# tudocomp/tudocomp

Hardware: AMD Instinct MI355X
Metric: input MB/s end-to-end lcpcomp+huffman (higher is better)
Workload: dtype u32; 1 GPU; lcpcomp(coder=huff,threshold=2,flatten=1,comp=arrays) on 2000000000 B english text (SURVEY 8d generator, seed 42): pinned host text -> H2D -> kernels + host Huffman table -> D2H -> stream in pinned host memory, all timed; bytes_per_gpu=2000000000, parallelism=single GPU

## Files before the change

tudocomp_amd/csrc/api_ctx.hip:

```cpp
#include "api.hpp"
#include "huffman_host.hpp"

#include <strings.h>
#include <ctype.h>

using namespace tdc;

namespace tdc {

int lcpcomp_enc_coder(int coder) {
    const int base = coder & 0xFF, k = coder >> 8;
    if (base == TDC_GPU_CODER_SLE) {
        if (k < 0 || k > 7) throw ArgError{TDC_GPU_ERR_ARG, "sle: kmer must be in 1..7"};
        return 3 | ((k ? k : 3) << 8);
    }
    if (k == 0 && base == TDC_GPU_CODER_HUFF) return 0;
    if (k == 0 && base == TDC_GPU_CODER_ARITH) return 1;
    if (k == 0 && base == TDC_GPU_CODER_ASCII) return 2;
    throw ArgError{TDC_GPU_ERR_UNSUPPORTED, "lcpcomp: coder must be huff, arithmetic, ascii or sle"};
}

void reserve_arena(Ctx& c, size_t bytes) {
    if (c.arena.size < bytes) {
        size_t fr = 0, tot = 0;
        if (hipMemGetInfo(&fr, &tot) == hipSuccess && fr + c.arena.size < bytes) {
            static thread_local char msg[256];
            snprintf(msg, sizeof(msg), "device %d has %.1f GB free of %.1f GB, this call needs an arena of %.1f GB (112 bytes per text byte + 192 MiB): "
                     "use smaller blocks (tdc_gpu_arena_bytes)", c.device, (double)(fr + c.arena.size) / 1e9, (double)tot / 1e9, (double)bytes / 1e9);
            throw ArgError{TDC_GPU_ERR_OOM, msg};
        }
        (void)hipGetLastError();
    }
    c.ensure_arena(bytes);
}

}

extern "C" {

const char* tdc_gpu_strerror(int status) {
    switch (status) {
        case TDC_GPU_OK: return "success";
        case TDC_GPU_ERR_HIP: return "HIP runtime error (is a gfx950 GPU visible?)";
        case TDC_GPU_ERR_ARG: return "invalid argument";
        case TDC_GPU_ERR_NO_SENTINEL: return "Expected a sentinel byte (0) at the end of the input text";
        case TDC_GPU_ERR_TOO_LARGE: return "input too large: text length must be < 2^31";
        case TDC_GPU_ERR_OOM: return "out of memory";
        case TDC_GPU_ERR_UNSUPPORTED: return "No implementation found for this coder/strategy";
        case TDC_GPU_ERR_INTERNAL: return "internal error";
        default: return "unknown status";
    }
}

const char* tdc_gpu_last_error(const tdc_gpu_ctx* ctx) { return ctx ? ctx->last_error.c_str() : ""; }

void tdc_gpu_free(void* p) { free(p); }

namespace {
struct OptionDef { const char* name; void (*set)(Ctx&, long); };
inline int clampi(long v, long lo, long hi) { return (int)(v < lo ? lo : (v > hi ? hi : v)); }
const OptionDef OPTIONS[] = {
    { "fastread",         [](Ctx& c, long v) { c.fast_read = v ? 1 : 0; } },
    { "sa_local",         [](Ctx& c, long v) { c.sa_local_sort = (int)v; } },
    { "radix_waves",      [](Ctx& c, long v) { c.radix_waves = v == 8 ? 8 : 4; } },
    { "window_lcut",      [](Ctx& c, long v) { c.window_lcut = clampi(v, 0, 63); } },
    { "window_halo",      [](Ctx& c, long v) { c.window_halo = clampi(v, 0, 2048); } },
    { "dec_seg",          [](Ctx& c, long v) { c.dec_seg = v < 4096 ? 4096 : (v > (1l << 30) ? (size_t)1 << 30 : (size_t)v); } },
    { "dec_lean",         [](Ctx& c, long v) { c.dec_lean = v != 0; } },
    { "dec_parse",        [](Ctx& c, long v) { c.dec_parse = clampi(v, 0, 2); } },
    { "dec_done",         [](Ctx& c, long v) { c.dec_done = v != 0; } },
    { "dec_log",          [](Ctx& c, long v) { c.dec_log = v != 0; } },
    { "bwt_log",          [](Ctx& c, long v) { c.bwt_log = v != 0; } },
    { "pipe_log",         [](Ctx& c, long v) { c.pipe_log = v != 0; } },
    { "window_force_fail",[](Ctx& c, long v) { c.window_force_fail = v ? 1 : 0; } },
    { "window_large",     [](Ctx& c, long v) { c.window_large_lists = v ? 1 : 0; } },
    { "window_src",       [](Ctx& c, long v) { c.window_src = v ? 1 : 0; } },
    { "plcp_samples",     [](Ctx& c, long v) { c.plcp_samples = v != 0; } },
    { "small_pipeline",   [](Ctx& c, long v) { c.small_pipeline = v != 0; } },
    { "small_big",        [](Ctx& c, long v) { c.small_big = (int)v; } },
    { "small_prof",       [](Ctx& c, long v) { c.small_prof = v != 0; } },
    { "phi_lazy",         [](Ctx& c, long v) { c.phi_lazy = v != 0; } },
    { "fs_pair",          [](Ctx& c, long v) { c.fs_pair = v != 0; } },
    { "enc_early",        [](Ctx& c, long v) { c.enc_early = (int)v; } },
    { "owner_rem",        [](Ctx& c, long v) { c.owner_rem = (int)std::min<long>(std::max<long>(v, 0), 8); } },
    { "enc_rec",          [](Ctx& c, long v) { c.enc_rec = v != 0; } },
    { "level_purge",      [](Ctx& c, long v) { c.level_purge = v != 0; } },
    { "level_log",        [](Ctx& c, long v) { c.level_log = v != 0; } },
    { "eager",            [](Ctx& c, long v) { c.eager_levels = v != 0; } },
    { "eager_dump",       [](Ctx& c, long v) { c.eager_dump = v != 0; } },
    { "flen_bytes",       [](Ctx& c, long v) { c.flen_bytes = v != 0; } },
    { "flatten_steps",    [](Ctx& c, long v) { c.flatten_steps = v <= 0 ? (1 << 30) : clampi(v, 1, 1 << 30); } },
    { "flatten_growth",   [](Ctx& c, long v) { c.flatten_growth = clampi(v, 2, 1 << 20); } },
    { "sa_refine",        [](Ctx& c, long v) { c.sa_refine = v != 0; } },
    { "sa_pairs",         [](Ctx& c, long v) { c.sa_pairs = v != 0; } },
    { "sa_stars",         [](Ctx& c, long v) { c.sa_stars = v != 0; } },
    { "sa_fused_init",    [](Ctx& c, long v) { c.sa_fused_init = v != 0; } },
    { "sa_init_syms",     [](Ctx& c, long v) { c.sa_init_syms = clampi(v, 0, 64); } },
    { "radix_lds",        [](Ctx& c, long v) { c.radix_lds = (v >= 0 && v <= 2) ? (int)v : 2; } },
    { "xcd_remap",        [](Ctx& c, long v) { c.xcd_remap = (v >= 0 && v <= 2) ? (int)v : 0; } },
    { "bucket_scatter",   [](Ctx& c, long v) { c.bucket_scatter = v ? 1 : 0; } },
    { "ssort",            [](Ctx& c, long v) { c.ssort = v ? 1 : 0; } },
    { "ssort_levels",     [](Ctx& c, long v) { c.ssort_levels = (v >= 1 && v <= 3) ? (int)v : 0; } },
    { "msd_partition",    [](Ctx& c, long v) { c.msd_partition = v ? 1 : 0; } },
    { "wsort",            [](Ctx& c, long v) { c.wsort = v ? 1 : 0; } },
    { "wsort_min",        [](Ctx& c, long v) { c.wsort_min = v < 4096 ? 4096 : (size_t)v; } },
    { "wsort_syms",       [](Ctx& c, long v) { c.wsort_syms = (v >= 4 && v <= 64) ? (int)v : 0; } },
    { "wsort_kw",         [](Ctx& c, long v) { c.wsort_kw = (v == 1 || v == 2) ? (int)v : 0; } },
    { "wsort_rounds",     [](Ctx& c, long v) { c.wsort_rounds = clampi(v, 0, 100); } },
    { "wsort_smallrun",   [](Ctx& c, long v) { c.wsort_small = v ? 1 : 0; } },
    { "wsort_overlap",    [](Ctx& c, long v) { c.wsort_overlap = v ? 1 : 0; } },
    { "wsort_predig",     [](Ctx& c, long v) { c.wsort_predig = v ? 1 : 0; } },
    { "wsort_prehist",    [](Ctx& c, long v) { c.wsort_prehist = v ? 1 : 0; } },
    { "sa_seg_bigcap",    [](Ctx& c, long v) { c.sa_seg_bigcap = clampi(v, 0, 65536); } },
    { "sa_seg_rounds",    [](Ctx& c, long v) { c.sa_seg_rounds = clampi(v, 0, 2); } },
    { "wsort_run_streams",[](Ctx& c, long v) { c.wsort_run_streams = v != 0; } },
    { "wsort_predig_skip",[](Ctx& c, long v) { c.wsort_predig_skip = clampi(v, 0, 24); } },
    { "wsort_fuse",       [](Ctx& c, long v) { c.wsort_fuse = v ? 1 : 0; } },
    { "wsort_order",      [](Ctx& c, long v) { c.wsort_order = v ? 1 : 0; } },
    { "wsort_two",        [](Ctx& c, long v) { c.wsort_two = (v >= 0 && v <= 2) ? (int)v : 0; } },
    { "wsort_leaf",       [](Ctx& c, long v) { c.wsort_leaf = v == 1024 ? 1024 : 2048; } },
    { "wsort_pack",       [](Ctx& c, long v) { c.wsort_pack = (v == 1024 || v == 4096) ? (int)v : 2048; } },
    { "wsort_cmax",       [](Ctx& c, long v) { c.wsort_cmax = clampi(v, 8, 64); } },
    { "wsort_log",        [](Ctx& c, long v) { c.wsort_log = v != 0; } },
    { "upload_chunks",    [](Ctx& c, long v) { c.upload_chunks = clampi(v, 4, 24); } },
    { "upload_tail_n",    [](Ctx& c, long v) { c.upload_tail_n = clampi(v, 0, 12); } },
    { "upload_tail_pct",  [](Ctx& c, long v) { c.upload_tail_pct = clampi(v, 30, 100); } },
    { "arena_log",        [](Ctx& c, long v) { c.arena_log = v != 0; } },
};
constexpr size_t NOPTIONS = sizeof(OPTIONS) / sizeof(OPTIONS[0]);
const OptionDef FOLD_OPTIONS[] = {
    { "fused_cand",       [](Ctx& c, long v) { c.fused_cand = v != 0; } },
    { "sel_tile_counts",  [](Ctx& c, long v) { c.sel_tile_counts = v != 0; } },
};
constexpr size_t NFOLD = sizeof(FOLD_OPTIONS) / sizeof(FOLD_OPTIONS[0]);
const OptionDef* find_option(const char* name) {
    if (!name) return nullptr;
    if (!strncasecmp(name, "TDC_GPU_", 8)) name += 8;
    for (size_t i = 0; i < NOPTIONS; ++i) if (!strcasecmp(name, OPTIONS[i].name)) return &OPTIONS[i];
    for (size_t i = 0; i < NFOLD; ++i) if (!strcasecmp(name, FOLD_OPTIONS[i].name)) return &FOLD_OPTIONS[i];
    return nullptr;
}
void apply_env_options(tdc_gpu_ctx* ctx) {
    const char* on = getenv("TDC_GPU_DEBUG_KNOBS");
    if (!on || atoi(on) == 0) return;
    for (size_t i = 0; i < NOPTIONS + NFOLD; ++i) {
        const OptionDef& o = i < NOPTIONS ? OPTIONS[i] : FOLD_OPTIONS[i - NOPTIONS];
        char var[64] = "TDC_GPU_";
        size_t k = 8;
        for (const char* q = o.name; *q && k + 1 < sizeof(var); ++q) var[k++] = (char)toupper((unsigned char)*q);
        var[k] = 0;
        if (const char* m = getenv(var)) o.set(ctx->c, atol(m));
    }
}
}

int tdc_gpu_ctx_set_option(tdc_gpu_ctx* ctx, const char* name, long value) {
    if (!ctx) return TDC_GPU_ERR_ARG;
    const OptionDef* o = find_option(name);
    if (!o) return TDC_GPU_ERR_ARG;
    o->set(ctx->c, value);
    return TDC_GPU_OK;
}
int tdc_gpu_option_count(void) { return (int)NOPTIONS; }
const char* tdc_gpu_option_name(int i) { return (i >= 0 && (size_t)i < NOPTIONS) ? OPTIONS[i].name : nullptr; }

int tdc_gpu_ctx_create(int device, tdc_gpu_ctx** out) {
    if (!out) return TDC_GPU_ERR_ARG;
    *out = nullptr;
    int count = 0;
    if (hipGetDeviceCount(&count) != hipSuccess || count <= 0) { (void)hipGetLastError(); return TDC_GPU_ERR_HIP; }
    if (device < 0 || device >= count) return TDC_GPU_ERR_ARG;
    tdc_gpu_ctx* ctx = new (std::nothrow) tdc_gpu_ctx();
    if (!ctx) return TDC_GPU_ERR_OOM;
    ctx->c.huff_ok = huffman_selfcheck();
    ctx->c.device = device;
    ctx->c.wpre = &ctx->pre;
    DeviceGuard dg(device);
    try {
        HIP_TRY(dg.enter());
        HIP_TRY(hipStreamCreateWithFlags(&ctx->c.stream, hipStreamNonBlocking));
        for (auto& e : ctx->c.ev) HIP_TRY(hipEventCreate(&e));
        HIP_TRY(hipStreamCreateWithFlags(&ctx->c.copy_stream, hipStreamNonBlocking));
        {
            int lo = 0, hi = 0;
            if (hipDeviceGetStreamPriorityRange(&lo, &hi) != hipSuccess) { lo = 0; (void)hipGetLastError(); }
            if (hipStreamCreateWithPriority(&ctx->c.aux_stream, hipStreamNonBlocking, lo) != hipSuccess) { ctx->c.aux_stream = nullptr; (void)hipGetLastError(); }
        }
        HIP_TRY(hipEventCreateWithFlags(&ctx->c.ev_join, hipEventDisableTiming));
        HIP_TRY(hipEventCreateWithFlags(&ctx->c.ev_dig2, hipEventDisableTiming));
        for (auto& e : ctx->c.ev_chunk) HIP_TRY(hipEventCreateWithFlags(&e, hipEventDisableTiming));
        ctx->c.pinned_size = 4096;
        HIP_TRY(hipHostMalloc(&ctx->c.pinned, ctx->c.pinned_size, hipHostMallocDefault));
        HIP_TRY(hipHostMalloc((void**)&ctx->c.pinned_hdr, Ctx::PINNED_HDR, hipHostMallocDefault));
        if (ctx->c.fast_read) {
            void* zc = nullptr;
            if (hipHostMalloc(&zc, (size_t)Ctx::ZC_WORDS * Ctx::ZC_BLOCKS * 4, hipHostMallocMapped | hipHostMallocCoherent) == hipSuccess) {
                void* dv = nullptr;
                if (hipHostGetDevicePointer(&dv, zc, 0) == hipSuccess) { ctx->c.zc_host = (u32*)zc; ctx->c.zc_dev = (u32*)dv; memset(zc, 0, (size_t)Ctx::ZC_WORDS * Ctx::ZC_BLOCKS * 4); }
                else { (void)hipHostFree(zc); (void)hipGetLastError(); }
            } else (void)hipGetLastError();
        }
        HIP_TRY(hipMalloc((void**)&ctx->c.d_err, 256));
        HIP_TRY(hipMemset(ctx->c.d_err, 0, 256));
        apply_env_options(ctx);
    } catch (const HipError&) {
        (void)hipGetLastError();
        tdc_gpu_ctx_destroy(ctx);
        return TDC_GPU_ERR_HIP;
    }
    *out = ctx;
    return TDC_GPU_OK;
}

void tdc_gpu_ctx_destroy(tdc_gpu_ctx* ctx) {
    if (!ctx) return;
    DeviceGuard dg(ctx->c.device);
    (void)dg.enter();
    (void)sync_streams(ctx->c);
    if (ctx->c.arena.base) (void)hipFree(ctx->c.arena.base);
    if (ctx->c.pinned) (void)hipHostFree(ctx->c.pinned);
    if (ctx->c.pinned_hdr) (void)hipHostFree(ctx->c.pinned_hdr);
    if (ctx->c.pinned_tab) (void)hipHostFree(ctx->c.pinned_tab);
    if (ctx->c.zc_host) (void)hipHostFree(ctx->c.zc_host);
    if (ctx->c.d_err) (void)hipFree(ctx->c.d_err);
    for (auto& e : ctx->c.ev) if (e) (void)hipEventDestroy(e);
    for (auto& e : ctx->c.ev_chunk) if (e) (void)hipEventDestroy(e);
    for (hipEvent_t e : {ctx->c.ev_join, ctx->c.ev_dig2}) if (e) (void)hipEventDestroy(e);
    if (ctx->c.copy_stream) (void)hipStreamDestroy(ctx->c.copy_stream);
    if (ctx->c.aux_stream) (void)hipStreamDestroy(ctx->c.aux_stream);
    if (ctx->c.ev_pool) { for (int i = 0; i < ctx->c.ev_pool_size; ++i) if (ctx->c.ev_pool[i]) (void)hipEventDestroy(ctx->c.ev_pool[i]); free(ctx->c.ev_pool); }
    free(ctx->c.pend);
    if (ctx->c.stream) (void)hipStreamDestroy(ctx->c.stream);
    delete ctx;
}

int tdc_gpu_ctx_set_profiling(tdc_gpu_ctx* ctx, int enabled) {
    return guarded(ctx, [&] {
        Ctx& c = ctx->c;
        if (enabled && !c.ev_pool) {
            c.ev_pool_size = 16384; c.pend_cap = 8192;
            c.ev_pool = (hipEvent_t*)calloc(c.ev_pool_size, sizeof(hipEvent_t));
            c.pend = (Ctx::Pending*)calloc(c.pend_cap, sizeof(Ctx::Pending));
            if (!c.ev_pool || !c.pend) throw std::bad_alloc();
            for (int i = 0; i < c.ev_pool_size; ++i) HIP_TRY(hipEventCreate(&c.ev_pool[i]));
        }
        c.profiling = enabled != 0;
    });
}

void tdc_gpu_ctx_reset_profile(tdc_gpu_ctx* ctx) {
    if (!ctx) return;
    for (auto& k : ctx->c.kprof) k = KernelProfile();
}

const char* tdc_gpu_ctx_kernel_profile(const tdc_gpu_ctx* ctx, int idx, double* ms, uint64_t* launches, uint64_t* bytes) {
    static const char* names[K_CLASS_COUNT] = {
        "rs_scatter_kernel<u64>", "rs_scatter_kernel<u32>", "rs_count_kernel", "scan_kernels",
        "sa_groups_kernel", "sa_build_keys_kernel", "phi_kernel", "plcp_kernel", "cand_kernels",
        "level_init_kernel", "mis_round_kernel", "resolve_kernel", "push_kernel", "apply_kernel", "pool_kernels", "small_level_kernel", "window_levels_kernel",
        "flatten_round_kernel", "gaps_kernel", "literal_hist_kernel", "tile_bits_kernel", "pack_kernel", "extract_kernels",
        "ss_leaf_sort_kernel", "sa_local_sort_kernel", "window_scatter_kernels",
        "ws_leaf_sort_kernel", "ws_leaf_count_kernel", "ws_run_kernels", "fs_image_kernel" };
    if (!ctx || idx < 0 || idx >= K_CLASS_COUNT) return nullptr;
    const KernelProfile& k = ctx->c.kprof[idx];
    if (ms) *ms = k.ms;
    if (launches) *launches = k.launches;
    if (bytes) *bytes = k.bytes;
    return names[idx];
}

size_t tdc_gpu_arena_bytes(size_t n) { return arena_need(n); }

int tdc_gpu_device_memory(int device, size_t* free_bytes, size_t* total_bytes) {
    if (!free_bytes || !total_bytes) return TDC_GPU_ERR_ARG;
    int count = 0;
    if (hipGetDeviceCount(&count) != hipSuccess || device < 0 || device >= count) { (void)hipGetLastError(); return TDC_GPU_ERR_ARG; }
    DeviceGuard dg(device);
    if (dg.enter() != hipSuccess || hipMemGetInfo(free_bytes, total_bytes) != hipSuccess) { (void)hipGetLastError(); return TDC_GPU_ERR_HIP; }
    return TDC_GPU_OK;
}

int tdc_gpu_ctx_reserve(tdc_gpu_ctx* ctx, size_t n) {
    return guarded(ctx, [&] { reserve_arena(ctx->c, arena_need(ctx->c, n)); });
}

int tdc_gpu_host_register(void* p, size_t bytes) {
    if (!p || !bytes) return TDC_GPU_ERR_ARG;
    if (hipHostRegister(p, bytes, hipHostRegisterPortable) != hipSuccess) { (void)hipGetLastError(); return TDC_GPU_ERR_HIP; }
    return TDC_GPU_OK;
}
int tdc_gpu_host_unregister(void* p) {
    if (!p) return TDC_GPU_ERR_ARG;
    if (hipHostUnregister(p) != hipSuccess) { (void)hipGetLastError(); return TDC_GPU_ERR_HIP; }
    return TDC_GPU_OK;
}

int tdc_gpu_device_count(void) {
    int count = 0;
    if (hipGetDeviceCount(&count) != hipSuccess) { (void)hipGetLastError(); return 0; }
    return count;
}

void* tdc_gpu_host_alloc(size_t bytes) {
    void* p = nullptr;
    if (hipHostMalloc(&p, bytes ? bytes : 1, hipHostMallocDefault) != hipSuccess) { (void)hipGetLastError(); return nullptr; }
    return p;
}
void tdc_gpu_host_free(void* p) { if (p) (void)hipHostFree(p); }

size_t tdc_escape(const uint8_t* in, size_t n, uint8_t* out) {
    size_t o = 0;
    for (size_t i = 0; i < n; ++i) {
        const uint8_t ch = in[i];
        if (ch == 0x00) { out[o++] = 0xFF; out[o++] = 0xFE; }
        else if (ch == 0xFF) { out[o++] = 0xFF; out[o++] = 0xFF; }
        else out[o++] = ch;
    }
    out[o++] = 0;
    return o;
}

size_t tdc_unescape(const uint8_t* in, size_t n, uint8_t* out) {
    size_t o = 0;
    if (n && in[n - 1] == 0) --n;
    for (size_t i = 0; i < n; ++i) {
        const uint8_t ch = in[i];
        if (ch == 0xFF && i + 1 < n) { const uint8_t d = in[++i]; out[o++] = (d == 0xFE) ? 0x00 : d; }
        else out[o++] = ch;
    }
    return o;
}

int tdc_huffman_selfcheck(void) { return huffman_selfcheck() ? TDC_GPU_OK : TDC_GPU_ERR_INTERNAL; }

int tdc_huffman_table(const uint32_t counts[256], uint32_t* sigma, uint32_t* longest, uint8_t order[256],
                      uint8_t len_of[256], uint64_t code_of[256]) {
    if (!counts) return TDC_GPU_ERR_ARG;
    try {
        HuffTable t;
        build_huffman_table(counts, &t);
        if (sigma) *sigma = t.sigma;
        if (longest) *longest = t.longest;
        if (order) memcpy(order, t.order, 256);
        if (len_of) memcpy(len_of, t.len_of, 256);
        if (code_of) memcpy(code_of, t.code_of, 256 * sizeof(uint64_t));
    } catch (...) { return TDC_GPU_ERR_OOM; }
    return TDC_GPU_OK;
}

}
```

tudocomp_amd/csrc/common.hpp:

```cpp
#pragma once

#include <hip/hip_runtime.h>
#include <stdint.h>
#include <stddef.h>
#include <stdio.h>
#include <string.h>

namespace tdc {

typedef uint8_t  u8;
typedef uint32_t u32;
typedef uint16_t u16;
typedef uint64_t u64;

constexpr u32 NONE32 = 0xFFFFFFFFu;
constexpr int WAVE = 64;

enum {
    TDC_OK = 0,
    TDC_ERR_HIP = -1,
    TDC_ERR_ARG = -2,
    TDC_ERR_NO_SENTINEL = -3,
    TDC_ERR_TOO_LARGE = -4,
    TDC_ERR_OOM = -5,
    TDC_ERR_UNSUPPORTED = -6,
    TDC_ERR_INTERNAL = -7,
};

struct HipError { hipError_t e; const char* file; int line; };

#define HIP_TRY(expr)                                                                  \
    do {                                                                               \
        hipError_t _e = (expr);                                                        \
        if (_e != hipSuccess) throw ::tdc::HipError{_e, __FILE__, __LINE__};           \
    } while (0)

inline unsigned bits_for(u64 v) {
    unsigned b = 0;
    if (v == 0) return 1;
    while (v) { ++b; v >>= 1; }
    return b;
}

inline size_t align_up(size_t x, size_t a) { return (x + a - 1) / a * a; }
inline unsigned cdiv(size_t a, size_t b) { return (unsigned)((a + b - 1) / b); }

struct Arena {
    char* base = nullptr;
    size_t size = 0;
    size_t top = 0;
    size_t high = 0;

    size_t top_hi = 0;

    void* alloc(size_t bytes) {
        size_t off = align_up(top, 256);
        if (off + bytes > size - top_hi) throw HipError{hipErrorOutOfMemory, "arena", (int)__LINE__};
        top = off + bytes;
        if (top > high) high = top;
        return base + off;
    }
    template <typename T> T* get(size_t count) { return (T*)alloc(count * sizeof(T)); }
    void* alloc_top(size_t bytes) {
        if (bytes + top_hi + 256 > size) throw HipError{hipErrorOutOfMemory, "arena (top)", (int)__LINE__};
        const size_t off = (size - top_hi - bytes) & ~(size_t)255;
        if (off < top) throw HipError{hipErrorOutOfMemory, "arena (top)", (int)__LINE__};
        top_hi = size - off;
        return base + off;
    }
    template <typename T> T* get_top(size_t count) { return (T*)alloc_top(count * sizeof(T)); }
    void release_top() { top_hi = 0; }
    size_t mark() const { return top; }
    void release(size_t m) { top = m; }
};

enum KernelClass {
    K_RS_SCATTER_U64 = 0, K_RS_SCATTER_U32, K_RS_COUNT, K_SCAN,
    K_SA_RANK_SCATTER, K_SA_BUILD_KEYS, K_PHI, K_PLCP, K_CAND,
    K_LEVEL_INIT, K_MIS_ROUND, K_RESOLVE, K_PUSH, K_APPLY, K_POOL, K_SMALL_LEVEL, K_WINDOW_LEVELS,
    K_FLATTEN_ROUND, K_ENC_GAPS, K_ENC_HIST, K_ENC_TILE_BITS, K_ENC_PACK, K_EXTRACT, K_SS_LEAF, K_SA_LOCAL_SORT, K_WINDOW_SCATTER,
    K_WS_LEAF_SORT, K_WS_LEAF_COUNT, K_WS_RUN, K_FS_IMAGE,
    K_CLASS_COUNT
};

struct KernelProfile {
    double ms = 0;
    u64 launches = 0;
    u64 bytes = 0;
};

#ifdef __HIPCC__
static __global__ void publish_words_kernel(const uint32_t* __restrict__ src, uint32_t nwords, uint32_t* host_dst, uint32_t* host_flag,
                                            uint32_t seq) {
    for (uint32_t i = threadIdx.x; i < nwords; i += blockDim.x)
        __hip_atomic_store(&host_dst[i], src[i], __ATOMIC_RELAXED, __HIP_MEMORY_SCOPE_SYSTEM);
    __syncthreads();
    if (threadIdx.x == 0) {
        __threadfence_system();
        __hip_atomic_store(host_flag, seq, __ATOMIC_RELEASE, __HIP_MEMORY_SCOPE_SYSTEM);
    }
}
#endif

struct Ctx {
    int device = 0;
    hipStream_t stream = nullptr;
    Arena arena;
    hipEvent_t ev[16] = {};
    void* pinned = nullptr;
    size_t pinned_size = 0;
    void* pinned_tab = nullptr;
    size_t pinned_tab_size = 0;
    u8* pinned_hdr = nullptr;
    static constexpr size_t PINNED_HDR = 65536;
    void* pinned_table(size_t bytes) {
        if (pinned_tab_size < bytes) {
            if (pinned_tab) { (void)hipHostFree(pinned_tab); pinned_tab = nullptr; pinned_tab_size = 0; }
            HIP_TRY(hipHostMalloc(&pinned_tab, bytes, hipHostMallocDefault));
            pinned_tab_size = bytes;
        }
        return pinned_tab;
    }
    static constexpr u32 ZC_SEG_OFF = 1040, ZC_WORDS = 1040 + 16384;
    static constexpr u32 ZC_BLOCKS = 3;
    u32* zc_host = nullptr;
    u32* zc_dev = nullptr;
    u32 zc_seq = 0;
    int fast_read = 1;
    u32* d_err = nullptr;
    int sa_local_sort = 1;
    int radix_waves = 4;
    int plcp_samples = 1;
    bool huff_ok = true;
    int flen_bytes = 1;
    int eager_levels = 1;
    int level_purge = 1;
    int enc_rec = 1;
    int owner_rem = 8;
    int enc_early = 1;
    int fused_cand = 1;
    int sel_tile_counts = 1;
    int fs_pair = 1;
    int small_big = 1;
    int small_pipeline = 1;
    int sa_pairs = 1;
    int sa_stars = 1;
    int sa_refine = 1;
    int sa_fused_init = 1;
    int radix_lds = 1;
    int xcd_remap = 1;
    int window_src = 1;
    int window_lcut = 56;
    int window_halo = 320;
    size_t dec_seg = 0;
    bool phi_lazy = true;
    int dec_lean = 1;
    int dec_parse = 1;
    int window_force_fail = 0;
    int window_large_lists = 0;
    int ssort = 1;
    int ssort_levels = 0;
    int wsort = 1;
    size_t wsort_min = (size_t)1 << 20;
    int wsort_syms = 0;
    int wsort_kw = 0;
    int wsort_rounds = 24;
    int wsort_cmax = 24;
    int wsort_overlap = 1;
    int wsort_prehist = 1;
    bool wsort_count_nonheads = true;
    int sa_seg_bigcap = 65536;
    int sa_seg_rounds = 2;
    int wsort_run_streams = 1;
    int wsort_predig_skip = 4;
    int wsort_predig = 1;
    int wsort_two = 0;
    int wsort_leaf = 2048;
    int wsort_pack = 1024;
    int wsort_order = 1;
    int wsort_fuse = 1;
    int wsort_small = 0;
    int msd_partition = 1;
    int bucket_scatter = 1;
    int upload_tail_n = 3, upload_tail_pct = 60;
    int upload_chunks = 16;
    int flatten_steps = 1;
    int flatten_growth = 8;
    int sa_init_syms = 0;
    int dec_done = 1;
    int dec_log = 0, bwt_log = 0, pipe_log = 0, level_log = 0, wsort_log = 0, eager_dump = 0, small_prof = 0, arena_log = 0;

    u32 hist_cache[256] = {};
    const u8* hist_ptr = nullptr;
    size_t hist_n = 0;
    hipStream_t copy_stream = nullptr;
    hipStream_t aux_stream = nullptr;
    hipEvent_t ev_join = nullptr;
    static constexpr size_t CHUNK_EVENTS = 32;
    hipEvent_t ev_chunk[CHUNK_EVENTS] = {};
    hipEvent_t ev_dig2 = nullptr;
    struct WPre* wpre = nullptr;
    u8* d2h_host = nullptr;
    size_t d2h_cap = 0;
    size_t d2h_done = 0;

    bool profiling = false;
    KernelProfile kprof[K_CLASS_COUNT];
    struct Pending { hipEvent_t a, b; int cls; u64 bytes; };
    Pending* pend = nullptr;
    int npend = 0, pend_cap = 0;
    hipEvent_t* ev_pool = nullptr;
    int ev_pool_size = 0, ev_pool_used = 0;

    int prof_begin(int cls, u64 bytes) {
        if (!profiling || npend >= pend_cap || ev_pool_used + 2 > ev_pool_size) return -1;
        Pending& p = pend[npend];
        p.a = ev_pool[ev_pool_used++]; p.b = ev_pool[ev_pool_used++]; p.cls = cls; p.bytes = bytes;
        HIP_TRY(hipEventRecord(p.a, stream));
        return npend++;
    }
    void prof_end(int idx) { if (idx >= 0) HIP_TRY(hipEventRecord(pend[idx].b, stream)); }
    void wait_for(hipStream_t waiter, hipStream_t signaller) {
        HIP_TRY(hipEventRecord(ev_join, signaller));
        HIP_TRY(hipStreamWaitEvent(waiter, ev_join, 0));
    }
    struct ProfScope {
        Ctx& c; int idx;
        ProfScope(Ctx& ctx, int cls, u64 bytes) : c(ctx), idx(ctx.prof_begin(cls, bytes)) {}
        ~ProfScope() { if (idx >= 0) (void)hipEventRecord(c.pend[idx].b, c.stream); }
    };
    void prof_collect() {
        for (int i = 0; i < npend; ++i) {
            float t = 0;
            HIP_TRY(hipEventElapsedTime(&t, pend[i].a, pend[i].b));
            KernelProfile& k = kprof[pend[i].cls];
            k.ms += t; k.launches++; k.bytes += pend[i].bytes;
        }
        npend = 0; ev_pool_used = 0;
    }

    void ensure_arena(size_t bytes) {
        arena.top_hi = 0;
        if (arena.size >= bytes) { arena.top = 0; return; }
        if (arena.base) { HIP_TRY(hipFree(arena.base)); arena.base = nullptr; arena.size = 0; }
        HIP_TRY(hipMalloc((void**)&arena.base, bytes));
        if (arena_log) fprintf(stderr, "arena: %zu bytes at %p\n", bytes, (void*)arena.base);
        arena.size = bytes;
        arena.top = 0;
    }
#ifdef __HIPCC__
    bool read_words_fast(const void* dptr, void* out, size_t bytes) {
        if (!fast_read || !zc_host || bytes == 0 || bytes > 4096 || (bytes & 3) || ((uintptr_t)dptr & 3)) return false;
        const u32 seq = ++zc_seq;
        publish_words_kernel<<<1, 64, 0, stream>>>((const u32*)dptr, (u32)(bytes / 4), zc_dev, zc_dev + 1024, seq);
        if (hipGetLastError() != hipSuccess) return false;
        volatile u32* flag = zc_host + 1024;
        for (u64 spins = 0;; ++spins) {
            if (__atomic_load_n((const u32*)flag, __ATOMIC_ACQUIRE) == seq) break;
            if ((spins & 0xFFFF) == 0xFFFF) {
                const hipError_t q = hipStreamQuery(stream);
                if (q != hipSuccess && q != hipErrorNotReady) throw HipError{q, __FILE__, __LINE__};
            }
        }
        memcpy(out, zc_host, bytes);
        return true;
    }
    bool publish_begin(u32** dst, u32** flag, u32* seq, u32 block = 0) {
        if (!fast_read || !zc_host) return false;
        *seq = ++zc_seq; *dst = zc_dev + (size_t)block * ZC_WORDS; *flag = *dst + 1024;
        return true;
    }
    u32 publish_async(const void* dptr, size_t bytes, u32 block) {
        if (!fast_read || !zc_host || bytes == 0 || bytes > 4096 || (bytes & 3) || ((uintptr_t)dptr & 3) || block >= ZC_BLOCKS) return 0;
        u32 seq = ++zc_seq;
        if (seq == 0) seq = ++zc_seq;
        u32* dst = zc_dev + (size_t)block * ZC_WORDS;
        publish_words_kernel<<<1, 64, 0, stream>>>((const u32*)dptr, (u32)(bytes / 4), dst, dst + 1024, seq);
        return hipGetLastError() == hipSuccess ? seq : 0;
    }
    void publish_wait(u32 seq, void* out, size_t bytes, u32 block = 0) {
        volatile u32* flag = zc_host + (size_t)block * ZC_WORDS + 1024;
        for (u64 spins = 0;; ++spins) {
            if (__atomic_load_n((const u32*)flag, __ATOMIC_ACQUIRE) == seq) break;
            if ((spins & 0xFFFF) == 0xFFFF) {
                const hipError_t q = hipStreamQuery(stream);
                if (q != hipSuccess && q != hipErrorNotReady) throw HipError{q, __FILE__, __LINE__};
            }
        }
        memcpy(out, zc_host + (size_t)block * ZC_WORDS, bytes);
    }
#else
    bool read_words_fast(const void*, void*, size_t) { return false; }
#endif
    template <typename T> T read(const T* dptr) {
        T v;
        if (read_words_fast(dptr, &v, sizeof(T))) return v;
        T* h = (T*)pinned;
        HIP_TRY(hipMemcpyAsync(h, dptr, sizeof(T), hipMemcpyDeviceToHost, stream));
        HIP_TRY(hipStreamSynchronize(stream));
        return *h;
    }
    template <typename T> void read_n(const T* dptr, T* out, size_t count) {
        const size_t bytes = sizeof(T) * count;
        if (read_words_fast(dptr, out, bytes)) return;
        if (bytes <= pinned_size) {
            HIP_TRY(hipMemcpyAsync(pinned, dptr, bytes, hipMemcpyDeviceToHost, stream));
            HIP_TRY(hipStreamSynchronize(stream));
            memcpy(out, pinned, bytes);
        } else {
            HIP_TRY(hipMemcpyAsync(out, dptr, bytes, hipMemcpyDeviceToHost, stream));
            HIP_TRY(hipStreamSynchronize(stream));
        }
    }
};

struct StreamSwap {
    Ctx& c; hipStream_t saved;
    StreamSwap(Ctx& ctx, hipStream_t other) : c(ctx), saved(ctx.stream) { c.stream = other; }
    ~StreamSwap() { c.stream = saved; }
};

#define LAUNCH_CHECK() HIP_TRY(hipGetLastError())

#ifdef __HIPCC__

__device__ __forceinline__ int lane_id() { return threadIdx.x & 63; }

__device__ __forceinline__ u32 xcd_tile(u32 bid, u32 per_xcd) { return per_xcd ? (bid & 7u) * per_xcd + (bid >> 3) : bid; }
__device__ __forceinline__ int wave_id() { return threadIdx.x >> 6; }

__device__ __forceinline__ u32 wave_inclusive_sum_u32(u32 v) {
    v += (u32)__builtin_amdgcn_update_dpp(0, (int)v, 0x111, 0xF, 0xF, false);
    v += (u32)__builtin_amdgcn_update_dpp(0, (int)v, 0x112, 0xF, 0xF, false);
    v += (u32)__builtin_amdgcn_update_dpp(0, (int)v, 0x114, 0xF, 0xF, false);
    v += (u32)__builtin_amdgcn_update_dpp(0, (int)v, 0x118, 0xF, 0xF, false);
    v += (u32)__builtin_amdgcn_update_dpp(0, (int)v, 0x142, 0xA, 0xF, false);
    v += (u32)__builtin_amdgcn_update_dpp(0, (int)v, 0x143, 0xC, 0xF, false);
    return v;
}
template <typename T>
__device__ __forceinline__ T wave_inclusive_sum(T v) {
    if constexpr (sizeof(T) == 4) return (T)wave_inclusive_sum_u32((u32)v);
    const int lane = lane_id();
#pragma unroll
    for (int d = 1; d < 64; d <<= 1) {
        T o = __shfl_up(v, d, 64);
        if (lane >= d) v += o;
    }
    return v;
}
__device__ __forceinline__ u32 wave_inclusive_max(u32 v) {
    v = max(v, (u32)__builtin_amdgcn_update_dpp(0, (int)v, 0x111, 0xF, 0xF, false));
    v = max(v, (u32)__builtin_amdgcn_update_dpp(0, (int)v, 0x112, 0xF, 0xF, false));
    v = max(v, (u32)__builtin_amdgcn_update_dpp(0, (int)v, 0x114, 0xF, 0xF, false));
    v = max(v, (u32)__builtin_amdgcn_update_dpp(0, (int)v, 0x118, 0xF, 0xF, false));
    v = max(v, (u32)__builtin_amdgcn_update_dpp(0, (int)v, 0x142, 0xA, 0xF, false));
    v = max(v, (u32)__builtin_amdgcn_update_dpp(0, (int)v, 0x143, 0xC, 0xF, false));
    return v;
}
template <typename T>
__device__ __forceinline__ T wave_reduce_sum(T v) {
    if constexpr (sizeof(T) == 4) return (T)__builtin_amdgcn_readlane((int)wave_inclusive_sum_u32((u32)v), 63);
#pragma unroll
    for (int d = 32; d >= 1; d >>= 1) v += __shfl_xor(v, d, 64);
    return v;
}
__device__ __forceinline__ u32 wave_reduce_max(u32 v) { return (u32)__builtin_amdgcn_readlane((int)wave_inclusive_max(v), 63); }
__device__ __forceinline__ u32 wave_reduce_min(u32 v) { return ~wave_reduce_max(~v); }

template <typename T> __device__ __forceinline__ T lds_load(const T* p) { return *(const volatile __attribute__((address_space(3))) T*)p; }
template <typename T> __device__ __forceinline__ void lds_store(T* p, T v) { *(volatile __attribute__((address_space(3))) T*)p = v; }

__device__ __forceinline__ u64 wave_match_lds(unsigned long long* M, u32 d, bool valid, u64 lanebit) {
    const u32 d0 = __builtin_amdgcn_readfirstlane(d);
    if (__all(valid && d == d0)) return ~0ull;
#ifdef TDC_MATCH_B64
    if (valid) atomicOr(&M[d], (unsigned long long)lanebit);
#else
    if (valid) atomicOr((unsigned*)&M[d] + (lane_id() >> 5), (unsigned)(lanebit >> (32 * (lane_id() >> 5))));
#endif
    __builtin_amdgcn_wave_barrier();
    const u64 peers = valid ? lds_load(&M[d]) : 0ull;
    __builtin_amdgcn_wave_barrier();
    if (valid) lds_store(&M[d], 0ull);
    return peers;
}

template <int PEEL, int MING>
__device__ __forceinline__ u64 wave_match_peel(unsigned long long* M, u32 d, bool valid, u64 lanebit) {
    u64 rem = __ballot(valid);
    u64 peers = 0;
    bool done = !valid;
#pragma unroll
    for (int it = 0; it < PEEL; ++it) {
        if (!rem) break;
        const int lead = __builtin_ctzll(rem);
        const u32 dl = (u32)__builtin_amdgcn_readlane((int)d, lead);
        const u64 grp = __ballot(!done && d == dl);
        if (__popcll(grp) < MING) break;
        if (!done && d == dl) { peers = grp; done = true; }
        rem &= ~grp;
    }
    if (rem) {
        if (!done) atomicOr((unsigned*)&M[d] + (lane_id() >> 5), (unsigned)(lanebit >> (32 * (lane_id() >> 5))));
        __builtin_amdgcn_wave_barrier();
        if (!done) peers = lds_load(&M[d]);
        __builtin_amdgcn_wave_barrier();
        if (!done) lds_store(&M[d], 0ull);
    }
    return peers;
}

template <typename T, int NW>
__device__ __forceinline__ T block_exclusive_sum(T v, T* smem, T& total) {
    const int lane = lane_id(), w = wave_id();
    T inc = wave_inclusive_sum(v);
    if (lane == 63) smem[w] = inc;
    __syncthreads();
    if (threadIdx.x == 0) {
        T run = 0;
#pragma unroll
        for (int i = 0; i < NW; ++i) { T t = smem[i]; smem[i] = run; run += t; }
        smem[NW] = run;
    }
    __syncthreads();
    T res = smem[w] + inc - v;
    total = smem[NW];
    __syncthreads();
    return res;
}

template <int NW>
__device__ __forceinline__ u32 block_inclusive_max(u32 v, u32* smem, u32& total) {
    const int lane = lane_id(), w = wave_id();
    u32 inc = wave_inclusive_max(v);
    if (lane == 63) smem[w] = inc;
    __syncthreads();
    if (threadIdx.x == 0) {
        u32 run = 0;
#pragma unroll
        for (int i = 0; i < NW; ++i) { u32 t = smem[i]; smem[i] = run; run = max(run, t); }
        smem[NW] = run;
    }
    __syncthreads();
// ... 62 lines not shown
```

tudocomp_amd/csrc/fused.hip:

```cpp
#include "stages.hpp"
#include "prim.hpp"

#include <type_traits>

namespace tdc {

constexpr int FS_TILE = 4096;
constexpr int FS_ITEMS = 16;
constexpr u32 FS_WMAX = 8192;

struct FSLevel {
    const u32* idx_in; const void* rp_in; const u32* prev_in; const u8* lcp_in;
    u32* idx_out; void* rp_out; u8* lcp_out;
    u32* counts; const u32* blk_seg; const u32* blk_start; const u32* seg_start;
    u32 nseg, R, per_xcd; int shift;
    int lsh;
};
__device__ __forceinline__ bool fs_row(const FSLevel& P, u32 row, size_t& base, u32& cnt) {
    const u32 blk = row / P.R;
    if (blk >= P.blk_start[P.nseg]) return false;
    const u32 s = P.blk_seg[blk];
    const u64 t = (u64)(blk - P.blk_start[s]) * P.R + row % P.R;
    const u32 s0 = P.seg_start[s], s1 = P.seg_start[s + 1];
    const u64 off = t * FS_TILE;
    base = s0; cnt = 0;
    if (off >= (u64)(s1 - s0)) return true;
    base = (size_t)s0 + off;
    const u64 left = (u64)(s1 - s0) - off;
    cnt = left < FS_TILE ? (u32)left : (u32)FS_TILE;
    return true;
}

template <int DB>
__global__ __launch_bounds__(256) void fs_count_kernel(FSLevel P, u32 rows) {
    constexpr u32 D = 1u << DB;
    __shared__ u32 hist[D];
    const u32 row = xcd_tile(blockIdx.x, P.per_xcd);
    if (row >= rows) return;
    size_t base; u32 cnt;
    if (!fs_row(P, row, base, cnt)) return;
    for (u32 i = threadIdx.x; i < D; i += 256) hist[i] = 0;
    if (cnt == 0) { for (u32 i = threadIdx.x; i < D; i += 256) P.counts[(size_t)row * D + i] = 0; return; }
    __syncthreads();
    const u32 lb = wave_id() * (64 * FS_ITEMS) + lane_id();
    const u32* ip = P.idx_in + base + lb;
    u32 kk[FS_ITEMS];
#pragma unroll
    for (int j = 0; j < FS_ITEMS; ++j) kk[j] = (lb + (u32)j * 64 < cnt) ? ip[j * 64] : 0u;
#pragma unroll
    for (int j = 0; j < FS_ITEMS; ++j) {
        const bool valid = lb + (u32)j * 64 < cnt;
        const u32 d = (kk[j] >> P.shift) & (D - 1);
        const u32 d0 = __builtin_amdgcn_readfirstlane(d);
        if (__all(valid && d == d0)) { if (lane_id() == 0) atomicAdd(&hist[d0], 64u); }
        else if (valid) atomicAdd(&hist[d], 1u);
    }
    __syncthreads();
    for (u32 i = threadIdx.x; i < D; i += 256) P.counts[(size_t)row * D + i] = hist[i];
}

#ifndef TDC_FS_WPE
#define TDC_FS_WPE 4
#endif
template <int DB, bool FIRST, int PAIR, bool WP>
__global__ __launch_bounds__(256 * PAIR) __attribute__((amdgpu_waves_per_eu(TDC_FS_WPE, TDC_FS_WPE))) void fs_scatter_kernel(FSLevel P, u32 rows) {
    constexpr int NT = 256 * PAIR;
    constexpr u32 TILE = (u32)FS_TILE * PAIR;
    constexpr u32 D = 1u << DB;
    __shared__ u32 tcnt[D];
    __shared__ u32 gbase[D];
    __shared__ __align__(16) u64 stage[TILE];
    __shared__ u32 scan_sm[NT / 64 + 1];
    const int lane = lane_id();
    const u32 row = xcd_tile(blockIdx.x, P.per_xcd) * PAIR;
    if (row >= rows) return;
    size_t base; u32 cnt;
    if (!fs_row(P, row, base, cnt) || cnt == 0) return;
    if (PAIR == 2 && row + 1 < rows) {
        size_t base2; u32 cnt2;
        if (fs_row(P, row + 1, base2, cnt2) && cnt2) cnt += cnt2;
    }
    for (u32 i = threadIdx.x; i < D; i += NT) tcnt[i] = 0;
    __syncthreads();
    const u32 lb = wave_id() * (64 * FS_ITEMS) + lane;
    const u32* ip = P.idx_in + base + lb;
    u32 k[FS_ITEMS], pos[FS_ITEMS];
#pragma unroll
    for (int j = 0; j < FS_ITEMS; ++j) k[j] = (lb + (u32)j * 64 < cnt) ? ip[j * 64] : 0u;
    using RT = typename std::conditional<WP, u64, u32>::type;
    RT rp[FS_ITEMS];
    u32 lc[FS_ITEMS];
    const u8* lst = (const u8*)stage;
    size_t lmis = 0;
    if (FIRST) {
        const u8* src = P.lcp_in + base;
        lmis = ((size_t)src) & 15;
        const uint4* a0 = (const uint4*)(src - lmis);
        const u32 nv = (cnt + (u32)lmis + 15u) / 16u;
        for (u32 i = threadIdx.x; i < nv; i += NT) ((uint4*)stage)[i] = a0[i];
        __syncthreads();
    }
#pragma unroll
    for (int j = 0; j < FS_ITEMS; ++j) {
        const u32 e = lb + (u32)j * 64;
        const bool valid = e < cnt;
        if (FIRST) { if constexpr (WP) rp[j] = (u64)(u32)(base + e + 1) | ((u64)(valid ? P.prev_in[base + e] : 0u) << 32); else rp[j] = (u32)(base + e + 1); }
        else rp[j] = valid ? ((const RT*)P.rp_in)[base + e] : (RT)0;
        lc[j] = (FIRST && valid) ? (u32)lst[lmis + e] : 0u;
    }
#pragma unroll
    for (int j = 0; j < FS_ITEMS; ++j) {
        const bool valid = lb + (u32)j * 64 < cnt;
        const u32 d = (k[j] >> P.shift) & (D - 1);
        const u32 d0 = __builtin_amdgcn_readfirstlane(d);
        u32 rank = 0;
        if (__all(valid && d == d0)) {
            if (lane == 0) rank = atomicAdd(&tcnt[d0], 64u);
            rank = __builtin_amdgcn_readfirstlane(rank) + (u32)lane;
        } else if (valid) rank = atomicAdd(&tcnt[d], 1u);
        pos[j] = rank;
    }
    __syncthreads();
    {
        const u32 t = threadIdx.x;
        constexpr u32 DPT = (D + NT - 1) / NT;
        u32 tot[DPT], sum = 0;
#pragma unroll
        for (u32 q = 0; q < DPT; ++q) { const u32 d = t * DPT + q; tot[q] = d < D ? tcnt[d] : 0u; sum += tot[q]; }
        u32 total;
        u32 start = block_exclusive_sum<u32, NT / 64>(sum, scan_sm, total);
#pragma unroll
        for (u32 q = 0; q < DPT; ++q) {
            const u32 d = t * DPT + q;
            if (d < D) {
                tcnt[d] = start;
                gbase[d] = P.counts[(size_t)row * D + d] - start;
            }
            start += tot[q];
        }
    }
    __syncthreads();
    u32 dst[FS_ITEMS];
    u32* stage32 = (u32*)stage;
    unsigned short* stage_d = (unsigned short*)(stage + TILE / 2);
#pragma unroll
    for (int j = 0; j < FS_ITEMS; ++j) {
        if (lb + (u32)j * 64 < cnt) {
            const u32 d = (k[j] >> P.shift) & (D - 1);
            pos[j] += tcnt[d];
            stage32[pos[j]] = FIRST ? ((k[j] & ((1u << P.lsh) - 1u)) | (lc[j] << P.lsh)) : k[j];
            stage_d[pos[j]] = (unsigned short)d;
        }
    }
    __syncthreads();
#pragma unroll
    for (int r = 0; r < FS_ITEMS; ++r) {
        const u32 sp = (u32)r * NT + threadIdx.x;
        dst[r] = 0xFFFFFFFFu;
        if (sp < cnt) {
            dst[r] = gbase[stage_d[sp]] + sp;
            P.idx_out[dst[r]] = stage32[sp];
        }
    }
    __syncthreads();
    RT* stage2 = (RT*)stage;
#pragma unroll
    for (int j = 0; j < FS_ITEMS; ++j) if (lb + (u32)j * 64 < cnt) stage2[pos[j]] = rp[j];
    __syncthreads();
#pragma unroll
    for (int r = 0; r < FS_ITEMS; ++r) if (dst[r] != 0xFFFFFFFFu) ((RT*)P.rp_out)[dst[r]] = stage2[(u32)r * NT + threadIdx.x];
}

constexpr int FS_IMG_T = 1024;
struct FSCand { u32 threshold, lcut; u8* cls; u8* res8; u8* flen8; u32* flen; u32* tilecnt; u32* acc; };
template <bool WP, bool CF>
__global__ __launch_bounds__(FS_IMG_T) void fs_image_kernel(const u32* __restrict__ idx, const void* __restrict__ rp_v, int lsh, size_t m, u32 W,
                                                             u32* __restrict__ isa, u32* __restrict__ phi, u32* __restrict__ plcp, u32* __restrict__ d_max,
                                                             FSCand cf) {
    __shared__ __align__(16) u32 img[FS_WMAX];
    __shared__ u32 smx[FS_IMG_T / 64];
    __shared__ u32 scf[CF ? FS_IMG_T / 64 : 1];
    __shared__ u32 shist[CF ? 64 : 1];
    if (CF && threadIdx.x < 64) shist[threadIdx.x] = 0;
    constexpr int R = FS_WMAX / FS_IMG_T;
    const size_t base = (size_t)blockIdx.x * W;
    const size_t end = (base + W < m) ? base + W : m;
    using RT = typename std::conditional<WP, u64, u32>::type;
    const RT* rp = (const RT*)rp_v;
    u32 ix[R];
    RT rr[R];
    u32 mx = 0;
#pragma unroll
    for (int r = 0; r < R; ++r) {
        const size_t j = base + (size_t)r * FS_IMG_T + threadIdx.x;
        const bool have = j < end;
        ix[r] = have ? idx[j] : 0xFFFFFFFFu;
        rr[r] = have ? rp[j] : (RT)0;
    }
#pragma unroll
    for (int r = 0; r < R; ++r) if (ix[r] != 0xFFFFFFFFu) img[ix[r] & (W - 1)] = (u32)rr[r];
    __syncthreads();
#pragma unroll
    for (int r = 0; r < R; ++r) { const size_t q = base + (size_t)r * FS_IMG_T + threadIdx.x; if (q < end) isa[q] = img[q - base]; }
    __syncthreads();
    if constexpr (WP) {
#pragma unroll
        for (int r = 0; r < R; ++r) if (ix[r] != 0xFFFFFFFFu) img[ix[r] & (W - 1)] = (u32)(rr[r] >> 32);
        __syncthreads();
#pragma unroll
        for (int r = 0; r < R; ++r) { const size_t q = base + (size_t)r * FS_IMG_T + threadIdx.x; if (q < end) phi[q] = img[q - base]; }
        __syncthreads();
    }
#pragma unroll
    for (int r = 0; r < R; ++r) if (ix[r] != 0xFFFFFFFFu) { const u32 l = (ix[r] >> lsh) & 0xFFu; img[ix[r] & (W - 1)] = l; mx = max(mx, l); }
    __syncthreads();
#pragma unroll
    for (int r = 0; r < R; ++r) { const size_t q = base + (size_t)r * FS_IMG_T + threadIdx.x; if (q < end) plcp[q] = img[q - base]; }
    if constexpr (CF) {
        u32 ncand = 0;
#pragma unroll
        for (int r = 0; r < R / 4; ++r) {
            const u32 o = ((u32)r * FS_IMG_T + threadIdx.x) * 4;
            const size_t q = base + o;
            u32 cw = 0, rw = 0, nv = 0;
            if (q < end) {
                nv = (end - q < 4) ? (u32)(end - q) : 4u;
                const uint4 x = *(const uint4*)&img[o];
                const u32 v[4] = { x.x, x.y, x.z, x.w };
#pragma unroll
                for (int j = 0; j < 4; ++j) {
                    if ((u32)j >= nv) break;
                    const u32 is_cand = (v[j] >= cf.threshold) ? 1u : 0u;
                    cw |= ((is_cand && v[j] > cf.lcut) ? 1u : 0u) << (8 * j);
                    rw |= (is_cand ? (v[j] > 255u ? 255u : v[j]) : 0u) << (8 * j);
                    ncand += is_cand;
                    if (j == 0 && cf.lcut && is_cand && v[j] < 64u && (q & 15) == 0) atomicAdd(&shist[v[j]], 1u);
                }
                if (nv == 4) {
                    *(u32*)(cf.cls + q) = cw;
                    if (cf.res8) *(u32*)(cf.res8 + q) = rw;
                    if (cf.flen8) *(u32*)(cf.flen8 + q) = 0u; else *(uint4*)(cf.flen + q) = make_uint4(0, 0, 0, 0);
                } else {
                    for (u32 j = 0; j < nv; ++j) {
                        cf.cls[q + j] = (u8)(cw >> (8 * j));
                        if (cf.res8) cf.res8[q + j] = (u8)(rw >> (8 * j));
                        if (cf.flen8) cf.flen8[q + j] = 0; else cf.flen[q + j] = 0;
                    }
                }
            }
            if (cf.tilecnt) {
                const u32 wsum = wave_reduce_sum((u32)__popc(cw));
                if (lane_id() == 0 && wsum) atomicAdd(&cf.tilecnt[q / SEL_TILE_CLASSES], wsum);
            }
        }
        ncand = wave_reduce_sum(ncand);
        if (lane_id() == 0) scf[wave_id()] = ncand;
    }
    mx = wave_reduce_max(mx);
    if (lane_id() == 0) smx[wave_id()] = mx;
    __syncthreads();
    if (wave_id() == 0) {
        u32 v = (lane_id() < FS_IMG_T / 64) ? smx[lane_id()] : 0u;
        v = wave_reduce_max(v);
        if (lane_id() == 0 && v) atomicMax(d_max, v);
    }
    if constexpr (CF) {
        u32* acc = cf.acc + (size_t)(blockIdx.x % CF_COPIES) * CF_ACC;
        if (threadIdx.x < 64) { if (shist[threadIdx.x]) atomicAdd(&acc[threadIdx.x], shist[threadIdx.x]); }
        else if (threadIdx.x == 64) { u32 t = 0; for (int i = 0; i < FS_IMG_T / 64; ++i) t += scf[i]; if (t) atomicAdd(&acc[64], t); }
    }
}
__global__ void fs_cand_fold_kernel(const u32* __restrict__ acc, u32* __restrict__ out) {
    if (threadIdx.x > 64) return;
    u32 t = 0;
    for (u32 k = 0; k < CF_COPIES; ++k) t += acc[(size_t)k * CF_ACC + threadIdx.x];
    out[threadIdx.x] = t;
}

__global__ void fs_first_kernel(const u32* __restrict__ sa, size_t n, u32* __restrict__ isa, u32* __restrict__ phi, u32* __restrict__ plcp, FSCand cf) {
    const u32 p = sa[0];
    isa[p] = 0; if (phi) phi[p] = sa[n - 1]; plcp[p] = 0;
    if (cf.cls) {
        cf.cls[p] = 0;
        if (cf.res8) cf.res8[p] = 0;
        if (cf.flen8) cf.flen8[p] = 0; else cf.flen[p] = 0;
    }
}
__global__ void fs_direct_kernel(const u32* __restrict__ sa, const u8* __restrict__ lcp8, size_t n, u32* __restrict__ isa, u32* __restrict__ phi,
                                 u32* __restrict__ plcp, u32* __restrict__ d_max) {
    const size_t i = (size_t)blockIdx.x * blockDim.x + threadIdx.x;
    u32 l = 0;
    if (i < n) {
        const u32 p = sa[i];
        isa[p] = (u32)i;
        if (phi) phi[p] = (i == 0) ? sa[n - 1] : sa[i - 1];
        l = (i == 0) ? 0u : (u32)lcp8[i];
        plcp[p] = l;
    }
    l = wave_reduce_max(l);
    if (lane_id() == 0 && l) atomicMax(d_max, l);
}

bool fused_scatter_has_image(const Ctx& c, size_t n) { return n >= ((size_t)1 << 20) && c.bucket_scatter; }

void build_isa_phi_plcp_fused(Ctx& c, const u32* sa, const u8* lcp8, size_t n, u32* isa, u32* phi, u32* plcp, u32* d_maxlcp, CandFused* cf) {
    hipStream_t s = c.stream;
    if (cf) cf->filled = false;
    HIP_TRY(hipMemsetAsync(d_maxlcp, 0, sizeof(u32), s));
    if (!n) return;
    const int bits = (int)bits_for(n - 1);
    if (!fused_scatter_has_image(c, n)) {
        Ctx::ProfScope prof(c, K_PHI, (u64)n * 17);
        fs_direct_kernel<<<cdiv(n, 256), 256, 0, s>>>(sa, lcp8, n, isa, phi, plcp, d_maxlcp);
        LAUNCH_CHECK();
        return;
    }
    const size_t mark = c.arena.mark();
    const size_t m = n - 1;
    const int db = (bits - 16 > 13) ? 9 : 8;
    const u32 D = 1u << db;
    u32* idx[2] = { c.arena.get<u32>(m), c.arena.get<u32>(m) };
    const bool wp = phi != nullptr;
    void* rp[2] = { c.arena.alloc(m * (wp ? 8 : 4)), c.arena.alloc(m * (wp ? 8 : 4)) };
    const u32* seg_start = ss_first_segment(c, m);
    u32 nseg = 1;
    for (int l = 0; l < 2; ++l) {
        u32* nstart = c.arena.get<u32>((size_t)nseg * D + 1);
        const size_t lm = c.arena.mark();
        SegTables Tb;
        ss_level_tables(c, seg_start, nseg, m, D, Tb);
        FSLevel P;
        if (l == 0) { P.idx_in = sa + 1; P.rp_in = nullptr; P.prev_in = sa; P.lcp_in = lcp8 + 1; }
        else { P.idx_in = idx[0]; P.rp_in = rp[0]; P.prev_in = nullptr; P.lcp_in = nullptr; }
        P.idx_out = idx[l]; P.rp_out = rp[l]; P.lcp_out = nullptr;
        P.lsh = bits - db;
        P.counts = Tb.counts; P.blk_seg = Tb.blk_seg; P.blk_start = Tb.blk_start; P.seg_start = seg_start;
        P.nseg = nseg; P.R = Tb.R; P.shift = bits - db * (l + 1);
        const u32 rows = Tb.rows;
        P.per_xcd = (c.xcd_remap == 1 && rows >= 64) ? cdiv(rows, 8) : 0u;
        const u32 grid = P.per_xcd ? 8 * P.per_xcd : rows;
        {
            const int pc = c.prof_begin(K_RS_COUNT, (u64)m * 4);
            if (db == 9) fs_count_kernel<9><<<grid, 256, 0, s>>>(P, rows); else fs_count_kernel<8><<<grid, 256, 0, s>>>(P, rows);
            LAUNCH_CHECK();
            c.prof_end(pc);
        }
        ss_level_offsets(c, Tb, seg_start, nseg, D, nstart, m);
        {
            const int ps = c.prof_begin(K_RS_SCATTER_U32, (u64)m * (wp ? (l == 0 ? 5 + 12 : 24) : (l == 0 ? 5 + 8 : 16)));
            const bool pair = (Tb.R % 2) == 0 && c.fs_pair;
            FSLevel P2 = P;
            const u32 groups = pair ? (rows + 1) / 2 : rows;
            P2.per_xcd = (c.xcd_remap == 1 && groups >= 64) ? cdiv(groups, 8) : 0u;
            const u32 grid2 = P2.per_xcd ? 8 * P2.per_xcd : groups;
            auto launch = [&](auto wpc) {
                constexpr bool WPC = decltype(wpc)::value;
                if (pair) {
                    if (l == 0) { if (db == 9) fs_scatter_kernel<9, true, 2, WPC><<<grid2, 512, 0, s>>>(P2, rows); else fs_scatter_kernel<8, true, 2, WPC><<<grid2, 512, 0, s>>>(P2, rows); }
                    else { if (db == 9) fs_scatter_kernel<9, false, 2, WPC><<<grid2, 512, 0, s>>>(P2, rows); else fs_scatter_kernel<8, false, 2, WPC><<<grid2, 512, 0, s>>>(P2, rows); }
                } else {
                    if (l == 0) { if (db == 9) fs_scatter_kernel<9, true, 1, WPC><<<grid, 256, 0, s>>>(P, rows); else fs_scatter_kernel<8, true, 1, WPC><<<grid, 256, 0, s>>>(P, rows); }
                    else { if (db == 9) fs_scatter_kernel<9, false, 1, WPC><<<grid, 256, 0, s>>>(P, rows); else fs_scatter_kernel<8, false, 1, WPC><<<grid, 256, 0, s>>>(P, rows); }
                }
            };
            if (wp) launch(std::true_type{}); else launch(std::false_type{});
            LAUNCH_CHECK();
            c.prof_end(ps);
        }
        c.arena.release(lm);
        seg_start = nstart;
        nseg *= D;
    }
    {
        const u32 W = 1u << (bits - 2 * db);
        if (W > FS_WMAX) throw HipError{hipErrorUnknown, "fused scatter: window larger than the LDS image", (int)__LINE__};
        if (W < 16) throw HipError{hipErrorUnknown, "fused scatter: window smaller than a thread's group of positions", (int)__LINE__};
        FSCand fc{};
        if (cf) {
            if (!cf->cls || !cf->acc || !cf->lvlhist || (!cf->flen8 && !cf->flen) || (cf->lcut && !cf->res8))
                throw HipError{hipErrorUnknown, "fused scatter: candidate arrays missing", (int)__LINE__};
            fc.threshold = cf->threshold; fc.lcut = cf->lcut;
            fc.cls = cf->cls; fc.res8 = cf->lcut ? cf->res8 : nullptr; fc.flen8 = cf->flen8; fc.flen = cf->flen; fc.tilecnt = cf->tilecnt; fc.acc = cf->acc;
            HIP_TRY(hipMemsetAsync(cf->acc, 0, (size_t)CF_COPIES * CF_ACC * sizeof(u32), s));
            if (cf->tilecnt) HIP_TRY(hipMemsetAsync(cf->tilecnt, 0, (size_t)cdiv(n, SEL_TILE_CLASSES) * sizeof(u32), s));
        }
        Ctx::ProfScope prof(c, K_FS_IMAGE, (u64)m * (wp ? 24 : 16) + (cf ? (u64)m * ((cf->lcut ? 2 : 1) + (cf->flen8 ? 1 : 4)) : 0));
        if (cf) {
            if (wp) fs_image_kernel<true, true><<<cdiv(m, W), FS_IMG_T, 0, s>>>(idx[1], rp[1], bits - db, m, W, isa, phi, plcp, d_maxlcp, fc);
            else fs_image_kernel<false, true><<<cdiv(m, W), FS_IMG_T, 0, s>>>(idx[1], rp[1], bits - db, m, W, isa, phi, plcp, d_maxlcp, fc);
        } else {
            if (wp) fs_image_kernel<true, false><<<cdiv(m, W), FS_IMG_T, 0, s>>>(idx[1], rp[1], bits - db, m, W, isa, phi, plcp, d_maxlcp, fc);
            else fs_image_kernel<false, false><<<cdiv(m, W), FS_IMG_T, 0, s>>>(idx[1], rp[1], bits - db, m, W, isa, phi, plcp, d_maxlcp, fc);
        }
        LAUNCH_CHECK();
        fs_first_kernel<<<1, 1, 0, s>>>(sa, n, isa, phi, plcp, fc);
        LAUNCH_CHECK();
        if (cf) {
            fs_cand_fold_kernel<<<1, 128, 0, s>>>(cf->acc, cf->lvlhist);
            LAUNCH_CHECK();
            cf->filled = true;
        }
    }
    c.arena.release(mark);
}

}
```

tudocomp_amd/csrc/prim.hpp:

```cpp
#pragma once
#include "common.hpp"

namespace tdc {

void exclusive_sum_u32(Ctx& c, const u32* in, u32* out, size_t n, u32* d_total);
void exclusive_sum_u64(Ctx& c, const u64* in, u64* out, size_t n, u64* d_total);
void inclusive_max_u32(Ctx& c, const u32* in, u32* out, size_t n);

int radix_sort_pairs_u64(Ctx& c, u64* keys[2], u32* vals[2], size_t n, int begin_bit, int end_bit);
int radix_sort_pairs_u32(Ctx& c, u32* keys[2], u32* vals[2], size_t n, int begin_bit, int end_bit);

struct TextKeyGen { const u8* text; size_t n; u32 sigma; int k, chunk; u64 top ; u8 code[256]; };
int radix_sort_text_keys_u64(Ctx& c, const TextKeyGen& g, u64* keys[2], u32* vals[2], int end_bit);

struct SplitSortStats { u32 levels = 0, range_leaves = 0, samples = 0, units = 0, large_leaves = 0, wide_units = 0; u64 large_pairs = 0; };
bool splitter_sort_applicable(size_t n);
int splitter_sort_pairs_u64(Ctx& c, u64* keys[2], u32* vals[2], size_t n, const TextKeyGen* gen, SplitSortStats* st);

void msd_partition_pairs_u32(Ctx& c, const u32* idx, const u32* val, size_t m, int bits, int db, u32* out_idx, u32* out_val, u32* tmp_idx, u32* tmp_val);

struct SegTables { u32* blk_start; u32* blk_seg; u32* counts; u32* bs; u32 R, blocks_ub, rows; };
struct UnitTables { u32* unit_rng; u32* cls_list; u32* large; u32 cap, large_cap; u32 hc[6];  int wide_classes = 0;  u32 whc[16] = {0, 0, 0, 0, 0, 0, 0, 0, 0, 0, 0, 0, 0, 0, 0, 0};  };
constexpr int WIDE_NCLS = 10;
__host__ __device__ inline u32 wide_class(u32 m) {
    if (m <= 2048u) return m <= 1024u ? 0u : (m - 769u) / 256u;
    if (m <= 4096u) return 5u + (m <= 2560u ? 0u : (m - 2049u) / 512u);
    return 9u;
}
u32* ss_first_segment(Ctx& c, size_t n);
void ss_level_tables(Ctx& c, const u32* seg_start, u32 nseg, size_t n, u32 D, SegTables& T);
void ss_level_offsets(Ctx& c, const SegTables& T, const u32* seg_start, u32 nseg, u32 D, u32* nstart, size_t n);
void ss_level_offsets_sub(Ctx& c, const SegTables& T, u32 nsub, const u32* blk_super, const u32* out_start, u32 nsuper, u32 D, u32* nstart, size_t n);
void ss_build_units(Ctx& c, const u32* leaf_start, u32 nleaf, UnitTables& U, u32 small = 0);
void ss_fanouts(Ctx& c, size_t n, int& L, u32 F[3], u32& os, u32 leaf3 = 0, int wide2 = 0);

struct WKeyGen { const u8* text; size_t n; int b, s, pad; u32 inv ; u8 code[256]; };
struct WSortStats { u32 levels = 0, range_leaves = 0, samples = 0, units = 0, large_leaves = 0, kw = 0, refined_units = 0, trunc_units = 0, longrun_units = 0, leaf_stages = 0, wave_runs = 0; u64 large_pairs = 0; u64 nonheads = 0; };
struct WPre {
    bool begun = false, active = false;
    const u8* text = nullptr; size_t n = 0;
    int KW = 0; WKeyGen g;
    int L = 0; u32 F[3] = { 1, 1, 1 }; u32 os = 0, NLr = 0, NS = 0, S = 0;
    u64* K1[2] = { nullptr, nullptr }; u64* K2[2] = { nullptr, nullptr }; u32* V[2] = { nullptr, nullptr };
    u16* digits = nullptr; u64* sp1 = nullptr; u64* sp2 = nullptr;
    u32 nchunks = 0; size_t chunk_off[33] = {};
    u32* nstart_all = nullptr;
    const u32* dig2_counts[32] = {}; const u32* dig2_blk[32] = {}; u32 dig2_R[32] = {};
    bool dig2 = false; u32 dig2_chunks = 0;
    u32 present[8] = { 0, 0, 0, 0, 0, 0, 0, 0 };
};
bool wsort_pre_begin(Ctx& c, WPre& P, const u8* text, size_t n, const size_t* chunk_off, u32 nchunks, const u32* hist0);
void wsort_pre_chunk(Ctx& c, WPre& P, u32 q);
void wsort_pre_finish(Ctx& c, WPre& P, const u32* hist_full);
bool wsort_applicable(const Ctx& c, size_t n);
void wsort_make_keygen(const Ctx& c, const u8* text, size_t n, u32 sigma, const u8* code, int& KW, WKeyGen& g);
int wsort_result_index(Ctx& c, size_t n);
int wsort_suffixes(Ctx& c, int KW, const WKeyGen& g, u64* K1[2], u64* K2[2], u32* V[2], size_t n, u8* flags, u8* lcp8, WSortStats* st);
void wsort_suffixes_pre(Ctx& c, const WPre& P, u32* v_final, u8* flags, u8* lcp8, WSortStats* st);
int wsort_records(Ctx& c, u64* K1[2], u64* K2[2], u32* V[2], size_t m, int k1_bits, WSortStats* st);
bool wsort_sorted_runs(Ctx& c, const u64* k1, u64* k2, u32* v, size_t m, int k1_bits);
bool wsort_sorted_runs_from_text(Ctx& c, const u32* a_sa, const u32* a_r1, size_t m, const WKeyGen& g, u32 h, u64* k1, u64* k2, u32* v, int k1_bits);

int sort_pairs_u64_distinct(Ctx& c, u64* keys[2], u32* vals[2], size_t n, int begin_bit, int end_bit);

void bucketed_scatter_u32(Ctx& c, const u32* idx, const u32* val, size_t m, u32* dst, size_t n_dst, u32* tmp_idx, u32* tmp_val,
                          u32* tmp_idx2, u32* tmp_val2, bool permutation = false);

constexpr size_t SEL_TILE_CLASSES = 2048;
void select_by_class(Ctx& c, const u8* cls, u8 want, size_t m, const u32* srcA, u32* outA, const u64* srcB, u64* outB,
                     u32* d_count, const u32* tile_counts = nullptr);

void mark_orbit_u32(Ctx& c, const u32* next, size_t n, u8* mark, u32* scratch1, u32* scratch2);

void fill_u32(Ctx& c, u32* p, size_t n, u32 v);
void fill_u8(Ctx& c, u8* p, size_t n, u8 v);

}
```

tudocomp_amd/csrc/ssort.hip:

```cpp
#include "prim.hpp"

#include <vector>

namespace tdc {

constexpr int SS_TILE = 4096;
constexpr int SS_ITEMS = 16;
constexpr int SS_SMALL = 4096;
constexpr int SS_UNIT_MAX = 8192;
constexpr int SS_GEN_HALO = 32;

struct SSLevel {
    const u64* keys_in; const u32* vals_in;
    u64* keys_out; u32* vals_out;
    u32* counts;
    const u32* blk_seg;
    const u32* blk_start;
    const u32* seg_start;
    const u64* sp;
    u16* digits;
    u32 nseg, F, stride, R, D, per_xcd;
};

__device__ __forceinline__ bool ss_row(const SSLevel& P, u32 row, u32& s, size_t& base, u32& cnt) {
    const u32 blk = row / P.R;
    if (blk >= P.blk_start[P.nseg]) return false;
    s = P.blk_seg[blk];
    const u64 t = (u64)(blk - P.blk_start[s]) * P.R + row % P.R;
    const u32 s0 = P.seg_start[s], s1 = P.seg_start[s + 1];
    const u64 off = t * SS_TILE;
    base = s0; cnt = 0;
    if (off >= (u64)(s1 - s0)) return true;
    base = (size_t)s0 + off;
    const u64 left = (u64)(s1 - s0) - off;
    cnt = left < SS_TILE ? (u32)left : (u32)SS_TILE;
    return true;
}

template <bool LAST>
__device__ __forceinline__ void ss_load_splitters(const SSLevel& P, u32 s, u64* spl) {
    for (u32 i = threadIdx.x; i < 256; i += blockDim.x) {
        u64 v = ~0ull;
        if (LAST) { if (i < P.F) v = P.sp[(size_t)s * P.F + i]; }
        else if (i + 1 < P.F) v = P.sp[((size_t)s * P.F + i + 1) * P.stride - 1];
        spl[i] = v;
    }
}

template <bool LAST>
__device__ __forceinline__ u32 ss_digit(const u64* spl, u64 x) {
    u32 lo = 0;
#pragma unroll
    for (u32 step = 128; step >= 1; step >>= 1) lo += (spl[lo + step - 1] < x) ? step : 0u;
    if (LAST) return 2 * lo + (spl[lo] == x ? 1u : 0u);
    return lo;
}

__device__ __forceinline__ void ss_gen_stage(const TextKeyGen& g, size_t t0, const u8* __restrict__ code, u8* __restrict__ sy) {
    const size_t p = t0 + (size_t)threadIdx.x * 16;
    u8 b[16];
    if (p + 16 <= g.n && (((size_t)g.text) & 15) == 0) {
        const uint4 v = *(const uint4*)(g.text + p);
        const u32 wv[4] = { v.x, v.y, v.z, v.w };
#pragma unroll
        for (int i = 0; i < 16; ++i) b[i] = (u8)(wv[i >> 2] >> (8 * (i & 3)));
    } else {
#pragma unroll
        for (int i = 0; i < 16; ++i) b[i] = (p + i < g.n) ? g.text[p + i] : (u8)0;
    }
    u32 o[4] = { 0, 0, 0, 0 };
#pragma unroll
    for (int i = 0; i < 16; ++i) o[i >> 2] |= (u32)((p + i < g.n) ? code[b[i]] : (u8)0) << (8 * (i & 3));
    *(uint4*)(sy + (size_t)threadIdx.x * 16) = make_uint4(o[0], o[1], o[2], o[3]);
    if (threadIdx.x < SS_GEN_HALO) {
        const size_t q = t0 + SS_TILE + threadIdx.x;
        sy[SS_TILE + threadIdx.x] = (q < g.n) ? code[g.text[q]] : (u8)0;
    }
}
__device__ __forceinline__ u64 ss_gen_key(const TextKeyGen& g, const u8* sy, int lb) {
    u64 key = 0;
    for (int j0 = 0; j0 < g.k; j0 += g.chunk) {
        const int len = (g.k - j0 < g.chunk) ? g.k - j0 : g.chunk;
        u32 acc = 0, scale = 1;
        for (int t = 0; t < len; ++t) { acc = acc * g.sigma + sy[lb + j0 + t]; scale *= g.sigma; }
        key = (j0 == 0) ? (u64)acc : key * scale + acc;
    }
    return key;
}

__device__ __forceinline__ size_t ss_sample_pos(u32 i, size_t n) {
    const u64 h = ((u64)i + 1) * 0x9E3779B97F4A7C15ull;
    return (size_t)(((unsigned __int128)(h ^ (h >> 29)) * n) >> 64);
}
template <bool GEN>
__global__ __launch_bounds__(256) void ss_sample_kernel(const u64* __restrict__ keys, TextKeyGen g, size_t n, u32 S, u64* __restrict__ out,
                                                        u32* __restrict__ dummy) {
    __shared__ u8 code[256];
    if (GEN) { code[threadIdx.x] = g.code[threadIdx.x]; __syncthreads(); }
    const u32 i = blockIdx.x * 256 + threadIdx.x;
    if (i >= S) return;
    const size_t p = ss_sample_pos(i, n);
    u64 key;
    if (GEN) {
        key = 0;
        for (int j0 = 0; j0 < g.k; j0 += g.chunk) {
            const int len = (g.k - j0 < g.chunk) ? g.k - j0 : g.chunk;
            u32 acc = 0, scale = 1;
            for (int t = 0; t < len; ++t) {
                const size_t q = p + j0 + t;
                acc = acc * g.sigma + ((q < n) ? code[g.text[q]] : 0u);
                scale *= g.sigma;
            }
            key = (j0 == 0) ? (u64)acc : key * scale + acc;
        }
    } else key = keys[p];
    out[i] = key;
    dummy[i] = i;
}
__global__ void ss_pick_kernel(const u64* __restrict__ sorted, u32 NS, u32 os, u64* __restrict__ sp) {
    const u32 i = blockIdx.x * blockDim.x + threadIdx.x;
    if (i < NS) sp[i] = sorted[(size_t)(i + 1) * os - 1];
    else if (i == NS) sp[i] = ~0ull;
}

__global__ void ss_nblk_kernel(const u32* __restrict__ seg_start, u32 nseg, u32 R, u32* __restrict__ nblk) {
    const u32 s = blockIdx.x * blockDim.x + threadIdx.x;
    if (s > nseg) return;
    if (s == nseg) { nblk[s] = 0; return; }
    const u64 size = seg_start[s + 1] - seg_start[s];
    nblk[s] = (u32)((size + (u64)SS_TILE * R - 1) / ((u64)SS_TILE * R));
}
__global__ void ss_blkseg_kernel(const u32* __restrict__ blk_start, u32 nseg, u32* __restrict__ blk_seg) {
    const u32 s = blockIdx.x * blockDim.x + threadIdx.x;
    if (s >= nseg) return;
    for (u32 b = blk_start[s]; b < blk_start[s + 1]; ++b) blk_seg[b] = s;
}

template <bool GEN, bool LAST>
__global__ __launch_bounds__(256) void ss_count_kernel(SSLevel P, TextKeyGen g, u32 rows) {
    __shared__ u32 hist[512];
    __shared__ u64 spl[256];
    __shared__ u8 code[256];
    __shared__ __align__(16) u8 sy[GEN ? SS_TILE + SS_GEN_HALO : 16];
    const u32 row = xcd_tile(blockIdx.x, P.per_xcd);
    if (row >= rows) return;
    u32 s, cnt; size_t base;
    if (!ss_row(P, row, s, base, cnt)) return;
    for (u32 i = threadIdx.x; i < P.D; i += 256) hist[i] = 0;
    if (cnt == 0) {
        for (u32 i = threadIdx.x; i < P.D; i += 256) P.counts[(size_t)row * P.D + i] = 0;
        return;
    }
    ss_load_splitters<LAST>(P, s, spl);
    if (GEN) code[threadIdx.x] = g.code[threadIdx.x];
    __syncthreads();
    if (GEN) { ss_gen_stage(g, base, code, sy); __syncthreads(); }
    if (GEN) {
        const int lb = wave_id() * (64 * SS_ITEMS) + lane_id() * SS_ITEMS;
        u64 key = ss_gen_key(g, sy, lb);
        u32 pk[SS_ITEMS / 2];
#pragma unroll
        for (int j = 0; j < SS_ITEMS; ++j) {
            const bool valid = (u32)(lb + j) < cnt;
            const u32 d = valid ? ss_digit<LAST>(spl, key) : 0u;
            key = (key - (u64)sy[lb + j] * g.top) * g.sigma + sy[lb + j + g.k];
            pk[j >> 1] = (j & 1) ? (pk[j >> 1] | (d << 16)) : d;
            const u32 d0 = __builtin_amdgcn_readfirstlane(d);
            if (__all(valid && d == d0)) { if (lane_id() == 0) atomicAdd(&hist[d0], 64u); }
            else if (valid) atomicAdd(&hist[d], 1u);
        }
        uint4* dp = (uint4*)(P.digits + base + lb);
        dp[0] = make_uint4(pk[0], pk[1], pk[2], pk[3]);
        dp[1] = make_uint4(pk[4], pk[5], pk[6], pk[7]);
    } else {
        const u32 lb = wave_id() * (64 * SS_ITEMS) + lane_id();
        const u64* kp = P.keys_in + base + lb;
        u16* dgp = P.digits + base + lb;
        u64 kk[SS_ITEMS];
#pragma unroll
        for (int j = 0; j < SS_ITEMS; ++j) kk[j] = (lb + (u32)j * 64 < cnt) ? kp[j * 64] : 0ull;
#pragma unroll 4
        for (int j = 0; j < SS_ITEMS; ++j) {
            const u32 e = lb + (u32)j * 64;
            const bool valid = e < cnt;
            const u32 d = valid ? ss_digit<LAST>(spl, kk[j]) : 0u;
            if (valid) dgp[j * 64] = (u16)d;
            const u32 d0 = __builtin_amdgcn_readfirstlane(d);
            if (__all(valid && d == d0)) { if (lane_id() == 0) atomicAdd(&hist[d0], 64u); }
            else if (valid) atomicAdd(&hist[d], 1u);
        }
    }
    __syncthreads();
    for (u32 i = threadIdx.x; i < P.D; i += 256) P.counts[(size_t)row * P.D + i] = hist[i];
}

__global__ __launch_bounds__(256) void ss_blocksum_kernel(const u32* __restrict__ counts, const u32* __restrict__ blk_start, u32 nseg,
                                                          u32 R, u32 D, u32* __restrict__ bs) {
    const u32 b = blockIdx.x;
    if (b >= blk_start[nseg]) return;
    for (u32 d = threadIdx.x; d < D; d += 256) {
        u32 acc = 0;
        for (u32 r = 0; r < R; ++r) acc += counts[((size_t)b * R + r) * D + d];
        bs[(size_t)b * D + d] = acc;
    }
}
__global__ __launch_bounds__(1024) void ss_segbase_kernel(u32* __restrict__ bs, const u32* __restrict__ blk_start, const u32* __restrict__ seg_start,
                                                          u32 D, u32* __restrict__ next_start) {
    __shared__ u32 part[4][2048];
    __shared__ u32 dstart[2048];
    __shared__ u32 wsum[16];
    const u32 s = blockIdx.x;
    const u32 b0 = blk_start[s], b1 = blk_start[s + 1];
    const u32 t = threadIdx.x & 255u, g = threadIdx.x >> 8;
    const u32 nb = b1 - b0, per = (nb + 3) / 4;
    const u32 lo = b0 + (g * per < nb ? g * per : nb);
    const u32 hi = (lo + per < b1) ? lo + per : b1;
    for (u32 d = t; d < D; d += 256) {
        u32 acc = 0;
        u32 b = lo;
        for (; b + 8 <= hi; b += 8) {
            u32 v[8];
#pragma unroll
            for (int i = 0; i < 8; ++i) v[i] = bs[(size_t)(b + i) * D + d];
#pragma unroll
            for (int i = 0; i < 8; ++i) acc += v[i];
        }
        for (; b < hi; ++b) acc += bs[(size_t)b * D + d];
        part[g][d] = acc;
    }
    __syncthreads();
    const u32 d0 = 2 * threadIdx.x, d1 = d0 + 1;
    const u32 tot0 = d0 < D ? part[0][d0] + part[1][d0] + part[2][d0] + part[3][d0] : 0u;
    const u32 tot1 = d1 < D ? part[0][d1] + part[1][d1] + part[2][d1] + part[3][d1] : 0u;
    const u32 tot = tot0 + tot1;
    u32 inc = wave_inclusive_sum(tot);
    if (lane_id() == 63) wsum[wave_id()] = inc;
    __syncthreads();
    {
        u32 run = 0;
        for (int w = 0; w < wave_id(); ++w) run += wsum[w];
        const u32 st = seg_start[s] + run + inc - tot;
        if (d0 < D) { dstart[d0] = st; next_start[(size_t)s * D + d0] = st; }
        if (d1 < D) { dstart[d1] = st + tot0; next_start[(size_t)s * D + d1] = st + tot0; }
    }
    __syncthreads();
    for (u32 d = t; d < D; d += 256) {
        u32 run = dstart[d];
        for (u32 k = 0; k < g; ++k) run += part[k][d];
        u32 b = lo;
        for (; b + 8 <= hi; b += 8) {
            u32 v[8];
#pragma unroll
            for (int i = 0; i < 8; ++i) v[i] = bs[(size_t)(b + i) * D + d];
#pragma unroll
            for (int i = 0; i < 8; ++i) { bs[(size_t)(b + i) * D + d] = run; run += v[i]; }
        }
        for (; b < hi; ++b) { const u32 v = bs[(size_t)b * D + d]; bs[(size_t)b * D + d] = run; run += v; }
    }
}
__global__ __launch_bounds__(256) void ss_apply_kernel(u32* __restrict__ counts, const u32* __restrict__ blk_start, u32 nseg, u32 R, u32 D,
                                                       const u32* __restrict__ bs) {
    const u32 b = blockIdx.x;
    if (b >= blk_start[nseg]) return;
    for (u32 d = threadIdx.x; d < D; d += 256) {
        u32 run = bs[(size_t)b * D + d];
        for (u32 r = 0; r < R; ++r) {
            const size_t i = ((size_t)b * R + r) * D + d;
            const u32 v = counts[i];
            counts[i] = run;
            run += v;
        }
    }
}
__global__ void ss_set_word_kernel(u32* p, u32 v) { *p = v; }

template <bool GEN, bool LAST>
__global__ __launch_bounds__(256) __attribute__((amdgpu_waves_per_eu(4, 4))) void ss_scatter_kernel(SSLevel P, TextKeyGen g, u32 rows) {
    constexpr int DMAX = LAST ? 512 : 256;
    __shared__ u32 tcnt[DMAX];
    __shared__ u32 gbase[DMAX];
    __shared__ __align__(16) u64 stage[SS_TILE];
    __shared__ u32 scan_sm[5];
    __shared__ u8 code[GEN ? 256 : 4];
    const int lane = lane_id(), w = wave_id();
    const u32 row = xcd_tile(blockIdx.x, P.per_xcd);
    if (row >= rows) return;
    u32 s, cnt; size_t base;
    if (!ss_row(P, row, s, base, cnt) || cnt == 0) return;
    u8* sy = (u8*)stage;
    u16* stage_d = (u16*)(stage + 2048);
    u32* stage32 = (u32*)stage;
    for (int i = threadIdx.x; i < DMAX; i += 256) tcnt[i] = 0;
    if (GEN) code[threadIdx.x] = g.code[threadIdx.x];
    __syncthreads();
    if (GEN) { ss_gen_stage(g, base, code, sy); __syncthreads(); }

    u64 k[SS_ITEMS];
    u32 v[SS_ITEMS];
    u32 ld[SS_ITEMS];
    const u32 lbs = GEN ? (u32)(w * (64 * SS_ITEMS) + lane * SS_ITEMS) : (u32)(w * (64 * SS_ITEMS) + lane);
    u64 gkey = 0;
    u32 pk[SS_ITEMS / 2];
    if (GEN) {
        gkey = ss_gen_key(g, sy, (int)lbs);
        const uint4* dp = (const uint4*)(P.digits + base + lbs);
        const uint4 q0 = dp[0], q1 = dp[1];
        pk[0] = q0.x; pk[1] = q0.y; pk[2] = q0.z; pk[3] = q0.w; pk[4] = q1.x; pk[5] = q1.y; pk[6] = q1.z; pk[7] = q1.w;
    }
    const u64* kp = GEN ? nullptr : P.keys_in + base + lbs;
    const u32* vp = GEN ? nullptr : P.vals_in + base + lbs;
    const u16* dgp = P.digits + base + lbs;
#pragma unroll
    for (int j = 0; j < SS_ITEMS; ++j) {
        const u32 e = GEN ? lbs + (u32)j : lbs + (u32)j * 64;
        const bool valid = e < cnt;
        if (GEN) {
            k[j] = gkey; v[j] = (u32)(base + e);
            gkey = (gkey - (u64)sy[lbs + j] * g.top) * g.sigma + sy[lbs + j + g.k];
            ld[j] = (pk[j >> 1] >> (16 * (j & 1))) & 0xFFFFu;
        } else {
            k[j] = valid ? kp[j * 64] : 0ull;
            v[j] = valid ? vp[j * 64] : 0u;
            ld[j] = valid ? (u32)dgp[j * 64] : 0u;
        }
    }
#pragma unroll
    for (int j = 0; j < SS_ITEMS; ++j) {
        const u32 e = GEN ? lbs + (u32)j : lbs + (u32)j * 64;
        const bool valid = e < cnt;
        const u32 d = valid ? ld[j] : 0u;
        u32 rank = 0;
        {
            u64 rem = __ballot(valid);
            bool done = !valid;
#pragma unroll
            for (int it = 0; it < 2; ++it) {
                if (!rem) break;
                const int lead = __ffsll((long long)rem) - 1;
                const u32 dl = __shfl(d, lead, 64);
                const u64 grp = __ballot(!done && d == dl);
                const u32 c = (u32)__popcll(grp);
                if (c < 8) break;
                u32 b0 = 0;
                if (lane == lead) b0 = atomicAdd(&tcnt[dl], c);
                b0 = __shfl(b0, lead, 64);
                if ((grp >> lane) & 1ull) { rank = b0 + (u32)__popcll(grp & ((1ull << lane) - 1)); done = true; }
                rem &= ~grp;
            }
            if (!done) rank = atomicAdd(&tcnt[d], 1u);
        }
        ld[j] = (d << 16) | rank;
    }
    __syncthreads();
    {
        const u32 t = threadIdx.x;
        u32 tot[DMAX / 256], sum = 0;
#pragma unroll
        for (int q = 0; q < DMAX / 256; ++q) {
            tot[q] = tcnt[t * (DMAX / 256) + q];
            sum += tot[q];
        }
        u32 total;
        u32 start = block_exclusive_sum<u32, 4>(sum, scan_sm, total);
#pragma unroll
        for (int q = 0; q < DMAX / 256; ++q) {
            const u32 d = t * (DMAX / 256) + q;
            tcnt[d] = start;
            gbase[d] = (d < P.D ? P.counts[(size_t)row * P.D + d] : 0u) - start;
            start += tot[q];
        }
    }
    __syncthreads();
    u32 dst[SS_ITEMS];
#pragma unroll
    for (int j = 0; j < SS_ITEMS; ++j) {
        const u32 e = GEN ? lbs + (u32)j : lbs + (u32)j * 64;
        const u32 d = ld[j] >> 16;
        const u32 pos = (ld[j] & 0xFFFFu) + tcnt[d];
        ld[j] = pos;
        if (e < cnt) { stage32[pos] = v[j]; stage_d[pos] = (u16)d; }
    }
    __syncthreads();
#pragma unroll
    for (int r = 0; r < SS_ITEMS; ++r) {
        const u32 sp = (u32)r * 256 + threadIdx.x;
        dst[r] = 0xFFFFFFFFu;
        if (sp < cnt) {
            dst[r] = gbase[stage_d[sp]] + sp;
            P.vals_out[dst[r]] = stage32[sp];
        }
    }
    __syncthreads();
#pragma unroll
    for (int j = 0; j < SS_ITEMS; ++j) {
        const u32 e = GEN ? lbs + (u32)j : lbs + (u32)j * 64;
        if (e < cnt) stage[ld[j]] = k[j];
    }
    __syncthreads();
#pragma unroll
    for (int r = 0; r < SS_ITEMS; ++r) {
        const u32 sp = (u32)r * 256 + threadIdx.x;
        if (dst[r] != 0xFFFFFFFFu) P.keys_out[dst[r]] = stage[sp];
    }
}

template <bool GEN, bool LAST>
__global__ __launch_bounds__(256) __attribute__((amdgpu_waves_per_eu(4, 4))) void ss_scatter_stable_kernel(SSLevel P, TextKeyGen g, u32 rows) {
    constexpr int DMAX = LAST ? 512 : 256;
    __shared__ __align__(16) u16 wcnt[4][DMAX];
    __shared__ u32 gbase[DMAX];
    __shared__ __align__(16) u64 stage[SS_TILE];
    __shared__ u32 scan_sm[5];
    __shared__ u8 code[GEN ? 256 : 4];
    const int lane = lane_id(), w = wave_id();
    const u32 row = xcd_tile(blockIdx.x, P.per_xcd);
    if (row >= rows) return;
    u32 s, cnt; size_t base;
    if (!ss_row(P, row, s, base, cnt) || cnt == 0) return;
    u8* sy = (u8*)stage;
    u16* stage_d = (u16*)(stage + 2048);
    u32* stage32 = (u32*)stage;
    unsigned long long* M = (unsigned long long*)stage + 1024 + w * DMAX;
    for (int i = threadIdx.x; i < 4 * DMAX; i += 256) { (&wcnt[0][0])[i] = 0; ((unsigned long long*)stage)[1024 + i] = 0; }
    if (GEN) code[threadIdx.x] = g.code[threadIdx.x];
    __syncthreads();
    if (GEN) { ss_gen_stage(g, base, code, sy); __syncthreads(); }

    u64 k[SS_ITEMS];
    u32 v[SS_ITEMS];
    u32 ld[SS_ITEMS];
    u16* mycnt = wcnt[w];
    const u64 lanebit = 1ull << lane;
    const u64 lt_mask = (lane == 0) ? 0ull : (~0ull >> (64 - lane));
    const u32 lbs = GEN ? (u32)(w * (64 * SS_ITEMS) + lane * SS_ITEMS) : (u32)(w * (64 * SS_ITEMS) + lane);
    u64 gkey = 0;
    u32 pk[SS_ITEMS / 2];
    if (GEN) {
        gkey = ss_gen_key(g, sy, (int)lbs);
        const uint4* dp = (const uint4*)(P.digits + base + lbs);
        const uint4 q0 = dp[0], q1 = dp[1];
        pk[0] = q0.x; pk[1] = q0.y; pk[2] = q0.z; pk[3] = q0.w; pk[4] = q1.x; pk[5] = q1.y; pk[6] = q1.z; pk[7] = q1.w;
    }
    const u64* kp = GEN ? nullptr : P.keys_in + base + lbs;
    const u32* vp = GEN ? nullptr : P.vals_in + base + lbs;
    const u16* dgp = P.digits + base + lbs;
#pragma unroll
    for (int j = 0; j < SS_ITEMS; ++j) {
        const u32 e = GEN ? lbs + (u32)j : lbs + (u32)j * 64;
        const bool valid = e < cnt;
        if (GEN) {
            k[j] = gkey; v[j] = (u32)(base + e);
            gkey = (gkey - (u64)sy[lbs + j] * g.top) * g.sigma + sy[lbs + j + g.k];
            ld[j] = (pk[j >> 1] >> (16 * (j & 1))) & 0xFFFFu;
        } else {
            k[j] = valid ? kp[j * 64] : 0ull;
            v[j] = valid ? vp[j * 64] : 0u;
            ld[j] = valid ? (u32)dgp[j * 64] : 0u;
        }
    }
#pragma unroll
    for (int j = 0; j < SS_ITEMS; ++j) {
        const u32 e = GEN ? lbs + (u32)j : lbs + (u32)j * 64;
        const bool valid = e < cnt;
        const u32 d = valid ? ld[j] : 0u;
        const u64 peers = wave_match_lds(M, d, valid, lanebit);
        const u32 prefix = lds_load(&mycnt[d]);
        const u32 rank = (u32)__popcll(peers & lt_mask);
        ld[j] = (d << 16) | (prefix + rank);
        if (valid && rank == 0) lds_store(&mycnt[d], (u16)(prefix + (u32)__popcll(peers)));
    }
    __syncthreads();
    {
        const u32 t = threadIdx.x;
        u32 tot[DMAX / 256], sum = 0;
#pragma unroll
        for (int q = 0; q < DMAX / 256; ++q) {
            const u32 d = t * (DMAX / 256) + q;
            tot[q] = (u32)wcnt[0][d] + wcnt[1][d] + wcnt[2][d] + wcnt[3][d];
            sum += tot[q];
        }
        u32 total;
        u32 start = block_exclusive_sum<u32, 4>(sum, scan_sm, total);
#pragma unroll
        for (int q = 0; q < DMAX / 256; ++q) {
            const u32 d = t * (DMAX / 256) + q;
            u32 run = start;
#pragma unroll
            for (int i = 0; i < 4; ++i) { const u32 c = wcnt[i][d]; wcnt[i][d] = (u16)run; run += c; }
            gbase[d] = (d < P.D ? P.counts[(size_t)row * P.D + d] : 0u) - start;
            start += tot[q];
        }
    }
    __syncthreads();
    u32 dst[SS_ITEMS];
#pragma unroll
    for (int j = 0; j < SS_ITEMS; ++j) {
        const u32 e = GEN ? lbs + (u32)j : lbs + (u32)j * 64;
        const u32 d = ld[j] >> 16;
        const u32 pos = (ld[j] & 0xFFFFu) + wcnt[w][d];
        ld[j] = pos;
        if (e < cnt) { stage32[pos] = v[j]; stage_d[pos] = (u16)d; }
    }
    __syncthreads();
#pragma unroll
    for (int r = 0; r < SS_ITEMS; ++r) {
        const u32 sp = (u32)r * 256 + threadIdx.x;
        dst[r] = 0xFFFFFFFFu;
        if (sp < cnt) {
            dst[r] = gbase[stage_d[sp]] + sp;
            P.vals_out[dst[r]] = stage32[sp];
        }
    }
    __syncthreads();
#pragma unroll
    for (int j = 0; j < SS_ITEMS; ++j) {
        const u32 e = GEN ? lbs + (u32)j : lbs + (u32)j * 64;
        if (e < cnt) stage[ld[j]] = k[j];
    }
    __syncthreads();
#pragma unroll
    for (int r = 0; r < SS_ITEMS; ++r) {
        const u32 sp = (u32)r * 256 + threadIdx.x;
        if (dst[r] != 0xFFFFFFFFu) P.keys_out[dst[r]] = stage[sp];
    }
}

struct PSLevel {
    const u32* idx_in; const u32* val_in; u32* idx_out; u32* val_out;
    u32* counts; const u32* blk_seg; const u32* blk_start; const u32* seg_start;
    u32 nseg, R, per_xcd; int shift;
};
__device__ __forceinline__ bool ps_row(const PSLevel& P, u32 row, size_t& base, u32& cnt) {
    const u32 blk = row / P.R;
    if (blk >= P.blk_start[P.nseg]) return false;
    const u32 s = P.blk_seg[blk];
    const u64 t = (u64)(blk - P.blk_start[s]) * P.R + row % P.R;
    const u32 s0 = P.seg_start[s], s1 = P.seg_start[s + 1];
    const u64 off = t * SS_TILE;
    base = s0; cnt = 0;
    if (off >= (u64)(s1 - s0)) return true;
    base = (size_t)s0 + off;
    const u64 left = (u64)(s1 - s0) - off;
    cnt = left < SS_TILE ? (u32)left : (u32)SS_TILE;
    return true;
}
template <int DB>
__global__ __launch_bounds__(256) void ps_count_kernel(PSLevel P, u32 rows) {
    constexpr u32 D = 1u << DB;
    __shared__ u32 hist[D];
    const u32 row = xcd_tile(blockIdx.x, P.per_xcd);
    if (row >= rows) return;
    size_t base; u32 cnt;
    if (!ps_row(P, row, base, cnt)) return;
    for (u32 i = threadIdx.x; i < D; i += 256) hist[i] = 0;
    if (cnt == 0) { for (u32 i = threadIdx.x; i < D; i += 256) P.counts[(size_t)row * D + i] = 0; return; }
    __syncthreads();
    const u32 lb = wave_id() * (64 * SS_ITEMS) + lane_id();
    const u32* ip = P.idx_in + base + lb;
    u32 kk[SS_ITEMS];
#pragma unroll
    for (int j = 0; j < SS_ITEMS; ++j) kk[j] = (lb + (u32)j * 64 < cnt) ? ip[j * 64] : 0u;
#pragma unroll
    for (int j = 0; j < SS_ITEMS; ++j) {
        const bool valid = lb + (u32)j * 64 < cnt;
        const u32 d = (kk[j] >> P.shift) & (D - 1);
        const u32 d0 = __builtin_amdgcn_readfirstlane(d);
        if (__all(valid && d == d0)) { if (lane_id() == 0) atomicAdd(&hist[d0], 64u); }
        else if (valid) atomicAdd(&hist[d], 1u);
    }
    __syncthreads();
    for (u32 i = threadIdx.x; i < D; i += 256) P.counts[(size_t)row * D + i] = hist[i];
}
template <int DB>
__global__ __launch_bounds__(256) __attribute__((amdgpu_waves_per_eu(4, 4))) void ps_scatter_kernel(PSLevel P, u32 rows) {
    constexpr u32 D = 1u << DB;
    __shared__ u32 tcnt[D];
    __shared__ u32 gbase[D];
    __shared__ u32 stage_i[SS_TILE];
    __shared__ u32 stage_v[SS_TILE];
    __shared__ u32 scan_sm[5];
    const int lane = lane_id();
    const u32 row = xcd_tile(blockIdx.x, P.per_xcd);
    if (row >= rows) return;
    size_t base; u32 cnt;
    if (!ps_row(P, row, base, cnt) || cnt == 0) return;
    for (u32 i = threadIdx.x; i < D; i += 256) tcnt[i] = 0;
    __syncthreads();
    const u32 lb = wave_id() * (64 * SS_ITEMS) + lane;
    const u32* ip = P.idx_in + base + lb;
    const u32* vp = P.val_in + base + lb;
    u32 k[SS_ITEMS], v[SS_ITEMS], ld[SS_ITEMS];
#pragma unroll
    for (int j = 0; j < SS_ITEMS; ++j) {
        const bool valid = lb + (u32)j * 64 < cnt;
        k[j] = valid ? ip[j * 64] : 0u;
        v[j] = valid ? vp[j * 64] : 0u;
    }
#pragma unroll
    for (int j = 0; j < SS_ITEMS; ++j) {
        const bool valid = lb + (u32)j * 64 < cnt;
        const u32 d = (k[j] >> P.shift) & (D - 1);
        const u32 d0 = __builtin_amdgcn_readfirstlane(d);
        u32 rank = 0;
        if (__all(valid && d == d0)) {
            if (lane == 0) rank = atomicAdd(&tcnt[d0], 64u);
            rank = __builtin_amdgcn_readfirstlane(rank) + (u32)lane;
        } else if (valid) rank = atomicAdd(&tcnt[d], 1u);
        ld[j] = rank;
    }
    __syncthreads();
    {
        const u32 t = threadIdx.x;
        u32 tot[D / 256], sum = 0;
#pragma unroll
        for (u32 q = 0; q < D / 256; ++q) { tot[q] = tcnt[t * (D / 256) + q]; sum += tot[q]; }
        u32 total;
        u32 start = block_exclusive_sum<u32, 4>(sum, scan_sm, total);
#pragma unroll
        for (u32 q = 0; q < D / 256; ++q) {
            const u32 d = t * (D / 256) + q;
            tcnt[d] = start;
            gbase[d] = P.counts[(size_t)row * D + d] - start;
            start += tot[q];
        }
    }
    __syncthreads();
#pragma unroll
    for (int j = 0; j < SS_ITEMS; ++j) {
        if (lb + (u32)j * 64 < cnt) {
            const u32 pos = ld[j] + tcnt[(k[j] >> P.shift) & (D - 1)];
            stage_i[pos] = k[j]; stage_v[pos] = v[j];
        }
    }
    __syncthreads();
#pragma unroll
    for (int r = 0; r < SS_ITEMS; ++r) {
        const u32 sp = (u32)r * 256 + threadIdx.x;
        if (sp < cnt) {
            const u32 key = stage_i[sp];
            const u32 dst = gbase[(key >> P.shift) & (D - 1)] + sp;
            P.idx_out[dst] = key;
            P.val_out[dst] = stage_v[sp];
        }
    }
}

void msd_partition_pairs_u32(Ctx& c, const u32* idx, const u32* val, size_t m, int bits, int db, u32* out_idx, u32* out_val, u32* tmp_idx, u32* tmp_val) {
    hipStream_t s = c.stream;
    const size_t mark = c.arena.mark();
    const u32 D = 1u << db;
    u32* seg_start = c.arena.get<u32>(2);
    ss_set_word_kernel<<<1, 1, 0, s>>>(seg_start, 0u);
    LAUNCH_CHECK();
    ss_set_word_kernel<<<1, 1, 0, s>>>(seg_start + 1, (u32)m);
    LAUNCH_CHECK();
    u32 nseg = 1;
    const u64 tiles = (m + SS_TILE - 1) / SS_TILE;
    for (int l = 0; l < 2; ++l) {
        u32 R = 128;
        while (R > 1 && (u64)nseg * R > tiles / 8 + 64) R >>= 1;
        const u32 blocks_ub = (u32)((tiles + R - 1) / R) + nseg;
        const u32 rows = blocks_ub * R;
        u32* nstart = c.arena.get<u32>((size_t)nseg * D + 1);
        const size_t lm = c.arena.mark();
        u32* blk_start = c.arena.get<u32>((size_t)nseg + 1);
        u32* blk_seg = c.arena.get<u32>(blocks_ub);
        u32* counts = c.arena.get<u32>((size_t)rows * D);
        u32* bs = c.arena.get<u32>((size_t)blocks_ub * D);
        ss_nblk_kernel<<<cdiv((size_t)nseg + 1, 256), 256, 0, s>>>(seg_start, nseg, R, blk_start);
        LAUNCH_CHECK();
        exclusive_sum_u32(c, blk_start, blk_start, (size_t)nseg + 1, nullptr);
        ss_blkseg_kernel<<<cdiv(nseg, 256), 256, 0, s>>>(blk_start, nseg, blk_seg);
        LAUNCH_CHECK();
        PSLevel P;
        P.idx_in = l == 0 ? idx : tmp_idx; P.val_in = l == 0 ? val : tmp_val;
        P.idx_out = l == 0 ? tmp_idx : out_idx; P.val_out = l == 0 ? tmp_val : out_val;
        P.counts = counts; P.blk_seg = blk_seg; P.blk_start = blk_start; P.seg_start = seg_start;
        P.nseg = nseg; P.R = R; P.shift = bits - db * (l + 1);
        P.per_xcd = (c.xcd_remap == 1 && rows >= 64) ? cdiv(rows, 8) : 0u;
        const u32 grid = P.per_xcd ? 8 * P.per_xcd : rows;
        {
            const int pc = c.prof_begin(K_RS_COUNT, (u64)m * 4);
            if (db == 9) ps_count_kernel<9><<<grid, 256, 0, s>>>(P, rows); else ps_count_kernel<8><<<grid, 256, 0, s>>>(P, rows);
            LAUNCH_CHECK();
            c.prof_end(pc);
        }
        {
            Ctx::ProfScope prof(c, K_SCAN, (u64)rows * D * 12);
            ss_blocksum_kernel<<<blocks_ub, 256, 0, s>>>(counts, blk_start, nseg, R, D, bs);
            LAUNCH_CHECK();
            ss_segbase_kernel<<<nseg, 1024, 0, s>>>(bs, blk_start, seg_start, D, nstart);
            LAUNCH_CHECK();
            ss_set_word_kernel<<<1, 1, 0, s>>>(nstart + (size_t)nseg * D, (u32)m);
            LAUNCH_CHECK();
            ss_apply_kernel<<<blocks_ub, 256, 0, s>>>(counts, blk_start, nseg, R, D, bs);
            LAUNCH_CHECK();
        }
        {
            const int ps = c.prof_begin(K_RS_SCATTER_U32, (u64)m * 16);
            if (db == 9) ps_scatter_kernel<9><<<grid, 256, 0, s>>>(P, rows); else ps_scatter_kernel<8><<<grid, 256, 0, s>>>(P, rows);
            LAUNCH_CHECK();
            c.prof_end(ps);
        }
        c.arena.release(lm);
        seg_start = nstart;
        nseg *= D;
    }
    c.arena.release(mark);
}

__device__ __forceinline__ u32 ss_leaf_class(const u32* __restrict__ leaf_start, u32 l, u32 small = SS_SMALL) {
    const u32 size = leaf_start[l + 1] - leaf_start[l];
    if (size <= small) return 0;
    if (l & 1u) return 2;
    return size <= SS_UNIT_MAX ? 1u : 3u;
}
__device__ __forceinline__ bool ss_unit_first(const u32* __restrict__ leaf_start, u32 l, u32 cls, u32 small = SS_SMALL) {
    if (cls == 1) return true;
    if (cls != 0) return false;
    if (l == 0) return true;
    return ss_leaf_class(leaf_start, l - 1, small) != 0 || (leaf_start[l] / small) != (leaf_start[l - 1] / small);
}
__global__ void ss_unit_flag_kernel(const u32* __restrict__ leaf_start, u32 nleaf, u32* __restrict__ flag, u32* __restrict__ large_list,
                                    u32* __restrict__ large_count, u32 large_cap, u32 small = SS_SMALL) {
    const u32 l = blockIdx.x * blockDim.x + threadIdx.x;
    if (l >= nleaf) return;
    const u32 cls = ss_leaf_class(leaf_start, l, small);
    flag[l] = ss_unit_first(leaf_start, l, cls, small) ? 1u : 0u;
    if (cls == 3) { const u32 i = atomicAdd(large_count, 1u); if (i < large_cap) large_list[i] = l; }
}
__global__ void ss_unit_fill_kernel(const u32* __restrict__ leaf_start, u32 nleaf, const u32* __restrict__ uidx, u32* __restrict__ unit_rng, u32 small = SS_SMALL) {
    const u32 l = blockIdx.x * blockDim.x + threadIdx.x;
    if (l >= nleaf) return;
    const u32 cls = ss_leaf_class(leaf_start, l, small);
    if (cls > 1) return;
    const bool first = ss_unit_first(leaf_start, l, cls, small);
    const u32 u = uidx[l] - (first ? 0u : 1u);
    if (first) unit_rng[2 * u] = leaf_start[l];
    bool last = (cls == 1) || (l + 1 == nleaf);
    if (!last) {
        const u32 c2 = ss_leaf_class(leaf_start, l + 1, small);
        last = c2 != 0 || (leaf_start[l + 1] / small) != (leaf_start[l] / small);
    }
    if (last) unit_rng[2 * u + 1] = leaf_start[l + 1];
}

constexpr int LS_NW = 8;
__device__ __forceinline__ u32 ls_rank(u32 d, bool valid, u32* mycnt, unsigned long long* M, u64 lanebit, u64 lt_mask) {
    const u64 peers = wave_match_lds(M, d, valid, lanebit);
    const u32 prefix = lds_load(&mycnt[d]);
    const u32 rank = (u32)__popcll(peers & lt_mask);
    if (valid && rank == 0) lds_store(&mycnt[d], prefix + (u32)__popcll(peers));
    return prefix + rank;
}
__device__ __forceinline__ void ls_digit_starts(u32 (*wcnt)[256], int lane) {
    uint4 c[LS_NW];
    u32 t0 = 0, t1 = 0, t2 = 0, t3 = 0;
#pragma unroll
    for (int i = 0; i < LS_NW; ++i) {
        c[i] = *(const uint4*)&wcnt[i][4 * lane];
        t0 += c[i].x; t1 += c[i].y; t2 += c[i].z; t3 += c[i].w;
    }
    const u32 sum = t0 + t1 + t2 + t3;
    u32 r0 = wave_inclusive_sum(sum) - sum;
    u32 r1 = r0 + t0, r2 = r1 + t1, r3 = r2 + t2;
#pragma unroll
    for (int i = 0; i < LS_NW; ++i) {
        *(uint4*)&wcnt[i][4 * lane] = make_uint4(r0, r1, r2, r3);
        r0 += c[i].x; r1 += c[i].y; r2 += c[i].z; r3 += c[i].w;
    }
}
template <int ROWS>
__global__ __launch_bounds__(LS_NW * 64) __attribute__((amdgpu_waves_per_eu(4, 4))) void ss_leaf_comp_kernel(u64* __restrict__ keys, u32* __restrict__ vals, const u32* __restrict__ unit_rng,
                                                                   const u32* __restrict__ list, u32 count, u32* __restrict__ d_err, u32* __restrict__ wide_list) {
    __shared__ __align__(16) u32 wcnt[LS_NW][256];
    __shared__ u64 stage[ROWS * LS_NW * 64];
    __shared__ u64 red[2][LS_NW];
    if (blockIdx.x >= count) return;
    const u32 u = list[blockIdx.x];
    const u32 a = unit_rng[2 * u], b = unit_rng[2 * u + 1];
    const u32 m = b - a;
    if (m <= 1) return;
    if (m > (u32)ROWS * LS_NW * 64) { if (threadIdx.x == 0) atomicOr(d_err, 2u); return; }
    const int lane = lane_id(), w = wave_id();
    const u32 wbase = (u32)w * ROWS * 64 + (u32)lane;
    u64 k[ROWS];
    u64 kmin = ~0ull, kmax = 0;
#pragma unroll
    for (int j = 0; j < ROWS; ++j) {
        const u32 L = wbase + (u32)j * 64;
        const bool valid = L < m;
        k[j] = valid ? keys[(size_t)a + L] : 0ull;
        if (valid) { kmin = k[j] < kmin ? k[j] : kmin; kmax = k[j] > kmax ? k[j] : kmax; }
    }
#pragma unroll
    for (int d = 32; d >= 1; d >>= 1) {
        const u64 o1 = __shfl_xor(kmin, d, 64), o2 = __shfl_xor(kmax, d, 64);
        kmin = o1 < kmin ? o1 : kmin; kmax = o2 > kmax ? o2 : kmax;
    }
    if (lane == 0) { red[0][w] = kmin; red[1][w] = kmax; }
    __syncthreads();
    kmin = red[0][0]; kmax = red[1][0];
#pragma unroll
    for (int i = 1; i < LS_NW; ++i) { kmin = red[0][i] < kmin ? red[0][i] : kmin; kmax = red[1][i] > kmax ? red[1][i] : kmax; }
    const u64 diff = kmin ^ kmax;
    if (diff == 0) return;
    const int nbits = 64 - __clzll((long long)diff);
    if (nbits + 13 > 64) { if (threadIdx.x == 0) wide_list[1 + atomicAdd(wide_list, 1u)] = u; return; }
    const u64 lt_mask = (lane == 0) ? 0ull : (~0ull >> (64 - lane));
    u32* mycnt = wcnt[w];
    u32* stage32 = (u32*)stage;
    unsigned long long* M = (unsigned long long*)stage + w * 256;
    const u64 lanebit = 1ull << lane;
    const u64 lowmask = (nbits == 64) ? ~0ull : ((1ull << nbits) - 1);
    const u64 high = kmin & ~lowmask;
#pragma unroll
    for (int j = 0; j < ROWS; ++j) k[j] = ((k[j] & lowmask) << 13) | (u64)(wbase + (u32)j * 64);
    for (int i = lane; i < 256; i += 64) mycnt[i] = 0;
    u32 loc[ROWS];
    for (int shift = 13; shift < 13 + nbits; shift += 8) {
        for (int i = lane; i < 256; i += 64) M[i] = 0;
#pragma unroll
        for (int j = 0; j < ROWS; ++j) {
            loc[j] = ls_rank((u32)(k[j] >> shift) & 255u, wbase + (u32)j * 64 < m, mycnt, M, lanebit, lt_mask);
            if ((j & 3) == 3) __builtin_amdgcn_sched_barrier(0);
        }
        __syncthreads();
        if (w == 0) ls_digit_starts(wcnt, lane);
        __syncthreads();
#pragma unroll
        for (int j = 0; j < ROWS; ++j)
            if (wbase + (u32)j * 64 < m) stage[loc[j] + mycnt[(u32)(k[j] >> shift) & 255u]] = k[j];
        for (int i = lane; i < 256; i += 64) mycnt[i] = 0;
        __syncthreads();
#pragma unroll
        for (int j = 0; j < ROWS; ++j) if (wbase + (u32)j * 64 < m) k[j] = stage[wbase + (u32)j * 64];
        __syncthreads();
    }
#pragma unroll
    for (int j = 0; j < ROWS; ++j) if (wbase + (u32)j * 64 < m) stage32[wbase + (u32)j * 64] = vals[(size_t)a + wbase + (u32)j * 64];
    __syncthreads();
#pragma unroll
    for (int j = 0; j < ROWS; ++j) {
        const u32 L = wbase + (u32)j * 64;
        if (L < m) {
            keys[(size_t)a + L] = (k[j] >> 13) | high;
            vals[(size_t)a + L] = stage32[(u32)k[j] & 8191u];
        }
    }
}

__global__ __launch_bounds__(LS_NW * 64) __attribute__((amdgpu_waves_per_eu(4, 4))) void ss_leaf_wide_kernel(u64* __restrict__ keys, u32* __restrict__ vals, const u32* __restrict__ unit_rng,
                                                                   const u32* __restrict__ wide_list, u32 count, u32* __restrict__ d_err) {
    __shared__ __align__(16) u32 wcnt[LS_NW][256];
    __shared__ u64 stage[SS_UNIT_MAX];
    if (blockIdx.x >= count) return;
    const u32 u = wide_list[1 + blockIdx.x];
    const u32 a = unit_rng[2 * u], b = unit_rng[2 * u + 1];
    const u32 m = b - a;
    if (m <= 1) return;
    if (m > SS_UNIT_MAX) { if (threadIdx.x == 0) atomicOr(d_err, 2u); return; }
    const int lane = lane_id(), w = wave_id();
    const u32 rows = (m + LS_NW * 64 - 1) / (LS_NW * 64);
    const u32 wbase = (u32)w * rows * 64 + (u32)lane;
    u64 k[SS_ITEMS];
    u32 v[SS_ITEMS];
    u32 loc[SS_ITEMS];
#pragma unroll
    for (int j = 0; j < SS_ITEMS; ++j) {
        const u32 L = wbase + (u32)j * 64;
        const bool valid = (u32)j < rows && L < m;
        k[j] = valid ? keys[(size_t)a + L] : 0ull;
        v[j] = valid ? vals[(size_t)a + L] : 0u;
    }
    const u64 lt_mask = (lane == 0) ? 0ull : (~0ull >> (64 - lane));
    u32* mycnt = wcnt[w];
    u32* stage32 = (u32*)stage;
    unsigned long long* M = (unsigned long long*)stage + w * 256;
    const u64 lanebit = 1ull << lane;
    for (int shift = 0; shift < 64; shift += 8) {
        for (int i = threadIdx.x; i < LS_NW * 256; i += LS_NW * 64) { (&wcnt[0][0])[i] = 0; stage[i] = 0; }
        __syncthreads();
#pragma unroll
        for (int j = 0; j < SS_ITEMS; ++j)
            if ((u32)j < rows) loc[j] = ls_rank((u32)(k[j] >> shift) & 255u, wbase + (u32)j * 64 < m, mycnt, M, lanebit, lt_mask);
        __syncthreads();
        if (w == 0) ls_digit_starts(wcnt, lane);
        __syncthreads();
#pragma unroll
        for (int j = 0; j < SS_ITEMS; ++j) {
            if ((u32)j < rows && wbase + (u32)j * 64 < m) {
                loc[j] += wcnt[w][(u32)(k[j] >> shift) & 255u];
                stage[loc[j]] = k[j];
            }
        }
        __syncthreads();
#pragma unroll
        for (int j = 0; j < SS_ITEMS; ++j) if ((u32)j < rows && wbase + (u32)j * 64 < m) k[j] = stage[wbase + (u32)j * 64];
        __syncthreads();
#pragma unroll
        for (int j = 0; j < SS_ITEMS; ++j) if ((u32)j < rows && wbase + (u32)j * 64 < m) stage32[loc[j]] = v[j];
        __syncthreads();
#pragma unroll
        for (int j = 0; j < SS_ITEMS; ++j) if ((u32)j < rows && wbase + (u32)j * 64 < m) v[j] = stage32[wbase + (u32)j * 64];
        __syncthreads();
    }
#pragma unroll
    for (int j = 0; j < SS_ITEMS; ++j) {
        const u32 L = wbase + (u32)j * 64;
        if ((u32)j < rows && L < m) { keys[(size_t)a + L] = k[j]; vals[(size_t)a + L] = v[j]; }
    }
}

constexpr int UC_T = 1024;
__global__ __launch_bounds__(UC_T) void ss_unit_class_kernel(const u32* __restrict__ unit_rng, const u32* __restrict__ d_nunits, u32* __restrict__ cls_count,
                                                            u32* __restrict__ cls_list, u32 cap, int wide = 0) {
    __shared__ u32 wcnt[UC_T / 64][16];
    __shared__ u32 wbase[16];
    const u32 u = blockIdx.x * blockDim.x + threadIdx.x;
    const u32 ncls = wide ? (u32)WIDE_NCLS : 4u;
    u32 c = 15u;
    if (u < *d_nunits) {
        const u32 m = unit_rng[2 * u + 1] - unit_rng[2 * u];
        if (m > 1 && m <= SS_UNIT_MAX) c = wide ? wide_class(m) : (m - 1) / 2048;
    }
    const int lane = lane_id(), w = wave_id();
    u32 below = 0;
    for (u32 q = 0; q < ncls; ++q) {
        const u64 mask = __ballot(c == q);
        if (lane == 0) wcnt[w][q] = (u32)__popcll(mask);
        if (c == q) below = (u32)__popcll(mask & ((1ull << lane) - 1));
    }
    __syncthreads();
    if (threadIdx.x < ncls) {
        const u32 q = threadIdx.x;
        u32 tot = 0;
        for (int i = 0; i < UC_T / 64; ++i) { const u32 t = wcnt[i][q]; wcnt[i][q] = tot; tot += t; }
        wbase[q] = tot ? atomicAdd(&cls_count[q], tot) : 0u;
    }
    __syncthreads();
    if (c < ncls) cls_list[(size_t)c * cap + wbase[c] + wcnt[w][c] + below] = u;
}

static u32 pow2_ceil(u64 x) { u32 p = 1; while ((u64)p < x) p <<= 1; return p; }

bool splitter_sort_applicable(size_t n) { return n >= ((size_t)1 << 20) && n < ((size_t)1 << 32); }

int splitter_sort_pairs_u64(Ctx& c, u64* keys[2], u32* vals[2], size_t n, const TextKeyGen* gen, SplitSortStats* st) {
    SplitSortStats local;
    if (!st) st = &local;
    *st = SplitSortStats();
    hipStream_t s = c.stream;
    const size_t mark = c.arena.mark();
    TextKeyGen g;
    if (gen) g = *gen; else memset(&g, 0, sizeof(g));

    int L = n <= (size_t)256 * 3072 ? 1 : ((n + 65535) / 65536 <= 4352 ? 2 : 3);
    if (c.ssort_levels >= 1 && c.ssort_levels <= 3) L = c.ssort_levels;
    u32 F[3] = { 1, 1, 1 };
    u32 os;
    {
        const u32 cap = L == 1 ? 256u : (L == 2 ? 65536u : (1u << 24));
        u32 nl = pow2_ceil((n + (L == 3 ? 2047 : 3071)) / (L == 3 ? 2048 : 3072));
        if (nl > cap) nl = cap;
        if (nl < (2u << (L - 1))) nl = 2u << (L - 1);
        const u32 lastF = nl > 256 ? 256u : (L == 1 ? nl : nl >> (L - 1));
        F[L - 1] = lastF;
        u32 rest = nl / lastF;
        if (L == 2) F[0] = rest;
        if (L == 3) { F[0] = 1; while ((u64)F[0] * F[0] < rest) F[0] <<= 1; F[1] = rest / F[0]; if (F[1] < 2) { F[1] = 2; } }
        const u64 avg = (n + nl - 1) / nl;
        os = avg > 3072 ? 64 : (avg > 2304 ? 32 : 16);
    }
    const u32 NLr = F[0] * F[1] * F[2];
    const u32 NS = NLr - 1;
    const u32 S = os * NLr;
    st->levels = (u32)L; st->range_leaves = NLr; st->samples = S;

    u64* sp = c.arena.get<u64>((size_t)NS + 1);
    {
        const size_t m2 = c.arena.mark();
        u64* sk[2] = { c.arena.get<u64>(S), c.arena.get<u64>(S) };
        u32* sv[2] = { c.arena.get<u32>(S), c.arena.get<u32>(S) };
        if (gen) ss_sample_kernel<true><<<cdiv(S, 256), 256, 0, s>>>(nullptr, g, n, S, sk[0], sv[0]);
        else ss_sample_kernel<false><<<cdiv(S, 256), 256, 0, s>>>(keys[0], g, n, S, sk[0], sv[0]);
        LAUNCH_CHECK();
        const int x = radix_sort_pairs_u64(c, sk, sv, S, 0, 64);
        ss_pick_kernel<<<cdiv((size_t)NS + 1, 256), 256, 0, s>>>(sk[x], NS, os, sp);
        LAUNCH_CHECK();
        c.arena.release(m2);
    }

    u16* digits = c.arena.get<u16>(align_up(n, SS_TILE) + SS_TILE);
    u32* seg_start = c.arena.get<u32>(2);
    ss_set_word_kernel<<<1, 1, 0, s>>>(seg_start, 0u);
    LAUNCH_CHECK();
    ss_set_word_kernel<<<1, 1, 0, s>>>(seg_start + 1, (u32)n);
    LAUNCH_CHECK();
    u32 nseg = 1;
    int cur = gen ? -1 : 0;
    for (int l = 0; l < L; ++l) {
        const bool last = (l == L - 1);
        const bool gl = gen && l == 0;
        const u32 D = last ? 2 * F[l] : F[l];
        u32 stride = 1;
        for (int q = l + 1; q < L; ++q) stride *= F[q];
        const u64 tiles = (n + SS_TILE - 1) / SS_TILE;
        u32 R = 128;
        while (R > 1 && (u64)nseg * R > tiles / 8 + 64) R >>= 1;
        const u32 blocks_ub = (u32)((tiles + R - 1) / R) + nseg;
        const u32 rows = blocks_ub * R;
        u32* nstart = c.arena.get<u32>((size_t)nseg * D + 1);
        const size_t lm2 = c.arena.mark();
        u32* blk_start = c.arena.get<u32>((size_t)nseg + 1);
        u32* blk_seg = c.arena.get<u32>(blocks_ub);
        u32* counts = c.arena.get<u32>((size_t)rows * D);
        u32* bs = c.arena.get<u32>((size_t)blocks_ub * D);
        ss_nblk_kernel<<<cdiv((size_t)nseg + 1, 256), 256, 0, s>>>(seg_start, nseg, R, blk_start);
        LAUNCH_CHECK();
        exclusive_sum_u32(c, blk_start, blk_start, (size_t)nseg + 1, nullptr);
        ss_blkseg_kernel<<<cdiv(nseg, 256), 256, 0, s>>>(blk_start, nseg, blk_seg);
        LAUNCH_CHECK();
        SSLevel P;
        P.keys_in = cur >= 0 ? keys[cur] : nullptr; P.vals_in = cur >= 0 ? vals[cur] : nullptr;
        const int nxt = cur < 0 ? 0 : (cur ^ 1);
        P.keys_out = keys[nxt]; P.vals_out = vals[nxt];
        P.digits = digits;
        P.counts = counts; P.blk_seg = blk_seg; P.blk_start = blk_start; P.seg_start = seg_start; P.sp = sp;
        P.nseg = nseg; P.F = F[l]; P.stride = stride; P.R = R; P.D = D;
        P.per_xcd = (c.xcd_remap == 1 && rows >= 64) ? cdiv(rows, 8) : 0u;
        const u32 grid = P.per_xcd ? 8 * P.per_xcd : rows;
        {
            const int pc = c.prof_begin(K_RS_COUNT, (u64)n * (gl ? 1 : 8));
            if (gl && last) ss_count_kernel<true, true><<<grid, 256, 0, s>>>(P, g, rows);
            else if (gl) ss_count_kernel<true, false><<<grid, 256, 0, s>>>(P, g, rows);
            else if (last) ss_count_kernel<false, true><<<grid, 256, 0, s>>>(P, g, rows);
            else ss_count_kernel<false, false><<<grid, 256, 0, s>>>(P, g, rows);
            LAUNCH_CHECK();
            c.prof_end(pc);
        }
        {
            Ctx::ProfScope prof(c, K_SCAN, (u64)rows * D * 12);
            ss_blocksum_kernel<<<blocks_ub, 256, 0, s>>>(counts, blk_start, nseg, R, D, bs);
            LAUNCH_CHECK();
            ss_segbase_kernel<<<nseg, 1024, 0, s>>>(bs, blk_start, seg_start, D, nstart);
            LAUNCH_CHECK();
            ss_set_word_kernel<<<1, 1, 0, s>>>(nstart + (size_t)nseg * D, (u32)n);
            LAUNCH_CHECK();
            ss_apply_kernel<<<blocks_ub, 256, 0, s>>>(counts, blk_start, nseg, R, D, bs);
            LAUNCH_CHECK();
        }
        {
            const int ps = c.prof_begin(K_RS_SCATTER_U64, (u64)n * (gl ? 13 : 24));
            if (gl && last) ss_scatter_stable_kernel<true, true><<<grid, 256, 0, s>>>(P, g, rows);
            else if (gl) ss_scatter_kernel<true, false><<<grid, 256, 0, s>>>(P, g, rows);
            else if (last) ss_scatter_stable_kernel<false, true><<<grid, 256, 0, s>>>(P, g, rows);
            else ss_scatter_kernel<false, false><<<grid, 256, 0, s>>>(P, g, rows);
            LAUNCH_CHECK();
            c.prof_end(ps);
        }
        c.arena.release(lm2);
        seg_start = nstart;
        nseg = nseg * D;
        cur = nxt;
    }
    const u32 nleaf = nseg;
    const u32* leaf_start = seg_start;

    constexpr u32 LARGE_CAP = 1024;
    u32* flag = c.arena.get<u32>((size_t)nleaf + 1);
    u32* unit_rng = c.arena.get<u32>(2 * ((size_t)nleaf + 1));
    u32* large = c.arena.get<u32>(LARGE_CAP + 6);
    u32* wide_list = c.arena.get<u32>((size_t)nleaf + 2);
    u32* cls_list = c.arena.get<u32>(4 * ((size_t)nleaf + 1));
    HIP_TRY(hipMemsetAsync(large, 0, 6 * sizeof(u32), s));
    HIP_TRY(hipMemsetAsync(wide_list, 0, sizeof(u32), s));
    ss_unit_flag_kernel<<<cdiv(nleaf, 256), 256, 0, s>>>(leaf_start, nleaf, flag, large + 6, large, LARGE_CAP);
    LAUNCH_CHECK();
    exclusive_sum_u32(c, flag, flag, nleaf, large + 1);
    ss_unit_fill_kernel<<<cdiv(nleaf, 256), 256, 0, s>>>(leaf_start, nleaf, flag, unit_rng);
    LAUNCH_CHECK();
    ss_unit_class_kernel<<<cdiv((size_t)nleaf + 1, UC_T), UC_T, 0, s>>>(unit_rng, large + 1, large + 2, cls_list, nleaf + 1);
    LAUNCH_CHECK();
    u32 hc[6];
    c.read_n(large, hc, 6);
    const u32 nlarge = hc[0], nunits = hc[1];
    st->units = nunits; st->large_leaves = nlarge;
    {
        Ctx::ProfScope prof(c, K_SS_LEAF, (u64)n * 24);
        u64* K = keys[cur]; u32* V = vals[cur];
        const u32 cap = nleaf + 1;
        if (hc[2]) { ss_leaf_comp_kernel<4><<<hc[2], LS_NW * 64, 0, s>>>(K, V, unit_rng, cls_list, hc[2], c.d_err, wide_list); LAUNCH_CHECK(); }
        if (hc[3]) { ss_leaf_comp_kernel<8><<<hc[3], LS_NW * 64, 0, s>>>(K, V, unit_rng, cls_list + (size_t)cap, hc[3], c.d_err, wide_list); LAUNCH_CHECK(); }
        if (hc[4]) { ss_leaf_comp_kernel<12><<<hc[4], LS_NW * 64, 0, s>>>(K, V, unit_rng, cls_list + 2 * (size_t)cap, hc[4], c.d_err, wide_list); LAUNCH_CHECK(); }
        if (hc[5]) { ss_leaf_comp_kernel<16><<<hc[5], LS_NW * 64, 0, s>>>(K, V, unit_rng, cls_list + 3 * (size_t)cap, hc[5], c.d_err, wide_list); LAUNCH_CHECK(); }
        const u32 nwide = (hc[2] | hc[3] | hc[4] | hc[5]) ? c.read(wide_list) : 0u;
        if (nwide) {
            ss_leaf_wide_kernel<<<nwide, LS_NW * 64, 0, s>>>(K, V, unit_rng, wide_list, nwide, c.d_err);
            LAUNCH_CHECK();
            st->wide_units = nwide;
        }
    }
    if (nlarge) {
        if (nlarge > LARGE_CAP) throw HipError{hipErrorUnknown, "splitter sort: too many oversized leaves", (int)__LINE__};
        std::vector<u32> ll(nlarge), ls((size_t)nleaf + 1);
        HIP_TRY(hipMemcpyAsync(ll.data(), large + 6, nlarge * sizeof(u32), hipMemcpyDeviceToHost, s));
        HIP_TRY(hipMemcpyAsync(ls.data(), leaf_start, ((size_t)nleaf + 1) * sizeof(u32), hipMemcpyDeviceToHost, s));
        HIP_TRY(hipStreamSynchronize(s));
        for (u32 i = 0; i < nlarge; ++i) {
            const size_t a = ls[ll[i]], b = ls[ll[i] + 1];
            u64* kk[2] = { keys[cur] + a, keys[cur ^ 1] + a };
            u32* vv[2] = { vals[cur] + a, vals[cur ^ 1] + a };
            const int y = radix_sort_pairs_u64(c, kk, vv, b - a, 0, 64);
            if (y == 1) {
                HIP_TRY(hipMemcpyAsync(kk[0], kk[1], (b - a) * sizeof(u64), hipMemcpyDeviceToDevice, s));
                HIP_TRY(hipMemcpyAsync(vv[0], vv[1], (b - a) * sizeof(u32), hipMemcpyDeviceToDevice, s));
            }
            st->large_pairs += b - a;
        }
    }
    c.arena.release(mark);
    return cur;
}

void ss_level_tables(Ctx& c, const u32* seg_start, u32 nseg, size_t n, u32 D, SegTables& T) {
    hipStream_t s = c.stream;
    const u64 tiles = (n + SS_TILE - 1) / SS_TILE;
    u32 R = 128;
    while (R > 1 && (u64)nseg * R > tiles / 8 + 64) R >>= 1;
    T.R = R;
    T.blocks_ub = (u32)((tiles + R - 1) / R) + nseg;
    T.rows = T.blocks_ub * R;
    T.blk_start = c.arena.get<u32>((size_t)nseg + 1);
    T.blk_seg = c.arena.get<u32>(T.blocks_ub);
    T.counts = c.arena.get<u32>((size_t)T.rows * D);
    T.bs = c.arena.get<u32>((size_t)T.blocks_ub * D);
    ss_nblk_kernel<<<cdiv((size_t)nseg + 1, 256), 256, 0, s>>>(seg_start, nseg, R, T.blk_start);
    LAUNCH_CHECK();
    exclusive_sum_u32(c, T.blk_start, T.blk_start, (size_t)nseg + 1, nullptr);
    ss_blkseg_kernel<<<cdiv(nseg, 256), 256, 0, s>>>(T.blk_start, nseg, T.blk_seg);
    LAUNCH_CHECK();
}
void ss_level_offsets(Ctx& c, const SegTables& T, const u32* seg_start, u32 nseg, u32 D, u32* nstart, size_t n) {
    hipStream_t s = c.stream;
    Ctx::ProfScope prof(c, K_SCAN, (u64)T.rows * D * 12);
    ss_blocksum_kernel<<<T.blocks_ub, 256, 0, s>>>(T.counts, T.blk_start, nseg, T.R, D, T.bs);
    LAUNCH_CHECK();
    ss_segbase_kernel<<<nseg, 1024, 0, s>>>(T.bs, T.blk_start, seg_start, D, nstart);
    LAUNCH_CHECK();
    ss_set_word_kernel<<<1, 1, 0, s>>>(nstart + (size_t)nseg * D, (u32)n);
    LAUNCH_CHECK();
    ss_apply_kernel<<<T.blocks_ub, 256, 0, s>>>(T.counts, T.blk_start, nseg, T.R, D, T.bs);
    LAUNCH_CHECK();
}
void ss_level_offsets_sub(Ctx& c, const SegTables& T, u32 nsub, const u32* blk_super, const u32* out_start, u32 nsuper, u32 D, u32* nstart, size_t n) {
    hipStream_t s = c.stream;
    Ctx::ProfScope prof(c, K_SCAN, (u64)T.rows * D * 12);
    ss_blocksum_kernel<<<T.blocks_ub, 256, 0, s>>>(T.counts, T.blk_start, nsub, T.R, D, T.bs);
    LAUNCH_CHECK();
    ss_segbase_kernel<<<nsuper, 1024, 0, s>>>(T.bs, blk_super, out_start, D, nstart);
    LAUNCH_CHECK();
    ss_set_word_kernel<<<1, 1, 0, s>>>(nstart + (size_t)nsuper * D, (u32)n);
    LAUNCH_CHECK();
    ss_apply_kernel<<<T.blocks_ub, 256, 0, s>>>(T.counts, T.blk_start, nsub, T.R, D, T.bs);
    LAUNCH_CHECK();
}
u32* ss_first_segment(Ctx& c, size_t n) {
    u32* seg_start = c.arena.get<u32>(2);
    ss_set_word_kernel<<<1, 1, 0, c.stream>>>(seg_start, 0u);
    LAUNCH_CHECK();
    ss_set_word_kernel<<<1, 1, 0, c.stream>>>(seg_start + 1, (u32)n);
    LAUNCH_CHECK();
    return seg_start;
}
void ss_build_units(Ctx& c, const u32* leaf_start, u32 nleaf, UnitTables& U, u32 small) {
    if (small == 0) small = SS_SMALL;
    hipStream_t s = c.stream;
    constexpr u32 LARGE_CAP = 1024;
    U.large_cap = LARGE_CAP;
    u32* flag = c.arena.get<u32>((size_t)nleaf + 1);
    U.unit_rng = c.arena.get<u32>(2 * ((size_t)nleaf + 1));
    U.large = c.arena.get<u32>(LARGE_CAP + 6);
    U.cls_list = c.arena.get<u32>((U.wide_classes ? (size_t)WIDE_NCLS : 4) * ((size_t)nleaf + 1));
    u32* wcnt = U.wide_classes ? c.arena.get<u32>(16) : nullptr;
    if (wcnt) HIP_TRY(hipMemsetAsync(wcnt, 0, 16 * sizeof(u32), s));
    U.cap = nleaf + 1;
    HIP_TRY(hipMemsetAsync(U.large, 0, 6 * sizeof(u32), s));
    ss_unit_flag_kernel<<<cdiv(nleaf, 256), 256, 0, s>>>(leaf_start, nleaf, flag, U.large + 6, U.large, LARGE_CAP, small);
    LAUNCH_CHECK();
    exclusive_sum_u32(c, flag, flag, nleaf, U.large + 1);
    ss_unit_fill_kernel<<<cdiv(nleaf, 256), 256, 0, s>>>(leaf_start, nleaf, flag, U.unit_rng, small);
    LAUNCH_CHECK();
    ss_unit_class_kernel<<<cdiv((size_t)nleaf + 1, UC_T), UC_T, 0, s>>>(U.unit_rng, U.large + 1, wcnt ? wcnt : U.large + 2, U.cls_list, nleaf + 1, U.wide_classes);
    LAUNCH_CHECK();
    c.read_n(U.large, U.hc, 6);
    if (wcnt) c.read_n(wcnt, U.whc, 16);
}
void ss_fanouts(Ctx& c, size_t n, int& L, u32 F[3], u32& os, u32 leaf3, int wide2) {
    L = n <= (size_t)256 * 3072 ? 1 : ((n + 65535) / 65536 <= 3584 ? 2 : 3);
    if (c.ssort_levels >= 1 && c.ssort_levels <= 3) L = c.ssort_levels;
    F[0] = F[1] = F[2] = 1;
    if (leaf3 == 0) leaf3 = 2048;
    if ((wide2 == 1 && L == 3) || wide2 == 2) {
        u32 nl2 = pow2_ceil((n + leaf3 - 1) / leaf3);
        if (nl2 <= (1u << 20) && nl2 >= 2048u) {
            L = 2;
            F[1] = 1024u;
            F[0] = nl2 / F[1];
            const u64 avg2 = (n + nl2 - 1) / nl2;
            os = avg2 > 3072 ? 64 : (avg2 > 2304 ? 32 : 16);
            return;
        }
    }
    const u32 cap = L == 1 ? 256u : (L == 2 ? 65536u : (1u << 24));
    u32 nl = pow2_ceil((n + (L == 3 ? leaf3 - 1 : 3071)) / (L == 3 ? leaf3 : 3072));
    if (nl > cap) nl = cap;
    if (nl < (2u << (L - 1))) nl = 2u << (L - 1);
    const u32 lastF = nl > 256 ? 256u : (L == 1 ? nl : nl >> (L - 1));
    F[L - 1] = lastF;
    u32 rest = nl / lastF;
    if (L == 2) F[0] = rest;
    if (L == 3) { F[0] = 1; while ((u64)F[0] * F[0] < rest) F[0] <<= 1; F[1] = rest / F[0]; if (F[1] < 2) { F[1] = 2; } }
    const u64 avg = (n + nl - 1) / nl;
    os = avg > 3072 ? 64 : (avg > 2304 ? 32 : 16);
}

}
```

tudocomp_amd/csrc/wsort.hip:

```cpp
#include "prim.hpp"

#include <vector>
#include <algorithm>
#include <stdlib.h>

namespace tdc {

constexpr int WS_TILE = 4096;
constexpr int WS_ITEMS = 16;
constexpr int WS_HALO = 64;
#ifndef TDC_WS_PEEL
#define TDC_WS_PEEL 0
#endif
#ifndef TDC_WS_CMAX
#define TDC_WS_CMAX 64
#endif
constexpr u32 WS_CMAX = TDC_WS_CMAX;
constexpr u32 WS_WAVE_MAX = 1024;

struct WSLevel {
    const u64* k1_in; const u64* k2_in; const u32* v_in;
    u64* k1_out; u64* k2_out; u32* v_out;
    u32* counts;
    const u32* blk_seg; const u32* blk_start; const u32* seg_start;
// ... 1077 lines not shown
        if (ll > 0) {
            const u64 x = key ^ prev;
            A.flags[(size_t)a + ll] = x ? 1 : 0;
            if (x && !PAIRS) A.lcp[(size_t)a + ll] = (u8)(((64u + (u32)__builtin_clzll(x)) * A.inv) >> 16);
        }
    }
}

template <int CAPR, bool PAIRS>
__global__ __launch_bounds__(256) void ws_run_wave_kernel(WLeaf A, const u32* __restrict__ list, u32 count) {
    constexpr int WR_ROWS = CAPR / 64;
    __shared__ u64 sk[4][CAPR];
    __shared__ u16 sid[4][CAPR];
    __shared__ __align__(16) u32 cnt[4][256];
    __shared__ u64 mt[4][256];
    const int lane = lane_id(), w = wave_id();
    const u32 r = blockIdx.x * 4 + (u32)w;
    if (r >= count) return;
    const u32 u = list[r];
    const u32 a = A.unit_rng[2 * u], m = (A.unit_rng[2 * u + 1] & 0x7FFFFFFFu) - a;
    if (m <= 1 || m > (u32)CAPR) return;
    u64* W = A.k2 + a;
    u64* K = sk[w]; u16* S = sid[w]; u32* mycnt = cnt[w];
    unsigned long long* M = (unsigned long long*)mt[w];
    const int rows = (int)((m + 63) >> 6);
    u64 k[WR_ROWS];
    u32 id[WR_ROWS];
    u64 orv = 0, andv = ~0ull;
#pragma unroll
    for (int j = 0; j < WR_ROWS; ++j) {
        const u32 L = (u32)j * 64 + (u32)lane;
        k[j] = (j < rows && L < m) ? W[L] : 0ull;
        id[j] = L;
        if (j < rows && L < m) { orv |= k[j]; andv &= k[j]; }
    }
#pragma unroll
    for (int d = 32; d >= 1; d >>= 1) { orv |= __shfl_xor(orv, d, 64); andv &= __shfl_xor(andv, d, 64); }
    const u64 diff = orv ^ andv;
    for (int i = lane; i < 256; i += 64) { mycnt[i] = 0; M[i] = 0; }
    __builtin_amdgcn_wave_barrier();
    if (diff) {
        const int hi = 64 - __builtin_clzll(diff), lo = __builtin_ctzll(diff);
        const u64 lanebit = 1ull << lane;
        const u64 lt_mask = (lane == 0) ? 0ull : (~0ull >> (64 - lane));
        for (int shift = lo; shift < hi; shift += 8) {
            if (((diff >> shift) & 255ull) == 0) continue;
            u32 loc[WR_ROWS];
#pragma unroll
            for (int j = 0; j < WR_ROWS; ++j)
                if (j < rows) loc[j] = wl_rank((u32)(k[j] >> shift) & 255u, (u32)j * 64 + (u32)lane < m, mycnt, M, lanebit, lt_mask);
            __builtin_amdgcn_wave_barrier();
            {
                const uint4 cc = *(const uint4*)&mycnt[4 * lane];
                const u32 sum = cc.x + cc.y + cc.z + cc.w;
                const u32 r0 = wave_inclusive_sum(sum) - sum;
                *(uint4*)&mycnt[4 * lane] = make_uint4(r0, r0 + cc.x, r0 + cc.x + cc.y, r0 + cc.x + cc.y + cc.z);
            }
            __builtin_amdgcn_wave_barrier();
#pragma unroll
            for (int j = 0; j < WR_ROWS; ++j) {
                if (j < rows && (u32)j * 64 + (u32)lane < m) {
                    const u32 p = loc[j] + lds_load(&mycnt[(u32)(k[j] >> shift) & 255u]);
                    lds_store(&K[p], k[j]); lds_store(&S[p], (u16)id[j]);
                }
            }
            __builtin_amdgcn_wave_barrier();
            for (int i = lane; i < 256; i += 64) mycnt[i] = 0;
#pragma unroll
            for (int j = 0; j < WR_ROWS; ++j) {
                const u32 L = (u32)j * 64 + (u32)lane;
                if (j < rows && L < m) { k[j] = lds_load(&K[L]); id[j] = (u32)lds_load(&S[L]); }
            }
            __builtin_amdgcn_wave_barrier();
        }
    }
#pragma unroll
    for (int j = 0; j < WR_ROWS; ++j) {
        const u32 L = (u32)j * 64 + (u32)lane;
        if (j < rows && L < m && L > 0) {
            const u64 x = diff ? (k[j] ^ lds_load(&K[L - 1])) : 0ull;
            A.flags[(size_t)a + L] = x ? 1 : 0;
            if (x && !PAIRS) A.lcp[(size_t)a + L] = (u8)(((64u + (u32)__builtin_clzll(x)) * A.inv) >> 16);
        }
    }
    if (!diff) return;
    __builtin_amdgcn_wave_barrier();
    u32* P = (u32*)K;
    u32 vr[WR_ROWS];
#pragma unroll
    for (int j = 0; j < WR_ROWS; ++j) { const u32 L = (u32)j * 64 + (u32)lane; vr[j] = (j < rows && L < m) ? A.v[(size_t)a + L] : 0u; }
    __builtin_amdgcn_wave_barrier();
#pragma unroll
    for (int j = 0; j < WR_ROWS; ++j) { const u32 L = (u32)j * 64 + (u32)lane; if (j < rows && L < m) lds_store(&P[L], vr[j]); }
    __builtin_amdgcn_wave_barrier();
#pragma unroll
    for (int j = 0; j < WR_ROWS; ++j) {
        const u32 L = (u32)j * 64 + (u32)lane;
        if (j < rows && L < m) {
            A.v[(size_t)a + L] = lds_load(&P[id[j]]);
            if (PAIRS) W[L] = k[j];
        }
    }
}

template <int KW>
__global__ __launch_bounds__(256) void ws_fix_kernel(const u32* __restrict__ leaf_start, u32 nleaf, const u32* __restrict__ v, WKeyGen g,
                                                     u8* __restrict__ flags, u8* __restrict__ lcp) {
    __shared__ u8 code[256];
    code[threadIdx.x] = g.code[threadIdx.x];
    __syncthreads();
    const u32 l = blockIdx.x * 256 + threadIdx.x;
    if (l >= nleaf) return;
    const u32 s = leaf_start[l];
    if (s == leaf_start[l + 1]) return;
    flags[s] = 1;
    if (s == 0) { lcp[0] = 0; return; }
    const size_t pa = v[s - 1], pb = v[s];
    u32 t = 0;
    while (t < (u32)g.s) {
        u64 wa = 0, wb = 0;
        if (pa + t + 8 <= g.n) __builtin_memcpy(&wa, g.text + pa + t, 8);
        else for (int e = 0; e < 8; ++e) if (pa + t + e < g.n) wa |= (u64)g.text[pa + t + e] << (8 * e);
        if (pb + t + 8 <= g.n) __builtin_memcpy(&wb, g.text + pb + t, 8);
        else for (int e = 0; e < 8; ++e) if (pb + t + e < g.n) wb |= (u64)g.text[pb + t + e] << (8 * e);
        bool stop = false;
        for (int e = 0; e < 8 && t < (u32)g.s; ++e, ++t) {
            const u32 ca = (pa + t < g.n) ? code[(wa >> (8 * e)) & 0xFFu] : 0u, cb = (pb + t < g.n) ? code[(wb >> (8 * e)) & 0xFFu] : 0u;
            if (ca != cb) { stop = true; break; }
        }
        if (stop) break;
    }
    lcp[s] = (u8)t;
}
template <int KW>
__global__ void ws_range_flags_kernel(const u64* __restrict__ k1, const u64* __restrict__ k2, u32 a, u32 bnd, u32 inv, u8* __restrict__ flags,
                                      u8* __restrict__ lcp) {
    const u32 i = a + 1 + blockIdx.x * blockDim.x + threadIdx.x;
    if (i >= bnd) return;
    const u64 x1 = k1[i] ^ k1[i - 1];
    const u64 x2 = KW == 2 ? (k2[i] ^ k2[i - 1]) : 0ull;
    const bool h = x1 != 0 || x2 != 0;
    flags[i] = h ? 1 : 0;
    if (h && lcp) lcp[i] = (u8)(((x1 ? (u32)__builtin_clzll(x1) : 64u + (u32)__builtin_clzll(x2)) * inv) >> 16);
}

__global__ __launch_bounds__(1024) void ws_sub_tables_kernel(const u32* __restrict__ nstart_all, u32 F0, u32 nch, u32* __restrict__ seg_begin,
                                                              u32* __restrict__ seg_end, u32* __restrict__ out_start) {
    __shared__ u32 tot[1024];
    const u32 b = threadIdx.x;
    u32 t = 0;
    if (b < F0) {
        for (u32 q = 0; q < nch; ++q) {
            const u32 lo = nstart_all[(size_t)q * (F0 + 1) + b], hi = nstart_all[(size_t)q * (F0 + 1) + b + 1];
            seg_begin[b * nch + q] = lo; seg_end[b * nch + q] = hi;
            t += hi - lo;
        }
    }
    tot[b] = t;
    __syncthreads();
    if (b == 0) {
        u32 run = 0;
        for (u32 i = 0; i < F0; ++i) { out_start[i] = run; run += tot[i]; }
        out_start[F0] = run;
    }
}
__global__ void ws_sub_nblk_kernel(const u32* __restrict__ seg_begin, const u32* __restrict__ seg_end, u32 nsub, u32 R, u32* __restrict__ nblk) {
    const u32 sidx = blockIdx.x * blockDim.x + threadIdx.x;
    if (sidx > nsub) return;
    if (sidx == nsub) { nblk[sidx] = 0; return; }
    const u64 size = seg_end[sidx] - seg_begin[sidx];
    nblk[sidx] = (u32)((size + (u64)WS_TILE * R - 1) / ((u64)WS_TILE * R));
}
__global__ void ws_blkseg_kernel(const u32* __restrict__ blk_start, u32 nseg, u32* __restrict__ blk_seg) {
    const u32 sidx = blockIdx.x * blockDim.x + threadIdx.x;
    if (sidx >= nseg) return;
    for (u32 b = blk_start[sidx]; b < blk_start[sidx + 1]; ++b) blk_seg[b] = sidx;
}
__global__ void ws_blk_super_kernel(const u32* __restrict__ blk_start, u32 nsuper, u32 sub, u32* __restrict__ blk_super) {
    const u32 S = blockIdx.x * blockDim.x + threadIdx.x;
    if (S <= nsuper) blk_super[S] = blk_start[(size_t)S * sub];
}
__global__ void ws_set2_kernel(u32* p, u32 a, u32 b) { p[0] = a; p[1] = b; }

struct WPreHist { const u32* counts[32]; const u32* blk[32]; u32 R[32]; u32 nch, chunks; };
__global__ __launch_bounds__(64) void ws_pre_hist_kernel(WPreHist H, const u32* __restrict__ blk_start, const u32* __restrict__ blk_seg, u32 nsub, u32 R, u32 D,
                                                         u32 rows, u32* __restrict__ counts) {
    const u32 row = blockIdx.x;
    if (row >= rows) return;
    const u32 blk = row / R;
    if (blk >= blk_start[nsub]) return;
    const u32 s = blk_seg[blk];
    const u32 q = s % H.nch, b = s / H.nch;
    if (q >= H.chunks) return;
    const u32 t = (blk - blk_start[s]) * R + row % R;
    const u32 lb0 = H.blk[q][b], lb1 = H.blk[q][b + 1], Rq = H.R[q];
    const bool in = t < (lb1 - lb0) * Rq;
    const u32* src = H.counts[q] + ((size_t)lb0 * Rq + t) * D;
    for (u32 d = threadIdx.x; d < D; d += 64) counts[(size_t)row * D + d] = in ? src[d] : 0u;
}

void wsort_make_keygen(const Ctx& c, const u8* text, size_t n, u32 sigma, const u8* code, int& KW, WKeyGen& g) {
    const int b = (int)bits_for(sigma > 1 ? sigma - 1 : 1);
    const int per_word = 64 / b;
    KW = c.wsort_kw ? c.wsort_kw : (per_word < 16 ? 2 : 1);
    g.text = text; g.n = n; g.b = b;
    g.s = (64 * KW) / b; if (g.s > 64) g.s = 64;
    if (c.wsort_syms > 0 && g.s > c.wsort_syms) g.s = c.wsort_syms;
    g.pad = 64 * KW - g.s * b;
    g.inv = (65536u + (u32)b - 1) / (u32)b;
    memcpy(g.code, code, 256);
}
bool wsort_applicable(const Ctx& c, size_t n) { return c.wsort && n >= c.wsort_min && n < ((size_t)1 << 32); }
int wsort_result_index(Ctx& c, size_t n) {
    int L; u32 F[3], os;
    ss_fanouts(c, n, L, F, os, (u32)c.wsort_leaf, c.wsort_two);
    if (c.wsort_order == 1 && L == 3) std::swap(F[0], F[2]);
    return (L - 1) & 1;
}

namespace {
struct WPlan { int L; u32 F[3]; u32 os, NLr, NS, S; };

template <int KW, bool GEN>
void ws_splitters(Ctx& c, const WPlan& pl, const u64* k1, const u64* k2, const WKeyGen& g, size_t n, u64* sp1, u64* sp2) {
    hipStream_t s = c.stream;
    const size_t m2 = c.arena.mark();
    const u32 S = pl.S;
    u64* a1[2] = { c.arena.get<u64>(S), c.arena.get<u64>(S) };
    u64* a2[2] = { nullptr, nullptr };
    if (KW == 2) { a2[0] = c.arena.get<u64>(S); a2[1] = c.arena.get<u64>(S); }
    u32* iv[2] = { c.arena.get<u32>(S), c.arena.get<u32>(S) };
    ws_sample_kernel<KW, GEN><<<cdiv(S, 256), 256, 0, s>>>(k1, k2, g, n, S, a1[0], a2[0], iv[0]);
    LAUNCH_CHECK();
    if (KW == 1) {
        const int x = radix_sort_pairs_u64(c, a1, iv, S, 0, 64);
        ws_pick_kernel<<<cdiv((size_t)pl.NS + 1, 256), 256, 0, s>>>(a1[x], nullptr, pl.NS, pl.os, sp1, nullptr);
        LAUNCH_CHECK();
    } else {
        ws_lsd_sort_wide(c, a1, a2, nullptr, S, 64);
        ws_pick_kernel<<<cdiv((size_t)pl.NS + 1, 256), 256, 0, s>>>(a1[1], a2[1], pl.NS, pl.os, sp1, sp2);
        LAUNCH_CHECK();
    }
    c.arena.release(m2);
}

template <int KW, bool GEN, bool PAIRS>
int ws_sort_impl(Ctx& c, const WKeyGen* gen, u64* K1[2], u64* K2[2], u32* V[2], size_t n, int k1_bits, u8* flags, u8* lcp8, WSortStats* st,
                 const WPre* pre = nullptr, u32* v_final = nullptr) {
    hipStream_t s = c.stream;
    const size_t mark = c.arena.mark();
    WKeyGen g;
    if (gen) g = *gen; else memset(&g, 0, sizeof(g));
    WPlan pl;
    u64* sp1; u64* sp2;
    if (pre) {
        pl.L = pre->L; pl.F[0] = pre->F[0]; pl.F[1] = pre->F[1]; pl.F[2] = pre->F[2]; pl.os = pre->os;
        pl.NLr = pre->NLr; pl.NS = pre->NS; pl.S = pre->S;
        sp1 = pre->sp1; sp2 = pre->sp2;
    } else {
        ss_fanouts(c, n, pl.L, pl.F, pl.os, (u32)c.wsort_leaf, c.wsort_two);
        if (c.wsort_order == 1 && pl.L == 3) std::swap(pl.F[0], pl.F[2]);
        pl.NLr = pl.F[0] * pl.F[1] * pl.F[2]; pl.NS = pl.NLr - 1; pl.S = pl.os * pl.NLr;
        sp1 = c.arena.get<u64>((size_t)pl.NS + 1);
        sp2 = KW == 2 ? c.arena.get<u64>((size_t)pl.NS + 1) : nullptr;
        ws_splitters<KW, GEN>(c, pl, K1[0], KW == 2 ? K2[0] : nullptr, g, n, sp1, sp2);
    }
    const int L = pl.L;
    st->levels = (u32)L; st->range_leaves = pl.NLr; st->samples = pl.S; st->kw = KW;

    unsigned long long* d_nonheads = (unsigned long long*)c.arena.get<u64>(1);
    HIP_TRY(hipMemsetAsync(d_nonheads, 0, sizeof(u64), s));
    if (PAIRS) flags = c.arena.get<u8>(n + 8);
    HIP_TRY(hipMemsetAsync(flags, 0, n, s));

    u16* digits = pre ? pre->digits : c.arena.get<u16>(align_up(n, WS_TILE) + WS_TILE);
    const u32* seg_start = pre ? nullptr : ss_first_segment(c, n);
    u32 nseg = 1;
    int cur = GEN ? -1 : 0;
    u32* Vlast = nullptr;
    if (pre) {
        const int l = 1;
        const bool last = (l == L - 1);
        const u32 F0 = pl.F[0], nch = pre->nchunks, nsub = F0 * nch;
        const u32 D = last ? 2 * pl.F[l] : pl.F[l];
        u32 stride = 1;
        for (int q = l + 1; q < L; ++q) stride *= pl.F[q];
        u32* nstart = c.arena.get<u32>((size_t)F0 * D + 1);
        const size_t lm2 = c.arena.mark();
        u32* seg_begin = c.arena.get<u32>(nsub + 1);
        u32* seg_end = c.arena.get<u32>(nsub + 1);
        u32* out_start = c.arena.get<u32>(F0 + 1);
        ws_sub_tables_kernel<<<1, 1024, 0, s>>>(pre->nstart_all, F0, nch, seg_begin, seg_end, out_start);
        LAUNCH_CHECK();
        SegTables Tb;
        {
            const u64 tiles = (n + WS_TILE - 1) / WS_TILE;
            u32 R = 128;
            while (R > 1 && (u64)nsub * R > tiles / 8 + 64) R >>= 1;
            Tb.R = R; Tb.blocks_ub = (u32)((tiles + R - 1) / R) + nsub; Tb.rows = Tb.blocks_ub * R;
            Tb.blk_start = c.arena.get<u32>((size_t)nsub + 1);
            Tb.blk_seg = c.arena.get<u32>(Tb.blocks_ub);
            Tb.counts = c.arena.get<u32>((size_t)Tb.rows * D);
            Tb.bs = c.arena.get<u32>((size_t)Tb.blocks_ub * D);
            ws_sub_nblk_kernel<<<cdiv((size_t)nsub + 1, 256), 256, 0, s>>>(seg_begin, seg_end, nsub, R, Tb.blk_start);
            LAUNCH_CHECK();
            exclusive_sum_u32(c, Tb.blk_start, Tb.blk_start, (size_t)nsub + 1, nullptr);
            ws_blkseg_kernel<<<cdiv(nsub, 256), 256, 0, s>>>(Tb.blk_start, nsub, Tb.blk_seg);
            LAUNCH_CHECK();
        }
        u32* blk_super = c.arena.get<u32>(F0 + 1);
        ws_blk_super_kernel<<<cdiv(F0 + 1, 256), 256, 0, s>>>(Tb.blk_start, F0, nch, blk_super);
        LAUNCH_CHECK();
        WSLevel P;
        P.k1_in = pre->K1[0]; P.k2_in = KW == 2 ? pre->K2[0] : nullptr; P.v_in = pre->V[0];
        Vlast = last ? v_final : pre->V[1];
        P.k1_out = pre->K1[1]; P.k2_out = KW == 2 ? pre->K2[1] : nullptr; P.v_out = Vlast;
        P.digits = digits;
        P.counts = Tb.counts; P.blk_seg = Tb.blk_seg; P.blk_start = Tb.blk_start; P.seg_start = seg_begin; P.seg_end = seg_end; P.sub = nch;
        P.sp1 = sp1; P.sp2 = sp2;
        P.nseg = nsub; P.F = pl.F[l]; P.stride = stride; P.R = Tb.R; P.D = D;
        P.pre_digits = pre->dig2 ? pre->dig2_chunks : 0u;
        P.pre_counts = (pre->dig2 && c.wsort_prehist) ? pre->dig2_chunks : 0u;
        P.gen_off = 0; P.gen_len = n;
        const u32 rows = Tb.rows;
        P.per_xcd = (c.xcd_remap == 1 && rows >= 64) ? cdiv(rows, 8) : 0u;
        const u32 grid = P.per_xcd ? 8 * P.per_xcd : rows;
        if (P.pre_counts) {
            WPreHist H;
            for (u32 q = 0; q < 32; ++q) { H.counts[q] = pre->dig2_counts[q]; H.blk[q] = pre->dig2_blk[q]; H.R[q] = pre->dig2_R[q]; }
            H.nch = nch; H.chunks = P.pre_counts;
            ws_pre_hist_kernel<<<Tb.rows, 64, 0, s>>>(H, Tb.blk_start, Tb.blk_seg, nsub, Tb.R, D, Tb.rows, Tb.counts);
            LAUNCH_CHECK();
        }
        {
            const int pc = c.prof_begin(K_RS_COUNT, (u64)n * 8 * KW);
            if (last) { if (P.F > 256) ws_count_kernel<KW, false, true, 1024><<<grid, 256, 0, s>>>(P, g, rows); else if (P.F > 64) ws_count_kernel<KW, false, true, 256><<<grid, 256, 0, s>>>(P, g, rows); else ws_count_kernel<KW, false, true, 64><<<grid, 256, 0, s>>>(P, g, rows); }
            else { if (P.F > 256) ws_count_kernel<KW, false, false, 1024><<<grid, 256, 0, s>>>(P, g, rows); else if (P.F > 64) ws_count_kernel<KW, false, false, 256><<<grid, 256, 0, s>>>(P, g, rows); else ws_count_kernel<KW, false, false, 64><<<grid, 256, 0, s>>>(P, g, rows); }
            LAUNCH_CHECK();
            c.prof_end(pc);
        }
        ss_level_offsets_sub(c, Tb, nsub, blk_super, out_start, F0, D, nstart, n);
        {
            const int ps = c.prof_begin(K_RS_SCATTER_U64, (u64)n * (2 * (4 + 8 * KW) + 2));
            if (last) { if (P.F > 256) ws_scatter_kernel<KW, false, true, 1024><<<grid, 256, 0, s>>>(P, g, rows); else ws_scatter_kernel<KW, false, true, 256><<<grid, 256, 0, s>>>(P, g, rows); }
            else { if (P.F > 256) ws_scatter_kernel<KW, false, false, 1024><<<grid, 256, 0, s>>>(P, g, rows); else ws_scatter_kernel<KW, false, false, 256><<<grid, 256, 0, s>>>(P, g, rows); }
            LAUNCH_CHECK();
            c.prof_end(ps);
        }
        c.arena.release(lm2);
        seg_start = nstart;
        nseg = F0 * D;
        cur = 1;
        K1 = const_cast<u64**>(pre->K1); K2 = const_cast<u64**>(pre->K2); V = const_cast<u32**>(pre->V);
    }
    for (int l = pre ? 2 : 0; l < L; ++l) {
        const bool last = (l == L - 1);
        const bool gl = GEN && l == 0;
        const u32 D = last ? 2 * pl.F[l] : pl.F[l];
        u32 stride = 1;
        for (int q = l + 1; q < L; ++q) stride *= pl.F[q];
        u32* nstart = c.arena.get<u32>((size_t)nseg * D + 1);
        const size_t lm2 = c.arena.mark();
        SegTables Tb;
        ss_level_tables(c, seg_start, nseg, n, D, Tb);
        WSLevel P;
        P.k1_in = cur >= 0 ? K1[cur] : nullptr; P.k2_in = (cur >= 0 && KW == 2) ? K2[cur] : nullptr;
        P.v_in = pre ? Vlast : (cur >= 0 ? V[cur] : nullptr);
        const int nxt = cur < 0 ? 0 : (cur ^ 1);
        P.k1_out = K1[nxt]; P.k2_out = KW == 2 ? K2[nxt] : nullptr;
        P.v_out = (pre && last) ? v_final : V[nxt];
        Vlast = P.v_out;
        P.digits = digits;
        P.counts = Tb.counts; P.blk_seg = Tb.blk_seg; P.blk_start = Tb.blk_start; P.seg_start = seg_start; P.sp1 = sp1; P.sp2 = sp2;
        P.seg_end = seg_start + 1; P.sub = 1;
        P.nseg = nseg; P.F = pl.F[l]; P.stride = stride; P.R = Tb.R; P.D = D;
        P.gen_off = 0; P.gen_len = n;
        const u32 rows = Tb.rows;
        P.per_xcd = (c.xcd_remap == 1 && rows >= 64) ? cdiv(rows, 8) : 0u;
        const u32 grid = P.per_xcd ? 8 * P.per_xcd : rows;
        {
            const int pc = c.prof_begin(K_RS_COUNT, (u64)n * (gl ? 1 : 8 * KW));
            if (gl && last) { if (P.F > 256) ws_count_kernel<KW, GEN, true, 1024><<<grid, 256, 0, s>>>(P, g, rows); else ws_count_kernel<KW, GEN, true, 256><<<grid, 256, 0, s>>>(P, g, rows); }
            else if (gl) { if (P.F > 256) ws_count_kernel<KW, GEN, false, 1024><<<grid, 256, 0, s>>>(P, g, rows); else ws_count_kernel<KW, GEN, false, 256><<<grid, 256, 0, s>>>(P, g, rows); }
            else if (last) { if (P.F > 256) ws_count_kernel<KW, false, true, 1024><<<grid, 256, 0, s>>>(P, g, rows); else if (P.F > 64) ws_count_kernel<KW, false, true, 256><<<grid, 256, 0, s>>>(P, g, rows); else ws_count_kernel<KW, false, true, 64><<<grid, 256, 0, s>>>(P, g, rows); }
            else { if (P.F > 256) ws_count_kernel<KW, false, false, 1024><<<grid, 256, 0, s>>>(P, g, rows); else if (P.F > 64) ws_count_kernel<KW, false, false, 256><<<grid, 256, 0, s>>>(P, g, rows); else ws_count_kernel<KW, false, false, 64><<<grid, 256, 0, s>>>(P, g, rows); }
            LAUNCH_CHECK();
            c.prof_end(pc);
        }
        ss_level_offsets(c, Tb, seg_start, nseg, D, nstart, n);
        {
            const int ps = c.prof_begin(K_RS_SCATTER_U64, (u64)n * (gl ? 3 + 4 + 8 * KW : 2 * (4 + 8 * KW) + 2));
            if (gl && last) { if (P.F > 256) ws_scatter_kernel<KW, GEN, true, 1024><<<grid, 256, 0, s>>>(P, g, rows); else ws_scatter_kernel<KW, GEN, true, 256><<<grid, 256, 0, s>>>(P, g, rows); }
            else if (gl) { if (P.F > 256) ws_scatter_kernel<KW, GEN, false, 1024><<<grid, 256, 0, s>>>(P, g, rows); else ws_scatter_kernel<KW, GEN, false, 256><<<grid, 256, 0, s>>>(P, g, rows); }
            else if (last) { if (P.F > 256) ws_scatter_kernel<KW, false, true, 1024><<<grid, 256, 0, s>>>(P, g, rows); else ws_scatter_kernel<KW, false, true, 256><<<grid, 256, 0, s>>>(P, g, rows); }
            else { if (P.F > 256) ws_scatter_kernel<KW, false, false, 1024><<<grid, 256, 0, s>>>(P, g, rows); else ws_scatter_kernel<KW, false, false, 256><<<grid, 256, 0, s>>>(P, g, rows); }
            LAUNCH_CHECK();
            c.prof_end(ps);
        }
        c.arena.release(lm2);
        seg_start = nstart;
        nseg = nseg * D;
        cur = nxt;
    }
    const u32 nleaf = nseg;
    const u32* leaf_start = seg_start;

    UnitTables U;
    U.wide_classes = 1;
    ss_build_units(c, leaf_start, nleaf, U, (u32)c.wsort_pack);
    const u32 nlarge = U.hc[0];
    st->units = U.hc[1]; st->large_leaves = nlarge;
    WLeaf A;
    A.k1 = K1[cur]; A.k2 = KW == 2 ? K2[cur] : nullptr; A.v = Vlast; A.unit_rng = U.unit_rng; A.flags = flags; A.lcp = lcp8;
    A.d_err = c.d_err; A.inv = g.b ? (65536u + (u32)g.b - 1) / (u32)g.b : 65536u;
    A.cmax = c.wsort_small ? 1u : (c.wsort_cmax < 1 ? 1u : (c.wsort_cmax > (int)WS_CMAX ? WS_CMAX : (u32)c.wsort_cmax));
    {
        const u32* cur_rng = U.unit_rng;
        const u32* cur_cls = U.cls_list;
        size_t cur_cap = U.cap;
        constexpr int NB = WIDE_NCLS;
        u32 cur_cnt[NB];
        for (int q = 0; q < NB; ++q) cur_cnt[q] = U.whc[q];
        u32 wave_cnt[4] = { 0, 0, 0, 0 };
        u64 wave_recs = 0;
        const u32* wave_list = nullptr;
        const u32 ediv = A.cmax + 1;
        const u32 ecap2 = (u32)(n / ediv + 2);
        u32* e_rng[2] = { c.arena.get<u32>(2 * (size_t)ecap2), c.arena.get<u32>(2 * (size_t)ecap2) };
        u32* e_cls[2] = { c.arena.get<u32>(EC_NCLS * (size_t)ecap2), c.arena.get<u32>(EC_NCLS * (size_t)ecap2) };
        u32* lc = c.arena.get<u32>(64);
        for (int stage = 0; stage < 8; ++stage) {
            if (wave_cnt[0] | wave_cnt[1] | wave_cnt[2] | wave_cnt[3]) {
                Ctx::ProfScope prof(c, K_WS_RUN, wave_recs * 18);
                A.unit_rng = cur_rng;
                const u32* l0 = wave_list, *l1 = wave_list + cur_cap, *l2 = wave_list + 2 * cur_cap, *l3 = wave_list + 3 * cur_cap;
                const bool fork = c.wsort_run_streams && c.aux_stream && (wave_cnt[0] + wave_cnt[1] + wave_cnt[2] + wave_cnt[3]) >= 4096;
                hipStream_t sl = fork ? c.copy_stream : s, sw = fork ? c.aux_stream : s;
                if (fork) { c.wait_for(sl, s); c.wait_for(sw, s); }
                if (wave_cnt[3]) { ws_run_wave_kernel<1024, PAIRS><<<cdiv(wave_cnt[3], 4), 256, 0, s>>>(A, l3, wave_cnt[3]); LAUNCH_CHECK(); }
                if (wave_cnt[2]) { ws_run_wave_kernel<256, PAIRS><<<cdiv(wave_cnt[2], 4), 256, 0, sw>>>(A, l2, wave_cnt[2]); LAUNCH_CHECK(); }
                if (wave_cnt[0]) { ws_run_lane_kernel<32, PAIRS><<<cdiv(wave_cnt[0], 8), 256, 0, sl>>>(A, l0, wave_cnt[0]); LAUNCH_CHECK(); }
                if (wave_cnt[1]) { ws_run_lane_kernel<64, PAIRS><<<cdiv(wave_cnt[1], 4), 256, 0, sl>>>(A, l1, wave_cnt[1]); LAUNCH_CHECK(); }
                if (fork) { c.wait_for(s, sl); c.wait_for(s, sw); }
                st->wave_runs += wave_cnt[0] + wave_cnt[1] + wave_cnt[2] + wave_cnt[3];
                wave_cnt[0] = wave_cnt[1] = wave_cnt[2] = wave_cnt[3] = 0;
            }
            { u32 any = 0; for (int q = 0; q < NB; ++q) any |= cur_cnt[q]; if (!any) break; }
            if (stage == 7) throw HipError{hipErrorUnknown, "wide splitter sort: leaf stages did not converge", (int)__LINE__};
            const size_t lm3 = c.arena.mark();
            u32* rl = c.arena.get<u32>(NB * cur_cap);
            u32* tl = c.arena.get<u32>(NB * cur_cap);
            HIP_TRY(hipMemsetAsync(lc, 0, 64 * sizeof(u32), s));
            A.unit_rng = cur_rng;
            HIP_TRY(hipMemsetAsync(e_rng[stage & 1], 0, 2 * (size_t)ecap2 * sizeof(u32), s));
            const WEmit E = { e_rng[stage & 1], ediv };
            const WEmit EA = { c.wsort_fuse ? E.rng : nullptr, ediv };
            const int pa = c.prof_begin(K_WS_LEAF_SORT, stage == 0 ? (u64)n * (4 + 8 * KW + 6) : 0);
            for (int q = 0; q < NB; ++q) {
                const u32 cnt = cur_cnt[q];
                if (!cnt) continue;
                const WLists Q = { rl + q * cur_cap, tl + q * cur_cap, lc + 2 * q };
                const u32* lst = cur_cls + q * cur_cap;
                switch (q) {
                case 0: ws_leaf_sort_kernel<KW, 4, 4, PAIRS><<<cnt, 4 * 64, 0, s>>>(A, lst, cnt, Q, EA); break;
                case 1: ws_leaf_sort_kernel<KW, 5, 4, PAIRS><<<cnt, 4 * 64, 0, s>>>(A, lst, cnt, Q, EA); break;
                case 2: ws_leaf_sort_kernel<KW, 6, 4, PAIRS><<<cnt, 4 * 64, 0, s>>>(A, lst, cnt, Q, EA); break;
                case 3: ws_leaf_sort_kernel<KW, 7, 4, PAIRS><<<cnt, 4 * 64, 0, s>>>(A, lst, cnt, Q, EA); break;
                case 4: ws_leaf_sort_kernel<KW, 8, 4, PAIRS><<<cnt, 4 * 64, 0, s>>>(A, lst, cnt, Q, EA); break;
                case 5: ws_leaf_sort_kernel<KW, 5, 8, PAIRS><<<cnt, 8 * 64, 0, s>>>(A, lst, cnt, Q, EA); break;
                case 6: ws_leaf_sort_kernel<KW, 6, 8, PAIRS><<<cnt, 8 * 64, 0, s>>>(A, lst, cnt, Q, EA); break;
                case 7: ws_leaf_sort_kernel<KW, 7, 8, PAIRS><<<cnt, 8 * 64, 0, s>>>(A, lst, cnt, Q, EA); break;
                case 8: ws_leaf_sort_kernel<KW, 8, 8, PAIRS><<<cnt, 8 * 64, 0, s>>>(A, lst, cnt, Q, EA); break;
                default: ws_leaf_sort_kernel<KW, 16, 8, PAIRS><<<cnt, 8 * 64, 0, s>>>(A, lst, cnt, Q, EA); break;
                }
                LAUNCH_CHECK();
            }
            c.prof_end(pa);
            u32 hl[2 * NB];
            c.read_n(lc, hl, 2 * NB);
            const int pb = c.prof_begin(K_WS_LEAF_COUNT, stage == 0 ? (u64)n * (8 + 4 + 1 + 4 + 2) : 0);
            const WEmit noE = { nullptr, 1 };
            auto count_pass = [&](int q, const u32* lst, u32 cnt, u32 mask, u32 val, const WCount& R, const WEmit& Em) {
                if (!cnt) return;
                switch (q) {
                case 0: ws_leaf_count_kernel<4, 4, PAIRS><<<cnt, 4 * 64, 0, s>>>(A, lst, cnt, mask, val, R, Em); break;
                case 1: ws_leaf_count_kernel<5, 4, PAIRS><<<cnt, 4 * 64, 0, s>>>(A, lst, cnt, mask, val, R, Em); break;
                case 2: ws_leaf_count_kernel<6, 4, PAIRS><<<cnt, 4 * 64, 0, s>>>(A, lst, cnt, mask, val, R, Em); break;
                case 3: ws_leaf_count_kernel<7, 4, PAIRS><<<cnt, 4 * 64, 0, s>>>(A, lst, cnt, mask, val, R, Em); break;
                case 4: ws_leaf_count_kernel<8, 4, PAIRS><<<cnt, 4 * 64, 0, s>>>(A, lst, cnt, mask, val, R, Em); break;
                case 5: ws_leaf_count_kernel<5, 8, PAIRS><<<cnt, 8 * 64, 0, s>>>(A, lst, cnt, mask, val, R, Em); break;
                case 6: ws_leaf_count_kernel<6, 8, PAIRS><<<cnt, 8 * 64, 0, s>>>(A, lst, cnt, mask, val, R, Em); break;
                case 7: ws_leaf_count_kernel<7, 8, PAIRS><<<cnt, 8 * 64, 0, s>>>(A, lst, cnt, mask, val, R, Em); break;
                case 8: ws_leaf_count_kernel<8, 8, PAIRS><<<cnt, 8 * 64, 0, s>>>(A, lst, cnt, mask, val, R, Em); break;
                default: ws_leaf_count_kernel<16, 8, PAIRS><<<cnt, 8 * 64, 0, s>>>(A, lst, cnt, mask, val, R, Em); break;
                }
                LAUNCH_CHECK();
            };
            for (int q = 0; q < NB; ++q) {
                const u32 nt = hl[2 * q + 1], nr = hl[2 * q];
                if (nt) {
                    st->trunc_units += nt;
                    const WCount t1 = { A.k1, KW == 2 ? A.k2 : nullptr, 0u };
                    count_pass(q, tl + q * cur_cap, nt, 0x80000000u, 0u, t1, E);
                    if (KW == 2) {
                        const WCount t2 = { A.k2, nullptr, 64u };
                        count_pass(q, tl + q * cur_cap, nt, 0x80000000u, 0x80000000u, t2, E);
                        count_pass(q, tl + q * cur_cap, nt, 0x80000000u, 0u, t2, noE);
                    }
                }
                if (KW == 2 && nr) {
                    st->refined_units += nr;
                    const WCount r2 = { A.k2, nullptr, 64u };
                    count_pass(q, rl + q * cur_cap, nr, 0u, 0u, r2, E);
                }
            }
            c.prof_end(pb);
            ws_emit_compact_kernel<<<cdiv(ecap2, EC_TILE), 256, 0, s>>>(e_rng[stage & 1], ecap2, e_cls[stage & 1], ecap2, lc + 2 * NB);
            LAUNCH_CHECK();
            u32 he[2 * EC_NCLS];
            c.read_n(lc + 2 * NB, he, 2 * EC_NCLS);
            if (c.wsort_log) {
                fprintf(stderr, "[wsort] n=%zu stage %d: units", n, stage);
                for (int q = 0; q < NB; ++q) fprintf(stderr, " %u", cur_cnt[q]);
                fprintf(stderr, " | r/t lists");
                for (int q = 0; q < NB; ++q) fprintf(stderr, " %u/%u", hl[2 * q], hl[2 * q + 1]);
                fprintf(stderr, " | handed on: lane %u %u wave %u %u block", he[0], he[1], he[2], he[3]);
                for (int q = 0; q < NB; ++q) fprintf(stderr, " %u", he[4 + q]);
                fprintf(stderr, "\n");
            }
            c.arena.release(lm3);
            for (int q = 0; q < EC_NCLS; ++q) st->longrun_units += he[q];
            cur_rng = e_rng[stage & 1]; cur_cls = e_cls[stage & 1] + 4 * (size_t)ecap2; cur_cap = ecap2;
            wave_list = e_cls[stage & 1];
            for (int q = 0; q < 4; ++q) wave_cnt[q] = he[q];
            wave_recs = (u64)he[EC_NCLS] + he[EC_NCLS + 1] + he[EC_NCLS + 2] + he[EC_NCLS + 3];
            for (int q = 0; q < NB; ++q) cur_cnt[q] = he[4 + q];
            st->leaf_stages = (u32)stage + 1;
        }
    }
    if (nlarge) {
        if (nlarge > U.large_cap) throw HipError{hipErrorUnknown, "wide splitter sort: too many oversized leaves", (int)__LINE__};
        std::vector<u32> ll(nlarge), ls((size_t)nleaf + 1);
        HIP_TRY(hipMemcpyAsync(ll.data(), U.large + 6, nlarge * sizeof(u32), hipMemcpyDeviceToHost, s));
        HIP_TRY(hipMemcpyAsync(ls.data(), leaf_start, ((size_t)nleaf + 1) * sizeof(u32), hipMemcpyDeviceToHost, s));
        HIP_TRY(hipStreamSynchronize(s));
        for (u32 i = 0; i < nlarge; ++i) {
            const size_t a = ls[ll[i]], b = ls[ll[i] + 1];
            u64* kk1[2] = { K1[cur] + a, K1[cur ^ 1] + a };
            u64* kk2[2] = { KW == 2 ? K2[cur] + a : nullptr, KW == 2 ? K2[cur ^ 1] + a : nullptr };
            u32* vv[2] = { Vlast + a, V[cur ^ 1] + a };
            ws_lsd_sort_wide(c, kk1, KW == 2 ? kk2 : nullptr, vv, b - a, 64);
            HIP_TRY(hipMemcpyAsync(kk1[0], kk1[1], (b - a) * sizeof(u64), hipMemcpyDeviceToDevice, s));
            if (KW == 2) HIP_TRY(hipMemcpyAsync(kk2[0], kk2[1], (b - a) * sizeof(u64), hipMemcpyDeviceToDevice, s));
            HIP_TRY(hipMemcpyAsync(vv[0], vv[1], (b - a) * sizeof(u32), hipMemcpyDeviceToDevice, s));
            if (!PAIRS) {
                ws_range_flags_kernel<KW><<<cdiv(b - a, 256), 256, 0, s>>>(kk1[0], kk2[0], 0u, (u32)(b - a), A.inv, flags + a, lcp8 + a);
                LAUNCH_CHECK();
            }
            st->large_pairs += b - a;
        }
    }
    if (!PAIRS) {
        ws_fix_kernel<KW><<<cdiv(nleaf, 256), 256, 0, s>>>(leaf_start, nleaf, Vlast, g, flags, lcp8);
        LAUNCH_CHECK();
        if (c.wsort_count_nonheads) {
            { unsigned gq = cdiv(n, 256 * 16); if (gq > 4096) gq = 4096; ws_count_flags_kernel<<<gq, 256, 0, s>>>(flags, n, d_nonheads); }
            LAUNCH_CHECK();
            u64 nh = 0;
            c.read_n((const u64*)d_nonheads, &nh, 1);
            st->nonheads = nh;
        }
    }
#ifdef TDC_WL_PROF
    if (!PAIRS) {
        unsigned long long hp[16];
        HIP_TRY(hipStreamSynchronize(s));
        HIP_TRY(hipMemcpyFromSymbol(hp, HIP_SYMBOL(wl_prof), sizeof(hp)));
        fprintf(stderr, "[wl_prof] wgs %llu records %llu passes %llu | ticks: load %llu lsd %llu heads %llu pos %llu k2 %llu count %llu fin %llu nofuse %llu\n", hp[15], hp[14], hp[13],
                hp[0], hp[1], hp[2], hp[3], hp[4], hp[5], hp[6], hp[7]);
        memset(hp, 0, sizeof(hp));
        HIP_TRY(hipMemcpyToSymbol(HIP_SYMBOL(wl_prof), hp, sizeof(hp)));
    }
#endif
    c.arena.release(mark);
    return cur;
}
}

int wsort_suffixes(Ctx& c, int KW, const WKeyGen& g, u64* K1[2], u64* K2[2], u32* V[2], size_t n, u8* flags, u8* lcp8, WSortStats* st) {
    WSortStats local;
    if (!st) st = &local;
    *st = WSortStats();
    if (KW == 2) return ws_sort_impl<2, true, false>(c, &g, K1, K2, V, n, 64, flags, lcp8, st);
    return ws_sort_impl<1, true, false>(c, &g, K1, K2, V, n, 64, flags, lcp8, st);
}

void wsort_suffixes_pre(Ctx& c, const WPre& P, u32* v_final, u8* flags, u8* lcp8, WSortStats* st) {
    WSortStats local;
    if (!st) st = &local;
    *st = WSortStats();
    u64* K1[2] = { P.K1[0], P.K1[1] }; u64* K2[2] = { P.K2[0], P.K2[1] }; u32* V[2] = { P.V[0], P.V[1] };
    if (P.KW == 2) (void)ws_sort_impl<2, true, false>(c, &P.g, K1, K2, V, P.n, 64, flags, lcp8, st, &P, v_final);
    else (void)ws_sort_impl<1, true, false>(c, &P.g, K1, K2, V, P.n, 64, flags, lcp8, st, &P, v_final);
}

bool wsort_pre_begin(Ctx& c, WPre& P, const u8* text, size_t n, const size_t* chunk_off, u32 nchunks, const u32* hist0) {
// ... 366 lines not shown
```

Baseline: 8687 MB/s.

## Parallelize segmented radix offset scan and pair count tiles in fused sort

Replaces the per-segment blocksum/segbase/apply offset pipeline with a wider scheme. A vectorized multi-row blocksum is followed by a chunked cross-block segmented scan with carry tables and a vectorized apply pass, so the scan no longer runs one 1024-thread block per segment. Small segment counts now build their block tables in a single kernel, and the first segment is set in one launch. The fused-sort count and scatter kernels can also run on double-size tiles with 512 threads, so count and scatter rows line up one-to-one. This adds more kernels and arena space for chunk sums, and brings a risk of correctness errors at segment and chunk boundaries.

```diff
diff --git a/tudocomp_amd/csrc/api_ctx.hip b/tudocomp_amd/csrc/api_ctx.hip
--- a/tudocomp_amd/csrc/api_ctx.hip
+++ b/tudocomp_amd/csrc/api_ctx.hip
@@ -131,6 +131,8 @@
 const OptionDef FOLD_OPTIONS[] = {
     { "fused_cand",       [](Ctx& c, long v) { c.fused_cand = v != 0; } },
     { "sel_tile_counts",  [](Ctx& c, long v) { c.sel_tile_counts = v != 0; } },
+    { "level_wide",       [](Ctx& c, long v) { c.level_wide = v != 0; } },
+    { "fs_count_pair",    [](Ctx& c, long v) { c.fs_count_pair = v != 0; } },
 };
 constexpr size_t NFOLD = sizeof(FOLD_OPTIONS) / sizeof(FOLD_OPTIONS[0]);
 const OptionDef* find_option(const char* name) {
diff --git a/tudocomp_amd/csrc/common.hpp b/tudocomp_amd/csrc/common.hpp
--- a/tudocomp_amd/csrc/common.hpp
+++ b/tudocomp_amd/csrc/common.hpp
@@ -140,6 +140,8 @@
     int enc_early = 1;
     int fused_cand = 1;
     int sel_tile_counts = 1;
+    int level_wide = 1;
+    int fs_count_pair = 1;
     int fs_pair = 1;
     int small_big = 1;
     int small_pipeline = 1;
diff --git a/tudocomp_amd/csrc/fused.hip b/tudocomp_amd/csrc/fused.hip
--- a/tudocomp_amd/csrc/fused.hip
+++ b/tudocomp_amd/csrc/fused.hip
@@ -14,6 +14,7 @@
     u32* idx_out; void* rp_out; u8* lcp_out;
     u32* counts; const u32* blk_seg; const u32* blk_start; const u32* seg_start;
     u32 nseg, R, per_xcd; int shift;
+    u32 tile;
     int lsh;
 };
 __device__ __forceinline__ bool fs_row(const FSLevel& P, u32 row, size_t& base, u32& cnt) {
@@ -22,25 +23,26 @@
     const u32 s = P.blk_seg[blk];
     const u64 t = (u64)(blk - P.blk_start[s]) * P.R + row % P.R;
     const u32 s0 = P.seg_start[s], s1 = P.seg_start[s + 1];
-    const u64 off = t * FS_TILE;
+    const u64 off = t * P.tile;
     base = s0; cnt = 0;
     if (off >= (u64)(s1 - s0)) return true;
     base = (size_t)s0 + off;
     const u64 left = (u64)(s1 - s0) - off;
-    cnt = left < FS_TILE ? (u32)left : (u32)FS_TILE;
+    cnt = left < P.tile ? (u32)left : P.tile;
     return true;
 }
 
-template <int DB>
-__global__ __launch_bounds__(256) void fs_count_kernel(FSLevel P, u32 rows) {
+template <int DB, int PAIR>
+__global__ __launch_bounds__(256 * PAIR) void fs_count_kernel(FSLevel P, u32 rows) {
     constexpr u32 D = 1u << DB;
+    constexpr u32 NT = 256 * PAIR;
     __shared__ u32 hist[D];
     const u32 row = xcd_tile(blockIdx.x, P.per_xcd);
     if (row >= rows) return;
     size_t base; u32 cnt;
     if (!fs_row(P, row, base, cnt)) return;
-    for (u32 i = threadIdx.x; i < D; i += 256) hist[i] = 0;
-    if (cnt == 0) { for (u32 i = threadIdx.x; i < D; i += 256) P.counts[(size_t)row * D + i] = 0; return; }
+    for (u32 i = threadIdx.x; i < D; i += NT) hist[i] = 0;
+    if (cnt == 0) { for (u32 i = threadIdx.x; i < D; i += NT) P.counts[(size_t)row * D + i] = 0; return; }
     __syncthreads();
     const u32 lb = wave_id() * (64 * FS_ITEMS) + lane_id();
     const u32* ip = P.idx_in + base + lb;
@@ -56,7 +58,7 @@
         else if (valid) atomicAdd(&hist[d], 1u);
     }
     __syncthreads();
-    for (u32 i = threadIdx.x; i < D; i += 256) P.counts[(size_t)row * D + i] = hist[i];
+    for (u32 i = threadIdx.x; i < D; i += NT) P.counts[(size_t)row * D + i] = hist[i];
 }
 
 #ifndef TDC_FS_WPE
@@ -72,11 +74,12 @@
     __shared__ __align__(16) u64 stage[TILE];
     __shared__ u32 scan_sm[NT / 64 + 1];
     const int lane = lane_id();
-    const u32 row = xcd_tile(blockIdx.x, P.per_xcd) * PAIR;
+    const bool whole = PAIR == 2 && P.tile == TILE;
+    const u32 row = xcd_tile(blockIdx.x, P.per_xcd) * (whole ? 1u : (u32)PAIR);
     if (row >= rows) return;
     size_t base; u32 cnt;
     if (!fs_row(P, row, base, cnt) || cnt == 0) return;
-    if (PAIR == 2 && row + 1 < rows) {
+    if (PAIR == 2 && !whole && row + 1 < rows) {
         size_t base2; u32 cnt2;
         if (fs_row(P, row + 1, base2, cnt2) && cnt2) cnt += cnt2;
     }
@@ -327,9 +330,11 @@
     for (int l = 0; l < 2; ++l) {
         u32* nstart = c.arena.get<u32>((size_t)nseg * D + 1);
         const size_t lm = c.arena.mark();
+        const bool whole = c.fs_pair && c.fs_count_pair;
         SegTables Tb;
-        ss_level_tables(c, seg_start, nseg, m, D, Tb);
+        ss_level_tables(c, seg_start, nseg, m, D, Tb, whole ? 2 * FS_TILE : FS_TILE);
         FSLevel P;
+        P.tile = whole ? 2 * FS_TILE : FS_TILE;
         if (l == 0) { P.idx_in = sa + 1; P.rp_in = nullptr; P.prev_in = sa; P.lcp_in = lcp8 + 1; }
         else { P.idx_in = idx[0]; P.rp_in = rp[0]; P.prev_in = nullptr; P.lcp_in = nullptr; }
         P.idx_out = idx[l]; P.rp_out = rp[l]; P.lcp_out = nullptr;
@@ -341,16 +346,17 @@
         const u32 grid = P.per_xcd ? 8 * P.per_xcd : rows;
         {
             const int pc = c.prof_begin(K_RS_COUNT, (u64)m * 4);
-            if (db == 9) fs_count_kernel<9><<<grid, 256, 0, s>>>(P, rows); else fs_count_kernel<8><<<grid, 256, 0, s>>>(P, rows);
+            if (whole) { if (db == 9) fs_count_kernel<9, 2><<<grid, 512, 0, s>>>(P, rows); else fs_count_kernel<8, 2><<<grid, 512, 0, s>>>(P, rows); }
+            else { if (db == 9) fs_count_kernel<9, 1><<<grid, 256, 0, s>>>(P, rows); else fs_count_kernel<8, 1><<<grid, 256, 0, s>>>(P, rows); }
             LAUNCH_CHECK();
             c.prof_end(pc);
         }
         ss_level_offsets(c, Tb, seg_start, nseg, D, nstart, m);
         {
             const int ps = c.prof_begin(K_RS_SCATTER_U32, (u64)m * (wp ? (l == 0 ? 5 + 12 : 24) : (l == 0 ? 5 + 8 : 16)));
-            const bool pair = (Tb.R % 2) == 0 && c.fs_pair;
+            const bool pair = whole || ((Tb.R % 2) == 0 && c.fs_pair);
             FSLevel P2 = P;
-            const u32 groups = pair ? (rows + 1) / 2 : rows;
+            const u32 groups = (pair && !whole) ? (rows + 1) / 2 : rows;
             P2.per_xcd = (c.xcd_remap == 1 && groups >= 64) ? cdiv(groups, 8) : 0u;
             const u32 grid2 = P2.per_xcd ? 8 * P2.per_xcd : groups;
             auto launch = [&](auto wpc) {
diff --git a/tudocomp_amd/csrc/prim.hpp b/tudocomp_amd/csrc/prim.hpp
--- a/tudocomp_amd/csrc/prim.hpp
+++ b/tudocomp_amd/csrc/prim.hpp
@@ -19,7 +19,7 @@
 
 void msd_partition_pairs_u32(Ctx& c, const u32* idx, const u32* val, size_t m, int bits, int db, u32* out_idx, u32* out_val, u32* tmp_idx, u32* tmp_val);
 
-struct SegTables { u32* blk_start; u32* blk_seg; u32* counts; u32* bs; u32 R, blocks_ub, rows; };
+struct SegTables { u32* blk_start; u32* blk_seg; u32* counts; u32* bs; u32 R, blocks_ub, rows; u32* cs = nullptr; u32 CB = 0;  };
 struct UnitTables { u32* unit_rng; u32* cls_list; u32* large; u32 cap, large_cap; u32 hc[6];  int wide_classes = 0;  u32 whc[16] = {0, 0, 0, 0, 0, 0, 0, 0, 0, 0, 0, 0, 0, 0, 0, 0};  };
 constexpr int WIDE_NCLS = 10;
 __host__ __device__ inline u32 wide_class(u32 m) {
@@ -28,7 +28,8 @@
     return 9u;
 }
 u32* ss_first_segment(Ctx& c, size_t n);
-void ss_level_tables(Ctx& c, const u32* seg_start, u32 nseg, size_t n, u32 D, SegTables& T);
+void ss_level_tables(Ctx& c, const u32* seg_start, u32 nseg, size_t n, u32 D, SegTables& T, u32 tile = 4096);
+void ss_level_chunks(Ctx& c, SegTables& T, u32 D);
 void ss_level_offsets(Ctx& c, const SegTables& T, const u32* seg_start, u32 nseg, u32 D, u32* nstart, size_t n);
 void ss_level_offsets_sub(Ctx& c, const SegTables& T, u32 nsub, const u32* blk_super, const u32* out_start, u32 nsuper, u32 D, u32* nstart, size_t n);
 void ss_build_units(Ctx& c, const u32* leaf_start, u32 nleaf, UnitTables& U, u32 small = 0);
diff --git a/tudocomp_amd/csrc/ssort.hip b/tudocomp_amd/csrc/ssort.hip
--- a/tudocomp_amd/csrc/ssort.hip
+++ b/tudocomp_amd/csrc/ssort.hip
@@ -123,12 +123,12 @@
     else if (i == NS) sp[i] = ~0ull;
 }
 
-__global__ void ss_nblk_kernel(const u32* __restrict__ seg_start, u32 nseg, u32 R, u32* __restrict__ nblk) {
+__global__ void ss_nblk_kernel(const u32* __restrict__ seg_start, u32 nseg, u32 R, u32* __restrict__ nblk, u32 tile = SS_TILE) {
     const u32 s = blockIdx.x * blockDim.x + threadIdx.x;
     if (s > nseg) return;
     if (s == nseg) { nblk[s] = 0; return; }
     const u64 size = seg_start[s + 1] - seg_start[s];
-    nblk[s] = (u32)((size + (u64)SS_TILE * R - 1) / ((u64)SS_TILE * R));
+    nblk[s] = (u32)((size + (u64)tile * R - 1) / ((u64)tile * R));
 }
 __global__ void ss_blkseg_kernel(const u32* __restrict__ blk_start, u32 nseg, u32* __restrict__ blk_seg) {
     const u32 s = blockIdx.x * blockDim.x + threadIdx.x;
@@ -273,6 +273,199 @@
     }
 }
 __global__ void ss_set_word_kernel(u32* p, u32 v) { *p = v; }
+
+struct SWGeo { u32 W, TPR, RP, RW, CH, NBW, GPB; };
+__host__ __device__ inline SWGeo sw_geo(u32 R, u32 D) {
+    SWGeo g;
+    g.W = D < 1024u ? D : 1024u;
+    g.TPR = g.W / 4;
+    g.RP = 256u / g.TPR;
+    g.RW = R > g.RP ? R : g.RP;
+    g.CH = g.RW / g.RP;
+    g.NBW = g.RW / R;
+    g.GPB = g.RP / g.NBW;
+    return g;
+}
+__device__ __forceinline__ uint4 sw_add(uint4 a, uint4 b) { return make_uint4(a.x + b.x, a.y + b.y, a.z + b.z, a.w + b.w); }
+__device__ __forceinline__ uint4 sw_rows_sum(const u32* __restrict__ counts, u32 row, u32 CH, u32 rows_end, u32 D, u32 col) {
+    uint4 acc = make_uint4(0, 0, 0, 0);
+    const uint4* p = (const uint4*)(counts + (size_t)row * D + col);
+    const size_t st = D / 4;
+    u32 k = 0;
+    if (row + CH <= rows_end) {
+        for (; k + 4 <= CH; k += 4) {
+            const uint4 a = p[(size_t)k * st], b = p[(size_t)(k + 1) * st], c2 = p[(size_t)(k + 2) * st], d2 = p[(size_t)(k + 3) * st];
+            acc = sw_add(acc, sw_add(sw_add(a, b), sw_add(c2, d2)));
+        }
+    }
+    for (; k < CH; ++k) if (row + k < rows_end) acc = sw_add(acc, p[(size_t)k * st]);
+    return acc;
+}
+__global__ __launch_bounds__(256) void sw_blocksum_kernel(const u32* __restrict__ counts, const u32* __restrict__ nblk_p, u32 R, u32 D, u32* __restrict__ bs) {
+    __shared__ uint4 part[256];
+    const SWGeo G = sw_geo(R, D);
+    const u32 nblk = *nblk_p, rows_end = nblk * R;
+    const u32 row0 = blockIdx.x * G.RW;
+    if (row0 >= rows_end) return;
+    const u32 tc = threadIdx.x % G.TPR, r0 = threadIdx.x / G.TPR;
+    for (u32 c0 = 0; c0 < D; c0 += G.W) {
+        part[threadIdx.x] = sw_rows_sum(counts, row0 + r0 * G.CH, G.CH, rows_end, D, c0 + 4 * tc);
+        __syncthreads();
+        if (threadIdx.x < G.NBW * G.TPR) {
+            const u32 j = threadIdx.x / G.TPR, q = threadIdx.x % G.TPR;
+            const u32 blk = row0 / R + j;
+            if (blk < nblk) {
+                uint4 s = make_uint4(0, 0, 0, 0);
+                for (u32 g = 0; g < G.GPB; ++g) s = sw_add(s, part[(j * G.GPB + g) * G.TPR + q]);
+                *(uint4*)(bs + (size_t)blk * D + c0 + 4 * q) = s;
+            }
+        }
+        __syncthreads();
+    }
+}
+__global__ __launch_bounds__(256) void sw_apply_kernel(u32* __restrict__ counts, const u32* __restrict__ nblk_p, u32 R, u32 D, const u32* __restrict__ bs) {
+    __shared__ uint4 part[256];
+    const SWGeo G = sw_geo(R, D);
+    const u32 nblk = *nblk_p, rows_end = nblk * R;
+    const u32 row0 = blockIdx.x * G.RW;
+    if (row0 >= rows_end) return;
+    const u32 tc = threadIdx.x % G.TPR, r0 = threadIdx.x / G.TPR;
+    const u32 row = row0 + r0 * G.CH;
+    const u32 blk = row / R;
+    for (u32 c0 = 0; c0 < D; c0 += G.W) {
+        const u32 col = c0 + 4 * tc;
+        part[threadIdx.x] = sw_rows_sum(counts, row, G.CH, rows_end, D, col);
+        __syncthreads();
+        if (blk < nblk) {
+            uint4 run = *(const uint4*)(bs + (size_t)blk * D + col);
+            for (u32 g = r0 - r0 % G.GPB; g < r0; ++g) run = sw_add(run, part[g * G.TPR + tc]);
+            uint4* p = (uint4*)(counts + (size_t)row * D + col);
+            const size_t st = D / 4;
+            for (u32 k = 0; k < G.CH && row + k < rows_end; ++k) {
+                const uint4 v = p[(size_t)k * st];
+                p[(size_t)k * st] = run;
+                run = sw_add(run, v);
+            }
+        }
+        __syncthreads();
+    }
+}
+__device__ __forceinline__ u32 sw_seg_of(const u32* __restrict__ blk_start, u32 nseg, u32 b) {
+    u32 lo = 0, hi = nseg;
+    while (hi - lo > 1) { const u32 mid = lo + (hi - lo) / 2; if (blk_start[mid] <= b) lo = mid; else hi = mid; }
+    return lo;
+}
+__global__ __launch_bounds__(256) void sw_chunksum_kernel(const u32* __restrict__ bs, const u32* __restrict__ blk_start, u32 nseg, u32 D, u32 CB, u32* __restrict__ cs) {
+    const u32 nblk = blk_start[nseg];
+    const u32 b0 = blockIdx.x * CB;
+    if (b0 >= nblk) return;
+    const u32 b1 = b0 + CB < nblk ? b0 + CB : nblk;
+    const u32 sF = sw_seg_of(blk_start, nseg, b0), sL = sw_seg_of(blk_start, nseg, b1 - 1);
+    const u32 he = blk_start[sF + 1] < b1 ? blk_start[sF + 1] : b1;
+    const u32 tb = blk_start[sL] > b0 ? blk_start[sL] : b0;
+    for (u32 d = threadIdx.x; d < D; d += blockDim.x) {
+        u32 h = 0, t = 0;
+        for (u32 b = b0; b < he; ++b) h += bs[(size_t)b * D + d];
+        if (sF == sL) t = h;
+        else for (u32 b = tb; b < b1; ++b) t += bs[(size_t)b * D + d];
+        cs[(size_t)(2 * blockIdx.x) * D + d] = h;
+        cs[(size_t)(2 * blockIdx.x + 1) * D + d] = t;
+    }
+}
+__global__ __launch_bounds__(256) void sw_segscan_kernel(u32* __restrict__ bs, const u32* __restrict__ cs, const u32* __restrict__ blk_start,
+                                                         const u32* __restrict__ seg_start, u32 nseg, u32 D, u32 CB, u32 nchunks, u32* __restrict__ nstart, u32 n) {
+    __shared__ u32 tot[2048];
+    __shared__ u32 cin[2048];
+    __shared__ u32 wsum[4];
+    const u32 T = blockDim.x;
+    if (blockIdx.x >= nchunks) {
+        const u32 e = blockIdx.x - nchunks;
+        const u32 s1 = (e + 1) * 64 < nseg ? (e + 1) * 64 : nseg;
+        for (u32 s = e * 64; s < s1; ++s) {
+            if (blk_start[s] != blk_start[s + 1]) continue;
+            const u32 st = seg_start[s];
+            for (u32 d = threadIdx.x; d < D; d += T) nstart[(size_t)s * D + d] = st;
+        }
+        if (e == 0 && threadIdx.x == 0) nstart[(size_t)nseg * D] = n;
+        return;
+    }
+    const u32 nblk = blk_start[nseg];
+    const u32 c = blockIdx.x;
+    const u32 b0 = c * CB;
+    if (b0 >= nblk) return;
+    const u32 b1 = b0 + CB < nblk ? b0 + CB : nblk;
+    const u32 K = D / T;
+    u32 b = b0;
+    while (b < b1) {
+        const u32 s = sw_seg_of(blk_start, nseg, b);
+        const u32 sb = blk_start[s], se = blk_start[s + 1];
+        const u32 e = se < b1 ? se : b1;
+        const u32 clo = sb / CB, chi = (se - 1) / CB;
+        for (u32 d = threadIdx.x; d < D; d += T) {
+            u32 carry = 0, sum = 0;
+            if (sb < b0) for (u32 q = clo; q < c; ++q) carry += cs[(size_t)(2 * q + 1) * D + d];
+            for (u32 x = b; x < e; ++x) sum += bs[(size_t)x * D + d];
+            if (se > b1) for (u32 q = c + 1; q <= chi; ++q) sum += cs[(size_t)(2 * q) * D + d];
+            cin[d] = carry;
+            tot[d] = carry + sum;
+        }
+        __syncthreads();
+        {
+            u32 v[8], mine = 0;
+#pragma unroll
+            for (u32 i = 0; i < 8; ++i) { v[i] = i < K ? tot[threadIdx.x * K + i] : 0u; mine += v[i]; }
+            const u32 inc = wave_inclusive_sum(mine);
+            if (lane_id() == 63) wsum[wave_id()] = inc;
+            __syncthreads();
+            u32 run = seg_start[s] + inc - mine;
+            for (int w = 0; w < wave_id(); ++w) run += wsum[w];
+#pragma unroll
+            for (u32 i = 0; i < 8; ++i) if (i < K) { tot[threadIdx.x * K + i] = run; run += v[i]; }
+        }
+        __syncthreads();
+        for (u32 d = threadIdx.x; d < D; d += T) {
+            const u32 st = tot[d];
+            if (sb >= b0) nstart[(size_t)s * D + d] = st;
+            u32 run = st + cin[d];
+            u32 x = b;
+            for (; x + 4 <= e; x += 4) {
+                u32* q = bs + (size_t)x * D + d;
+                const u32 v0 = q[0], v1 = q[D], v2 = q[2 * (size_t)D], v3 = q[3 * (size_t)D];
+                q[0] = run; run += v0; q[D] = run; run += v1; q[2 * (size_t)D] = run; run += v2; q[3 * (size_t)D] = run; run += v3;
+            }
+            for (; x < e; ++x) { const size_t i = (size_t)x * D + d; const u32 v = bs[i]; bs[i] = run; run += v; }
+        }
+        __syncthreads();
+        b = e;
+    }
+}
+__global__ __launch_bounds__(256) void sw_tables_kernel(const u32* __restrict__ seg_start, u32 nseg, u32 tr_log2, u32* __restrict__ blk_start, u32* __restrict__ blk_seg) {
+    __shared__ u32 st[1025];
+    __shared__ u32 wsum[5];
+    u32 nb[4], mine = 0;
+#pragma unroll
+    for (u32 i = 0; i < 4; ++i) {
+        const u32 s = 4 * threadIdx.x + i;
+        nb[i] = 0;
+        if (s < nseg) nb[i] = (u32)(((u64)(seg_start[s + 1] - seg_start[s]) + ((u64)1 << tr_log2) - 1) >> tr_log2);
+        mine += nb[i];
+    }
+    u32 total;
+    u32 run = block_exclusive_sum<u32, 4>(mine, wsum, total);
+#pragma unroll
+    for (u32 i = 0; i < 4; ++i) {
+        const u32 s = 4 * threadIdx.x + i;
+        if (s <= nseg) { st[s] = run; blk_start[s] = run; }
+        run += nb[i];
+    }
+    __syncthreads();
+    for (u32 b = threadIdx.x; b < total; b += 256) {
+        u32 lo = 0, hi = nseg;
+        while (hi - lo > 1) { const u32 mid = lo + (hi - lo) / 2; if (st[mid] <= b) lo = mid; else hi = mid; }
+        blk_seg[b] = lo;
+    }
+}
+__global__ void sw_set2_kernel(u32* p, u32 a, u32 b) { p[0] = a; p[1] = b; }
 
 template <bool GEN, bool LAST>
 __global__ __launch_bounds__(256) __attribute__((amdgpu_waves_per_eu(4, 4))) void ss_scatter_kernel(SSLevel P, TextKeyGen g, u32 rows) {
@@ -649,34 +842,19 @@
     hipStream_t s = c.stream;
     const size_t mark = c.arena.mark();
     const u32 D = 1u << db;
-    u32* seg_start = c.arena.get<u32>(2);
-    ss_set_word_kernel<<<1, 1, 0, s>>>(seg_start, 0u);
-    LAUNCH_CHECK();
-    ss_set_word_kernel<<<1, 1, 0, s>>>(seg_start + 1, (u32)m);
-    LAUNCH_CHECK();
+    const u32* seg_start = ss_first_segment(c, m);
     u32 nseg = 1;
-    const u64 tiles = (m + SS_TILE - 1) / SS_TILE;
     for (int l = 0; l < 2; ++l) {
-        u32 R = 128;
-        while (R > 1 && (u64)nseg * R > tiles / 8 + 64) R >>= 1;
-        const u32 blocks_ub = (u32)((tiles + R - 1) / R) + nseg;
-        const u32 rows = blocks_ub * R;
         u32* nstart = c.arena.get<u32>((size_t)nseg * D + 1);
         const size_t lm = c.arena.mark();
-        u32* blk_start = c.arena.get<u32>((size_t)nseg + 1);
-        u32* blk_seg = c.arena.get<u32>(blocks_ub);
-        u32* counts = c.arena.get<u32>((size_t)rows * D);
-        u32* bs = c.arena.get<u32>((size_t)blocks_ub * D);
-        ss_nblk_kernel<<<cdiv((size_t)nseg + 1, 256), 256, 0, s>>>(seg_start, nseg, R, blk_start);
-        LAUNCH_CHECK();
-        exclusive_sum_u32(c, blk_start, blk_start, (size_t)nseg + 1, nullptr);
-        ss_blkseg_kernel<<<cdiv(nseg, 256), 256, 0, s>>>(blk_start, nseg, blk_seg);
-        LAUNCH_CHECK();
+        SegTables T;
+        ss_level_tables(c, seg_start, nseg, m, D, T);
+        const u32 rows = T.rows;
         PSLevel P;
         P.idx_in = l == 0 ? idx : tmp_idx; P.val_in = l == 0 ? val : tmp_val;
         P.idx_out = l == 0 ? tmp_idx : out_idx; P.val_out = l == 0 ? tmp_val : out_val;
-        P.counts = counts; P.blk_seg = blk_seg; P.blk_start = blk_start; P.seg_start = seg_start;
-        P.nseg = nseg; P.R = R; P.shift = bits - db * (l + 1);
+        P.counts = T.counts; P.blk_seg = T.blk_seg; P.blk_start = T.blk_start; P.seg_start = seg_start;
+        P.nseg = nseg; P.R = T.R; P.shift = bits - db * (l + 1);
         P.per_xcd = (c.xcd_remap == 1 && rows >= 64) ? cdiv(rows, 8) : 0u;
         const u32 grid = P.per_xcd ? 8 * P.per_xcd : rows;
         {
@@ -685,17 +863,7 @@
             LAUNCH_CHECK();
             c.prof_end(pc);
         }
-        {
-            Ctx::ProfScope prof(c, K_SCAN, (u64)rows * D * 12);
-            ss_blocksum_kernel<<<blocks_ub, 256, 0, s>>>(counts, blk_start, nseg, R, D, bs);
-            LAUNCH_CHECK();
-            ss_segbase_kernel<<<nseg, 1024, 0, s>>>(bs, blk_start, seg_start, D, nstart);
-            LAUNCH_CHECK();
-            ss_set_word_kernel<<<1, 1, 0, s>>>(nstart + (size_t)nseg * D, (u32)m);
-            LAUNCH_CHECK();
-            ss_apply_kernel<<<blocks_ub, 256, 0, s>>>(counts, blk_start, nseg, R, D, bs);
-            LAUNCH_CHECK();
-        }
+        ss_level_offsets(c, T, seg_start, nseg, D, nstart, m);
         {
             const int ps = c.prof_begin(K_RS_SCATTER_U32, (u64)m * 16);
             if (db == 9) ps_scatter_kernel<9><<<grid, 256, 0, s>>>(P, rows); else ps_scatter_kernel<8><<<grid, 256, 0, s>>>(P, rows);
@@ -992,11 +1160,7 @@
     }
 
     u16* digits = c.arena.get<u16>(align_up(n, SS_TILE) + SS_TILE);
-    u32* seg_start = c.arena.get<u32>(2);
-    ss_set_word_kernel<<<1, 1, 0, s>>>(seg_start, 0u);
-    LAUNCH_CHECK();
-    ss_set_word_kernel<<<1, 1, 0, s>>>(seg_start + 1, (u32)n);
-    LAUNCH_CHECK();
+    const u32* seg_start = ss_first_segment(c, n);
     u32 nseg = 1;
     int cur = gen ? -1 : 0;
     for (int l = 0; l < L; ++l) {
@@ -1005,29 +1169,18 @@
         const u32 D = last ? 2 * F[l] : F[l];
         u32 stride = 1;
         for (int q = l + 1; q < L; ++q) stride *= F[q];
-        const u64 tiles = (n + SS_TILE - 1) / SS_TILE;
-        u32 R = 128;
-        while (R > 1 && (u64)nseg * R > tiles / 8 + 64) R >>= 1;
-        const u32 blocks_ub = (u32)((tiles + R - 1) / R) + nseg;
-        const u32 rows = blocks_ub * R;
         u32* nstart = c.arena.get<u32>((size_t)nseg * D + 1);
         const size_t lm2 = c.arena.mark();
-        u32* blk_start = c.arena.get<u32>((size_t)nseg + 1);
-        u32* blk_seg = c.arena.get<u32>(blocks_ub);
-        u32* counts = c.arena.get<u32>((size_t)rows * D);
-        u32* bs = c.arena.get<u32>((size_t)blocks_ub * D);
-        ss_nblk_kernel<<<cdiv((size_t)nseg + 1, 256), 256, 0, s>>>(seg_start, nseg, R, blk_start);
-        LAUNCH_CHECK();
-        exclusive_sum_u32(c, blk_start, blk_start, (size_t)nseg + 1, nullptr);
-        ss_blkseg_kernel<<<cdiv(nseg, 256), 256, 0, s>>>(blk_start, nseg, blk_seg);
-        LAUNCH_CHECK();
+        SegTables T;
+        ss_level_tables(c, seg_start, nseg, n, D, T);
+        const u32 rows = T.rows;
         SSLevel P;
         P.keys_in = cur >= 0 ? keys[cur] : nullptr; P.vals_in = cur >= 0 ? vals[cur] : nullptr;
         const int nxt = cur < 0 ? 0 : (cur ^ 1);
         P.keys_out = keys[nxt]; P.vals_out = vals[nxt];
         P.digits = digits;
-        P.counts = counts; P.blk_seg = blk_seg; P.blk_start = blk_start; P.seg_start = seg_start; P.sp = sp;
-        P.nseg = nseg; P.F = F[l]; P.stride = stride; P.R = R; P.D = D;
+        P.counts = T.counts; P.blk_seg = T.blk_seg; P.blk_start = T.blk_start; P.seg_start = seg_start; P.sp = sp;
+        P.nseg = nseg; P.F = F[l]; P.stride = stride; P.R = T.R; P.D = D;
         P.per_xcd = (c.xcd_remap == 1 && rows >= 64) ? cdiv(rows, 8) : 0u;
         const u32 grid = P.per_xcd ? 8 * P.per_xcd : rows;
         {
@@ -1039,17 +1192,7 @@
             LAUNCH_CHECK();
             c.prof_end(pc);
         }
-        {
-            Ctx::ProfScope prof(c, K_SCAN, (u64)rows * D * 12);
-            ss_blocksum_kernel<<<blocks_ub, 256, 0, s>>>(counts, blk_start, nseg, R, D, bs);
-            LAUNCH_CHECK();
-            ss_segbase_kernel<<<nseg, 1024, 0, s>>>(bs, blk_start, seg_start, D, nstart);
-            LAUNCH_CHECK();
-            ss_set_word_kernel<<<1, 1, 0, s>>>(nstart + (size_t)nseg * D, (u32)n);
-            LAUNCH_CHECK();
-            ss_apply_kernel<<<blocks_ub, 256, 0, s>>>(counts, blk_start, nseg, R, D, bs);
-            LAUNCH_CHECK();
-        }
+        ss_level_offsets(c, T, seg_start, nseg, D, nstart, n);
         {
             const int ps = c.prof_begin(K_RS_SCATTER_U64, (u64)n * (gl ? 13 : 24));
             if (gl && last) ss_scatter_stable_kernel<true, true><<<grid, 256, 0, s>>>(P, g, rows);
@@ -1123,9 +1266,16 @@
     return cur;
 }
 
-void ss_level_tables(Ctx& c, const u32* seg_start, u32 nseg, size_t n, u32 D, SegTables& T) {
+static bool sw_applies(const Ctx& c, u32 D) { return c.level_wide && D >= 64 && D <= 2048 && (D & (D - 1)) == 0; }
+void ss_level_chunks(Ctx& c, SegTables& T, u32 D) {
+    T.cs = nullptr; T.CB = 0;
+    if (!sw_applies(c, D)) return;
+    T.CB = std::max(16u, cdiv(T.blocks_ub, 2048));
+    T.cs = c.arena.get<u32>((size_t)2 * cdiv(T.blocks_ub, T.CB) * D);
+}
+void ss_level_tables(Ctx& c, const u32* seg_start, u32 nseg, size_t n, u32 D, SegTables& T, u32 tile) {
     hipStream_t s = c.stream;
-    const u64 tiles = (n + SS_TILE - 1) / SS_TILE;
+    const u64 tiles = (n + tile - 1) / tile;
     u32 R = 128;
     while (R > 1 && (u64)nseg * R > tiles / 8 + 64) R >>= 1;
     T.R = R;
@@ -1135,38 +1285,59 @@
     T.blk_seg = c.arena.get<u32>(T.blocks_ub);
     T.counts = c.arena.get<u32>((size_t)T.rows * D);
     T.bs = c.arena.get<u32>((size_t)T.blocks_ub * D);
-    ss_nblk_kernel<<<cdiv((size_t)nseg + 1, 256), 256, 0, s>>>(seg_start, nseg, R, T.blk_start);
+    ss_level_chunks(c, T, D);
+    const u64 tr = (u64)tile * R;
+    if (c.level_wide && nseg < 1024 && (tr & (tr - 1)) == 0) {
+        u32 tr_log2 = 0;
+        while (((u64)1 << tr_log2) < tr) ++tr_log2;
+        sw_tables_kernel<<<1, 256, 0, s>>>(seg_start, nseg, tr_log2, T.blk_start, T.blk_seg);
+        LAUNCH_CHECK();
+        return;
+    }
+    ss_nblk_kernel<<<cdiv((size_t)nseg + 1, 256), 256, 0, s>>>(seg_start, nseg, R, T.blk_start, tile);
     LAUNCH_CHECK();
     exclusive_sum_u32(c, T.blk_start, T.blk_start, (size_t)nseg + 1, nullptr);
     ss_blkseg_kernel<<<cdiv(nseg, 256), 256, 0, s>>>(T.blk_start, nseg, T.blk_seg);
     LAUNCH_CHECK();
 }
-void ss_level_offsets(Ctx& c, const SegTables& T, const u32* seg_start, u32 nseg, u32 D, u32* nstart, size_t n) {
+static void ss_offsets(Ctx& c, const SegTables& T, const u32* nblk_p, const u32* blk_first, const u32* out_start, u32 nseg, u32 D, u32* nstart, size_t n) {
     hipStream_t s = c.stream;
     Ctx::ProfScope prof(c, K_SCAN, (u64)T.rows * D * 12);
-    ss_blocksum_kernel<<<T.blocks_ub, 256, 0, s>>>(T.counts, T.blk_start, nseg, T.R, D, T.bs);
+    if (T.cs) {
+        const SWGeo G = sw_geo(T.R, D);
+        const u32 grid = cdiv(T.rows, G.RW), nchunks = cdiv(T.blocks_ub, T.CB), TB = D < 256 ? D : 256;
+        sw_blocksum_kernel<<<grid, 256, 0, s>>>(T.counts, nblk_p, T.R, D, T.bs);
+        LAUNCH_CHECK();
+        sw_chunksum_kernel<<<nchunks, TB, 0, s>>>(T.bs, blk_first, nseg, D, T.CB, T.cs);
+        LAUNCH_CHECK();
+        sw_segscan_kernel<<<nchunks + cdiv(nseg, 64), TB, 0, s>>>(T.bs, T.cs, blk_first, out_start, nseg, D, T.CB, nchunks, nstart, (u32)n);
+        LAUNCH_CHECK();
+        sw_apply_kernel<<<grid, 256, 0, s>>>(T.counts, nblk_p, T.R, D, T.bs);
+        LAUNCH_CHECK();
+        return;
+    }
+    ss_blocksum_kernel<<<T.blocks_ub, 256, 0, s>>>(T.counts, nblk_p, 0, T.R, D, T.bs);
     LAUNCH_CHECK();
-    ss_segbase_kernel<<<nseg, 1024, 0, s>>>(T.bs, T.blk_start, seg_start, D, nstart);
+    ss_segbase_kernel<<<nseg, 1024, 0, s>>>(T.bs, blk_first, out_start, D, nstart);
     LAUNCH_CHECK();
     ss_set_word_kernel<<<1, 1, 0, s>>>(nstart + (size_t)nseg * D, (u32)n);
     LAUNCH_CHECK();
-    ss_apply_kernel<<<T.blocks_ub, 256, 0, s>>>(T.counts, T.blk_start, nseg, T.R, D, T.bs);
+    ss_apply_kernel<<<T.blocks_ub, 256, 0, s>>>(T.counts, nblk_p, 0, T.R, D, T.bs);
     LAUNCH_CHECK();
 }
+void ss_level_offsets(Ctx& c, const SegTables& T, const u32* seg_start, u32 nseg, u32 D, u32* nstart, size_t n) {
+    ss_offsets(c, T, T.blk_start + nseg, T.blk_start, seg_start, nseg, D, nstart, n);
+}
 void ss_level_offsets_sub(Ctx& c, const SegTables& T, u32 nsub, const u32* blk_super, const u32* out_start, u32 nsuper, u32 D, u32* nstart, size_t n) {
-    hipStream_t s = c.stream;
-    Ctx::ProfScope prof(c, K_SCAN, (u64)T.rows * D * 12);
-    ss_blocksum_kernel<<<T.blocks_ub, 256, 0, s>>>(T.counts, T.blk_start, nsub, T.R, D, T.bs);
-    LAUNCH_CHECK();
-    ss_segbase_kernel<<<nsuper, 1024, 0, s>>>(T.bs, blk_super, out_start, D, nstart);
-    LAUNCH_CHECK();
-    ss_set_word_kernel<<<1, 1, 0, s>>>(nstart + (size_t)nsuper * D, (u32)n);
-    LAUNCH_CHECK();
-    ss_apply_kernel<<<T.blocks_ub, 256, 0, s>>>(T.counts, T.blk_start, nsub, T.R, D, T.bs);
-    LAUNCH_CHECK();
+    ss_offsets(c, T, T.blk_start + nsub, blk_super, out_start, nsuper, D, nstart, n);
 }
 u32* ss_first_segment(Ctx& c, size_t n) {
     u32* seg_start = c.arena.get<u32>(2);
+    if (c.level_wide) {
+        sw_set2_kernel<<<1, 1, 0, c.stream>>>(seg_start, 0u, (u32)n);
+        LAUNCH_CHECK();
+        return seg_start;
+    }
     ss_set_word_kernel<<<1, 1, 0, c.stream>>>(seg_start, 0u);
     LAUNCH_CHECK();
     ss_set_word_kernel<<<1, 1, 0, c.stream>>>(seg_start + 1, (u32)n);
diff --git a/tudocomp_amd/csrc/wsort.hip b/tudocomp_amd/csrc/wsort.hip
--- a/tudocomp_amd/csrc/wsort.hip
+++ b/tudocomp_amd/csrc/wsort.hip
@@ -1403,6 +1403,7 @@
             Tb.blk_seg = c.arena.get<u32>(Tb.blocks_ub);
             Tb.counts = c.arena.get<u32>((size_t)Tb.rows * D);
             Tb.bs = c.arena.get<u32>((size_t)Tb.blocks_ub * D);
+            ss_level_chunks(c, Tb, D);
             ws_sub_nblk_kernel<<<cdiv((size_t)nsub + 1, 256), 256, 0, s>>>(seg_begin, seg_end, nsub, R, Tb.blk_start);
             LAUNCH_CHECK();
             exclusive_sum_u32(c, Tb.blk_start, Tb.blk_start, (size_t)nsub + 1, nullptr);
```

Result: no change. 8749 MB/s, median of 6 (+0.7%).
